# jianzongwu/betrayed-by-captions

Measured on NVIDIA B200. Metric: decoder_head_images_per_sec_1024, higher is better.
Workload: dtype bf16

## Files before the change

### betrayed-by-captions_b200/csrc/api.cu

```cuda
#include "../../include/cgg_b200.h"
#include "kernels.h"
#include "gemm_tc.h"
#include "gemm_tf32.h"
#include "tc_state.h"

#include <math.h>
#include <stdio.h>
#include <string.h>
#include <stdlib.h>
#include <string>
#include <vector>

using namespace cgg;

struct cgg_handle {
  cgg_config cfg;
  std::string err;
  bool prepared = false;
  int H4 = 0, W4 = 0, lh[CGG_NUM_LEVELS] = {0, 0, 0}, lw[CGG_NUM_LEVELS] = {0, 0, 0};
  int nl[CGG_NUM_LEVELS] = {0, 0, 0};
  float* pos_level[CGG_NUM_LEVELS] = {nullptr, nullptr, nullptr};
  float* wkv[CGG_NUM_LEVELS] = {nullptr, nullptr, nullptr};
  float* rk[CGG_NUM_LEVELS] = {nullptr, nullptr, nullptr};
  float* bkv[CGG_NUM_LEVELS] = {nullptr, nullptr, nullptr};
  TcState* tc = nullptr;
  cudaStream_t side[2] = {nullptr, nullptr};
  cudaEvent_t ev_fork = nullptr, ev_join[2] = {nullptr, nullptr}, ev_kv[CGG_NUM_LEVELS] = {nullptr, nullptr, nullptr};
  cudaEvent_t ev_me[CGG_MAX_LAYERS + 1] = {};
  bool overlap_kv = false;
  bool final_mask_only = false;
  TcState* tc_aux = nullptr;
  Tf32Ctx* tf32 = nullptr;
  struct K7Buf {
    __nv_bfloat16 *pred_hl = nullptr, *cap_hl = nullptr, *dst_hl = nullptr, *capT_hl = nullptr;
    float* S = nullptr;
    size_t n_pred = 0, n_cap = 0, n_dst = 0, n_capT = 0, n_S = 0;
    void release() {
      cudaFree(pred_hl); cudaFree(cap_hl); cudaFree(dst_hl); cudaFree(capT_hl); cudaFree(S);
      pred_hl = cap_hl = dst_hl = capT_hl = nullptr; S = nullptr; n_pred = n_cap = n_dst = n_capT = n_S = 0;
    }
  } k7;
  void free_tables() {
    for (int l = 0; l < CGG_NUM_LEVELS; ++l) {
      cudaFree(pos_level[l]); cudaFree(wkv[l]); cudaFree(rk[l]); cudaFree(bkv[l]);
      pos_level[l] = wkv[l] = rk[l] = bkv[l] = nullptr;
    }
  }
};

namespace {

int fail(cgg_handle* h, int code, const std::string& msg) {
  if (h) h->err = msg;
  return code;
}
#define CU(call)                                                                              \
  do {                                                                                        \
    cudaError_t e__ = (call);                                                                 \
    if (e__ != cudaSuccess)                                                                   \
      return fail(h, CGG_ERR_CUDA, std::string(#call) + ": " + cudaGetErrorString(e__));      \
  } while (0)
#define ST(call)                       \
  do {                                 \
    int s__ = (call);                  \
    if (s__ != CGG_OK) return s__;     \
  } while (0)

inline size_t align_up(size_t x) { return (x + 255) & ~(size_t)255; }

struct Workspace {
  size_t total = 0;
  size_t kv[CGG_NUM_LEVELS];
  size_t z, h1, h2, me, qb, kb, vb, o, t, x1, x2, f, xs, bitmap, allm, tcws;
  void carve(const cgg_handle* h, int B) {
    const cgg_config& c = h->cfg;
    size_t off = 0;
    auto take = [&](size_t bytes) { size_t o = off; off += align_up(bytes); return o; };
    const size_t kv_elt = (c.precision == CGG_BF16) ? 2 : 4;
    for (int l = 0; l < CGG_NUM_LEVELS; ++l)
      kv[l] = take((size_t)B * h->lh[l] * h->lw[l] * h->nl[l] * 2 * c.embed_dim * kv_elt);
    const size_t bqc = (size_t)B * c.num_queries * c.embed_dim * sizeof(float);
    z = take(bqc); h1 = take(bqc); h2 = take(bqc); me = take(bqc); qb = take(bqc); kb = take(bqc);
    vb = take(bqc); o = take(bqc); t = take(bqc); x1 = take(bqc); x2 = take(bqc);
    f = take((size_t)B * c.num_queries * c.ffn_dim * sizeof(float));
    xs = take(bqc * (c.num_layers + 1));
    int maxk = 0;
    for (int l = 0; l < CGG_NUM_LEVELS; ++l) maxk = max(maxk, h->lh[l] * h->lw[l]);
    bitmap = take((size_t)B * c.num_queries * ((maxk + 31) / 32) * sizeof(uint32_t));
    allm = take((size_t)B * c.num_queries);
    tcws = take(tc_workspace_bytes(h->tc, B));
    total = off;
  }
};

template <typename T>
T* at(void* ws, size_t off) { return reinterpret_cast<T*>(static_cast<char*>(ws) + off); }

int check_ws(cgg_handle* h, int B, void* ws, size_t bytes, Workspace& w) {
  if (!h->prepared) return fail(h, CGG_ERR_NOT_PREPARED, "cgg_prepare() has not been called");
  if (B <= 0) return fail(h, CGG_ERR_BAD_SHAPE, "batch must be positive");
  w.carve(h, B);
  if (!ws || bytes < w.total) return fail(h, CGG_ERR_WORKSPACE, "workspace too small");
  return CGG_OK;
}

int linear_rows(cgg_handle* h, cudaStream_t s, const float* x, const float* a2, int a2_mod, const float* W,
                const float* bias, float* y, int rows, int N, int K, float alpha = 1.f,
                const float* R = nullptr, bool relu = false) {
  GemmF32 p;
  p.A = x; p.sAm = K; p.sAk = 1;
  if (a2) { p.A2 = a2; p.sA2m = K; p.sA2k = 1; p.a2_mod = a2_mod; }
  p.W = W; p.sWn = K; p.sWk = 1;
  p.bias = bias; p.alpha = alpha;
  if (R) { p.R = R; p.sRm = N; p.sRn = 1; p.r_mod = rows; }
  p.C = y; p.sCm = N; p.sCn = 1;
  p.M = rows; p.N = N; p.K = K; p.batch = 1;
  if (relu) p.relu_from = 0;
  CU(launch_gemm_f32(p, s));
  return CGG_OK;
}

}

extern "C" const char* cgg_version(void) { return "1.0 sm_100a"; }

extern "C" uint64_t cgg_launch_count(void) { return (uint64_t)cgg::launch_count(); }

extern "C" const char* cgg_last_error(const cgg_handle* h) { return h ? h->err.c_str() : "null handle"; }

extern "C" int cgg_create(cgg_handle** out, const cgg_config* cfg) {
  if (!out || !cfg) return CGG_ERR_NULL;
  *out = nullptr;
  if (cfg->embed_dim != 256 || cfg->num_heads != 8) return CGG_ERR_UNSUPPORTED;
  if (cfg->num_layers < 1 || cfg->num_layers > CGG_MAX_LAYERS) return CGG_ERR_BAD_SHAPE;
  if (cfg->num_queries < 1 || cfg->num_queries > 1024 || cfg->ffn_dim < 1 || cfg->num_classes_p1 < 1 ||
      cfg->d_lang < 0 || (cfg->d_lang == 0 && cfg->pred_emb_norm))
    return CGG_ERR_BAD_SHAPE;
  if (cfg->precision != CGG_FP32 && cfg->precision != CGG_BF16) return CGG_ERR_UNSUPPORTED;
  int ndev = 0;
  if (cudaGetDeviceCount(&ndev) != cudaSuccess || ndev == 0) return CGG_ERR_CUDA;
  cgg_handle* h = new (std::nothrow) cgg_handle();
  if (!h) return CGG_ERR_CUDA;
  h->cfg = *cfg;
  if (cfg->precision == CGG_BF16) {
    h->tc = tc_create(*cfg);
    if (!h->tc) { delete h; return CGG_ERR_CUDA; }
    {
      int lo = 0, hi = 0;
      cudaDeviceGetStreamPriorityRange(&lo, &hi);
      bool ok = true;
      for (int i = 0; i < 2; ++i) ok = ok && cudaStreamCreateWithPriority(&h->side[i], cudaStreamNonBlocking, lo) == cudaSuccess;
      ok = ok && cudaEventCreateWithFlags(&h->ev_fork, cudaEventDisableTiming) == cudaSuccess;
      for (int i = 0; i < 2; ++i) ok = ok && cudaEventCreateWithFlags(&h->ev_join[i], cudaEventDisableTiming) == cudaSuccess;
      for (int i = 0; i < CGG_NUM_LEVELS; ++i) ok = ok && cudaEventCreateWithFlags(&h->ev_kv[i], cudaEventDisableTiming) == cudaSuccess;
      for (int i = 0; i <= CGG_MAX_LAYERS; ++i) ok = ok && cudaEventCreateWithFlags(&h->ev_me[i], cudaEventDisableTiming) == cudaSuccess;
      h->overlap_kv = ok;
// ... 89 lines not shown
  Workspace w;
  w.carve(h, batch);
  return w.total;
}

extern "C" size_t cgg_workspace_offset(const cgg_handle* h, int batch, const char* what) {
  if (!h || !h->prepared || batch <= 0 || !what) return (size_t)-1;
  Workspace w;
  w.carve(h, batch);
  const std::string n(what);
  if (n == "kv0") return w.kv[0];
  if (n == "kv1") return w.kv[1];
  if (n == "kv2") return w.kv[2];
  const size_t o = tc_workspace_offset(h->tc, batch, what);
  return o == (size_t)-1 ? o : w.tcws + o;
}

static int kv_project_levels(cgg_handle* h, const cgg_weights* w, int batch, const void* const memories[CGG_NUM_LEVELS],
                             void* workspace, size_t workspace_bytes, cudaStream_t s, int l_begin, int l_end,
                             int cta_cap = 0) {
  if (!h || !w || !memories) return CGG_ERR_NULL;
  Workspace ws;
  ST(check_ws(h, batch, workspace, workspace_bytes, ws));
  const int C = h->cfg.embed_dim;
  for (int l = l_begin; l < l_end; ++l) {
    if (h->nl[l] == 0) continue;
    if (!memories[l]) return fail(h, CGG_ERR_NULL, "null memory level");
    const int K = h->lh[l] * h->lw[l], N = h->nl[l] * 2 * C;
    if (h->cfg.precision == CGG_BF16) {
      int st = tc_kv_project(h->tc, l, batch, memories[l], at<void>(workspace, ws.kv[l]), at<void>(workspace, ws.tcws), s, cta_cap);
      if (st != CGG_OK) return fail(h, st, std::string("tc_kv_project: ") + tc_last_error(h->tc));
      continue;
    }
    GemmF32 p;
    p.A = static_cast<const float*>(memories[l]); p.sAb = (long)C * K; p.sAm = 1; p.sAk = K; p.a_mmajor = true;
    p.W = h->wkv[l]; p.sWn = C; p.sWk = 1;
    p.bias = h->bkv[l];
    p.R = h->rk[l]; p.sRm = (long)h->nl[l] * C; p.sRn = 1; p.r_mod = K; p.r_ncols = h->nl[l] * C;
    p.C = at<float>(workspace, ws.kv[l]); p.sCb = (long)K * N; p.sCm = N; p.sCn = 1;
    p.M = K; p.N = N; p.K = C; p.batch = batch;
    CU(launch_gemm_f32(p, s));
  }
  return CGG_OK;
}

extern "C" int cgg_kv_project(cgg_handle* h, const cgg_weights* w, int batch, const void* const memories[CGG_NUM_LEVELS],
                              void* workspace, size_t workspace_bytes, void* stream) {
  return kv_project_levels(h, w, batch, memories, workspace, workspace_bytes, (cudaStream_t)stream, 0, CGG_NUM_LEVELS);
}

extern "C" int cgg_attn_mask_from_logits(cgg_handle* h, int batch, const float* mask_pred, int H4, int W4, int th,
                                         int tw, uint32_t* bitmap, uint8_t* all_masked, void* stream) {
  if (!h || !mask_pred || !bitmap || !all_masked) return CGG_ERR_NULL;
  if (batch <= 0 || H4 <= 0 || W4 <= 0 || th <= 0 || tw <= 0) return fail(h, CGG_ERR_BAD_SHAPE, "bad shape");
  CU(launch_mask_bits(mask_pred, batch * h->cfg.num_queries, H4, W4, th, tw, bitmap, all_masked, (cudaStream_t)stream));
  return CGG_OK;
}

static int head_call_impl(cgg_handle* h, const cgg_weights* w, int batch, const float* x, const void* mask_features,
                          int target_level, float* cls, float* emb, void* mask, float* mask_embed_out,
                          uint32_t* bitmap, uint8_t* all_masked, void* workspace, size_t workspace_bytes,
                          cudaStream_t s, int call_slot, bool defer_einsum, bool fds_ready, bool z_ready = false) {
  if (!h || !w || !x || !mask_features || !cls || (!emb && h->cfg.d_lang > 0)) return CGG_ERR_NULL;
  if (!mask && !defer_einsum) return CGG_ERR_NULL;
  Workspace ws;
  ST(check_ws(h, batch, workspace, workspace_bytes, ws));
  if (bitmap && (target_level < 0 || target_level >= CGG_NUM_LEVELS)) return fail(h, CGG_ERR_BAD_SHAPE, "bad level");
  if (bitmap && !all_masked) return CGG_ERR_NULL;
  const cgg_config& c = h->cfg;
  const int C = c.embed_dim, Q = c.num_queries, rows = batch * Q, HW = h->H4 * h->W4;
  float* z = at<float>(workspace, ws.z);
  float* h1 = at<float>(workspace, ws.h1);
  float* h2 = at<float>(workspace, ws.h2);
  float* me = mask_embed_out ? mask_embed_out : at<float>(workspace, ws.me);
  if (c.precision == CGG_BF16) {
    int st = tc_query_heads(h->tc, w, batch, x, cls, emb, me, at<void>(workspace, ws.tcws), s, call_slot, z_ready);
    if (st != CGG_OK) return fail(h, st, std::string("tc_query_heads: ") + tc_last_error(h->tc));
  } else {
  CU(launch_layernorm(x, nullptr, w->post_norm_w, w->post_norm_b, z, rows, C, 1e-5f, true, s));
  ST(linear_rows(h, s, z, nullptr, 1, w->cls_w, w->cls_b, cls, rows, c.num_classes_p1, C));
  if (c.d_lang > 0) ST(linear_rows(h, s, z, nullptr, 1, w->v2l_w, w->v2l_b, emb, rows, c.d_lang, C));
  ST(linear_rows(h, s, z, nullptr, 1, w->me_w[0], w->me_b[0], h1, rows, C, C, 1.f, nullptr, true));
  ST(linear_rows(h, s, h1, nullptr, 1, w->me_w[1], w->me_b[1], h2, rows, C, C, 1.f, nullptr, true));
  ST(linear_rows(h, s, h2, nullptr, 1, w->me_w[2], w->me_b[2], me, rows, C, C));
  }
  if (c.pred_emb_norm && c.d_lang > 0) CU(launch_l2norm_rows(emb, rows, c.d_lang, s));
  if (c.precision == CGG_BF16) {
    void* tws = at<void>(workspace, ws.tcws);
#define TC(call)                                                                                \
  do {                                                                                          \
    int st__ = (call);                                                                          \
    if (st__ != CGG_OK) return fail(h, st__, std::string(#call) + ": " + tc_last_error(h->tc)); \
  } while (0)
    TC(tc_store_mask_embed(h->tc, batch, call_slot, me, tws, s));
    if (bitmap) {
      if (!fds_ready) TC(tc_downsample(h->tc, batch, mask_features, tws, s));
      TC(tc_mask_bits(h->tc, batch, call_slot, target_level, bitmap, all_masked, tws, s));
    }
    if (!defer_einsum) TC(tc_mask_einsum(h->tc, batch, call_slot, 1, mask_features, mask, 0, tws, s));
    return CGG_OK;
  }
  GemmF32 p;
  p.A = static_cast<const float*>(mask_features); p.sAb = (long)C * HW; p.sAm = 1; p.sAk = HW; p.a_mmajor = true;
  p.W = me; p.sWb = (long)Q * C; p.sWn = C; p.sWk = 1;
  p.C = static_cast<float*>(mask); p.sCb = (long)Q * HW; p.sCm = 1; p.sCn = HW; p.c_mmajor = true;
  p.M = HW; p.N = Q; p.K = C; p.batch = batch;
  CU(launch_gemm_f32(p, s));
  if (bitmap)
    CU(launch_mask_bits(static_cast<const float*>(mask), rows, h->H4, h->W4, h->lh[target_level], h->lw[target_level],
                        bitmap, all_masked, s));
  return CGG_OK;
}

extern "C" int cgg_head_call(cgg_handle* h, const cgg_weights* w, int batch, const float* x, const void* mask_features,
                             int target_level, float* cls, float* emb, void* mask, float* mask_embed_out,
                             uint32_t* bitmap, uint8_t* all_masked, void* workspace, size_t workspace_bytes,
                             void* stream) {
  if (!mask) return CGG_ERR_NULL;
  return head_call_impl(h, w, batch, x, mask_features, target_level, cls, emb, mask, mask_embed_out, bitmap, all_masked,
                        workspace, workspace_bytes, (cudaStream_t)stream, 0, false, false);
}

extern "C" int cgg_mask_einsum(cgg_handle* h, int batch, int first_call, int num_calls, const void* mask_features,
                               void* mask, void* workspace, size_t workspace_bytes, void* stream) {
  if (!h || !mask_features || !mask) return CGG_ERR_NULL;
  if (h->cfg.precision != CGG_BF16) return fail(h, CGG_ERR_UNSUPPORTED, "cgg_mask_einsum is a CGG_BF16 stage");
  Workspace ws;
  ST(check_ws(h, batch, workspace, workspace_bytes, ws));
  if (first_call < 0 || num_calls < 1 || first_call + num_calls > h->cfg.num_layers + 1)
    return fail(h, CGG_ERR_BAD_SHAPE, "bad head-call range");
  const long call_stride = (long)batch * h->cfg.num_queries * h->H4 * h->W4;
  int st = tc_mask_einsum(h->tc, batch, first_call, num_calls, mask_features, mask, call_stride,
                          at<void>(workspace, ws.tcws), (cudaStream_t)stream);
  if (st != CGG_OK) return fail(h, st, std::string("tc_mask_einsum: ") + tc_last_error(h->tc));
  return CGG_OK;
}

extern "C" int cgg_masked_attention(cgg_handle* h, int batch, int num_keys, const float* q, const void* k,
                                    const void* v, long kv_stride, long kv_batch_stride, const uint32_t* bitmap,
                                    const uint8_t* all_masked, float* out, void* stream) {
  if (!h || !q || !k || !v || !out) return CGG_ERR_NULL;
  if (batch <= 0 || num_keys <= 0) return fail(h, CGG_ERR_BAD_SHAPE, "bad shape");
  cudaStream_t s = (cudaStream_t)stream;
  if (h->cfg.precision == CGG_BF16) {
    int st = tc_attention(h->tc, batch, num_keys, q, k, v, kv_stride, kv_batch_stride, bitmap, all_masked, out, nullptr, s);
    if (st != CGG_OK) return fail(h, st, std::string("tc_attention: ") + tc_last_error(h->tc));
    return CGG_OK;
  }
  CU(launch_attention_f32(q, k, v, false, kv_stride, kv_batch_stride, bitmap, all_masked, out, nullptr, batch,
                          h->cfg.num_queries, num_keys, h->cfg.num_heads, s));
  return CGG_OK;
}

static int decoder_layer_impl(cgg_handle* h, const cgg_weights* w, int batch, int layer, const float* x_in,
                              const uint32_t* bitmap, const uint8_t* all_masked, float* x_out, void* workspace,
                              size_t workspace_bytes, void* stream, bool chained_in, bool chained_out,
                              bool q_ready = false);

extern "C" int cgg_decoder_layer(cgg_handle* h, const cgg_weights* w, int batch, int layer, const float* x_in,
                                 const uint32_t* bitmap, const uint8_t* all_masked, float* x_out, void* workspace,
                                 size_t workspace_bytes, void* stream) {
  return decoder_layer_impl(h, w, batch, layer, x_in, bitmap, all_masked, x_out, workspace, workspace_bytes, stream, false,
                            false);
}

static int decoder_layer_impl(cgg_handle* h, const cgg_weights* w, int batch, int layer, const float* x_in,
                              const uint32_t* bitmap, const uint8_t* all_masked, float* x_out, void* workspace,
                              size_t workspace_bytes, void* stream, bool chained_in, bool chained_out, bool q_ready) {
  if (!h || !w || !x_in || !x_out) return CGG_ERR_NULL;
  cudaStream_t s = (cudaStream_t)stream;
  Workspace ws;
  ST(check_ws(h, batch, workspace, workspace_bytes, ws));
  const cgg_config& c = h->cfg;
  if (layer < 0 || layer >= c.num_layers) return fail(h, CGG_ERR_BAD_SHAPE, "bad layer index");
  const int C = c.embed_dim, Q = c.num_queries, rows = batch * Q, F = c.ffn_dim;
  const int l = layer % CGG_NUM_LEVELS, sl = layer / CGG_NUM_LEVELS, n = h->nl[l];
  const int K = h->lh[l] * h->lw[l];
  if (c.precision == CGG_BF16) {
    const long kvs = (long)n * 2 * C, kvb = (long)K * kvs;
    const __nv_bfloat16* kv = at<__nv_bfloat16>(workspace, ws.kv[l]);
    int st = tc_decoder_layer(h->tc, w, batch, layer, x_in, kv + (size_t)sl * C, kv + (size_t)(n + sl) * C, kvs, kvb, K,
                              bitmap, all_masked, x_out, at<void>(workspace, ws.tcws), s, chained_in, chained_out, q_ready);
    if (st != CGG_OK) return fail(h, st, std::string("tc_decoder_layer: ") + tc_last_error(h->tc));
    return CGG_OK;
  }
  const cgg_layer_weights& lw = w->layers[layer];
  const float qscale = 1.0f / sqrtf((float)(C / c.num_heads));
  float* qb = at<float>(workspace, ws.qb);
  float* kb = at<float>(workspace, ws.kb);
  float* vb = at<float>(workspace, ws.vb);
  float* o = at<float>(workspace, ws.o);
  float* t = at<float>(workspace, ws.t);
  float* x1 = at<float>(workspace, ws.x1);
  float* x2 = at<float>(workspace, ws.x2);
  float* f = at<float>(workspace, ws.f);
  ST(linear_rows(h, s, x_in, w->query_embed, Q, lw.cross_in_w, lw.cross_in_b, qb, rows, C, C, qscale));
  const long kv_stride = (long)n * 2 * C, kv_bstride = (long)K * kv_stride;
  if (c.precision == CGG_BF16) {
    const __nv_bfloat16* kv = at<__nv_bfloat16>(workspace, ws.kv[l]);
    ST(cgg_masked_attention(h, batch, K, qb, kv + (size_t)sl * C, kv + (size_t)(n + sl) * C, kv_stride, kv_bstride,
                            bitmap, all_masked, o, stream));
  } else {
    const float* kv = at<float>(workspace, ws.kv[l]);
    ST(cgg_masked_attention(h, batch, K, qb, kv + (size_t)sl * C, kv + (size_t)(n + sl) * C, kv_stride, kv_bstride,
                            bitmap, all_masked, o, stream));
  }
  ST(linear_rows(h, s, o, nullptr, 1, lw.cross_out_w, lw.cross_out_b, t, rows, C, C, 1.f, x_in));
  CU(launch_layernorm(t, nullptr, lw.norm_w[0], lw.norm_b[0], x1, rows, C, 1e-5f, true, s));
  ST(linear_rows(h, s, x1, w->query_embed, Q, lw.self_in_w, lw.self_in_b, qb, rows, C, C, qscale));
  ST(linear_rows(h, s, x1, w->query_embed, Q, lw.self_in_w + (size_t)C * C, lw.self_in_b + C, kb, rows, C, C));
  ST(linear_rows(h, s, x1, nullptr, 1, lw.self_in_w + (size_t)2 * C * C, lw.self_in_b + 2 * C, vb, rows, C, C));
  CU(launch_attention_f32(qb, kb, vb, false, C, (long)Q * C, nullptr, nullptr, o, nullptr, batch, Q, Q, c.num_heads, s));
  ST(linear_rows(h, s, o, nullptr, 1, lw.self_out_w, lw.self_out_b, t, rows, C, C, 1.f, x1));
  CU(launch_layernorm(t, nullptr, lw.norm_w[1], lw.norm_b[1], x2, rows, C, 1e-5f, true, s));
  ST(linear_rows(h, s, x2, nullptr, 1, lw.ffn_w1, lw.ffn_b1, f, rows, F, C, 1.f, nullptr, true));
  ST(linear_rows(h, s, f, nullptr, 1, lw.ffn_w2, lw.ffn_b2, t, rows, C, F, 1.f, x2));
  CU(launch_layernorm(t, nullptr, lw.norm_w[2], lw.norm_b[2], x_out, rows, C, 1e-5f, true, s));
  return CGG_OK;
}

extern "C" int cgg_set_final_mask_only(cgg_handle* h, int on) {
  if (!h) return CGG_ERR_NULL;
  if (on && h->cfg.precision != CGG_BF16) return fail(h, CGG_ERR_UNSUPPORTED, "final-mask-only is a CGG_BF16 option");
  h->final_mask_only = on != 0;
  return CGG_OK;
}

extern "C" int cgg_decoder_forward(cgg_handle* h, const cgg_weights* w, int batch, const void* mask_features,
                                   const void* const memories[CGG_NUM_LEVELS], float* cls, float* emb, void* mask,
                                   float* x_states, uint32_t* const* bitmaps, uint8_t* all_masked, void* workspace,
                                   size_t workspace_bytes, void* stream) {
  if (!h || !w || !mask_features || !memories || !cls || (!emb && h->cfg.d_lang > 0) || !mask) return CGG_ERR_NULL;
  cudaStream_t s = (cudaStream_t)stream;
  Workspace ws;
  ST(check_ws(h, batch, workspace, workspace_bytes, ws));
  const cgg_config& c = h->cfg;
  const int C = c.embed_dim, Q = c.num_queries, L = c.num_layers;
  const size_t bqc = (size_t)batch * Q * C;
  const size_t HW = (size_t)h->H4 * h->W4;
  const size_t mask_elt = (c.precision == CGG_BF16) ? 2 : 4;
  float* xs = x_states ? x_states : at<float>(workspace, ws.xs);
  const bool tcm = c.precision == CGG_BF16;
  const bool ovl_kv = tcm && h->overlap_kv && L >= CGG_NUM_LEVELS;
  void* tws = at<void>(workspace, ws.tcws);
  if (ovl_kv) {
    CU(cudaEventRecord(h->ev_fork, s));
    CU(cudaStreamWaitEvent(h->side[0], h->ev_fork, 0));
    ST(kv_project_levels(h, w, batch, memories, workspace, workspace_bytes, s, 0, 1));
    for (int l = 1; l < CGG_NUM_LEVELS; ++l) {
      ST(kv_project_levels(h, w, batch, memories, workspace, workspace_bytes, h->side[0], l, l + 1));
      CU(cudaEventRecord(h->ev_kv[l], h->side[0]));
    }
  } else {
    ST(cgg_kv_project(h, w, batch, memories, workspace, workspace_bytes, stream));
  }
  if (tcm) {
    int st = tc_downsample(h->tc, batch, mask_features, tws, s);
    if (st != CGG_OK) return fail(h, st, std::string("tc_downsample: ") + tc_last_error(h->tc));
  }
  CU(launch_broadcast_rows(w->query_feat, xs, batch, Q, C, s));
  for (int j = 0; j <= L; ++j) {
    const bool need_mask = j < L;
    const bool q_par = ovl_kv && j > 0 && j < L;
    if (q_par) {
      CU(cudaEventRecord(h->ev_me[j], s));
      CU(cudaStreamWaitEvent(h->side[1], h->ev_me[j], 0));
      int st = tc_layer_qproj(h->tc, w, batch, j, tws, h->side[1]);
      if (st != CGG_OK) return fail(h, st, std::string("tc_layer_qproj: ") + tc_last_error(h->tc));
      CU(cudaEventRecord(h->ev_join[1], h->side[1]));
    }
    uint32_t* bm = need_mask ? ((bitmaps && bitmaps[j]) ? bitmaps[j] : at<uint32_t>(workspace, ws.bitmap)) : nullptr;
    uint8_t* am = need_mask ? (all_masked ? all_masked + (size_t)j * batch * Q : at<uint8_t>(workspace, ws.allm))
                            : nullptr;
    ST(head_call_impl(h, w, batch, xs + j * bqc, mask_features, j % CGG_NUM_LEVELS,
                      cls + (size_t)j * batch * Q * c.num_classes_p1, emb ? emb + (size_t)j * batch * Q * c.d_lang : nullptr,
                      static_cast<char*>(mask) + (size_t)j * batch * Q * HW * mask_elt, nullptr, bm, am, workspace,
                      workspace_bytes, s, j, tcm, true, tcm && j > 0));
    if (j < L) {
      const int lvl = j % CGG_NUM_LEVELS;
      if (ovl_kv && j == lvl && lvl > 0) CU(cudaStreamWaitEvent(s, h->ev_kv[lvl], 0));
      if (q_par) CU(cudaStreamWaitEvent(s, h->ev_join[1], 0));
      ST(decoder_layer_impl(h, w, batch, j, xs + j * bqc, bm, am, xs + (j + 1) * bqc, workspace, workspace_bytes, stream,
                            tcm && j > 0, tcm, q_par));
    }
  }
  if (tcm && h->final_mask_only) {
    int st = tc_mask_einsum(h->tc, batch, L, 1, mask_features, mask, (long)batch * Q * HW, tws, s);
    if (st != CGG_OK) return fail(h, st, std::string("tc_mask_einsum: ") + tc_last_error(h->tc));
  } else if (tcm) {
    int st = tc_mask_einsum(h->tc, batch, 0, L + 1, mask_features, mask, (long)batch * Q * HW, tws, s);
    if (st != CGG_OK) return fail(h, st, std::string("tc_mask_einsum: ") + tc_last_error(h->tc));
  }
  return CGG_OK;
}

extern "C" int cgg_noun_embeddings(cgg_handle* h, const float* table, const float* ln_w, const float* ln_b,
                                   const int64_t* ids, int n_ids, int d_lang, float eps, int text_emb_norm, float* out,
                                   void* stream) {
  if (!h || !table || !ids || !out) return CGG_ERR_NULL;
  if (text_emb_norm && (!ln_w || !ln_b)) return CGG_ERR_NULL;
  if (n_ids < 0 || d_lang <= 0) return fail(h, CGG_ERR_BAD_SHAPE, "bad shape");
  CU(launch_layernorm(table, ids, ln_w, ln_b, out, n_ids, d_lang, eps, text_emb_norm != 0, (cudaStream_t)stream));
  return CGG_OK;
}

extern "C" int cgg_similarity(cgg_handle* h, const float* a, const float* b, int M, int N, int D, float scale,
// ... 491 lines not shown
```

### betrayed-by-captions_b200/csrc/gemm_tc.cu

```cuda
#include "gemm_tc.h"
#include "kernels.h"
#include <cuda_fp16.h>
#include "tc_ptx.cuh"
#include "tc_state.h"

#include <cuda.h>
#include <cuda_bf16.h>
#include <string>
#include <stdio.h>
#include <stdlib.h>

namespace cgg {

namespace {

constexpr int TC_THREADS = 64 + 16 * 32;
constexpr int TC_BM = 128;
constexpr int TC_BK = 64;
constexpr int A_CHUNK_BYTES = 2 * 64 * 64 * 2;

enum { EPI_MASK_T = 0, EPI_ROWMAJOR = 1, EPI_BITS = 2, EPI_LINEAR_T = 3 };

struct TcGemmP {
  int NT, N_TILE, KC, stages;
  int a_resident;
  int a_kmajor;
  int k_identity;
  int a_kcoord[12];
  int b_kcoord[12];
  int split_cpc, split_K;
  TcSeg seg[3]; int nseg; const float* lin_bias; int n_tokens;
  long kpart_stride;
  int b_row0;
  int b_rows_per_batch;
  int acc_stride;
  int tmem_cols;
  int epi;
  int dbg;
  int f16;
  int ein_split, q_rows;
  int M_valid;
  int m_tiles, n_batch, n_work;
  __nv_bfloat16* out_mask; long out_call_stride, out_batch_stride, HW; int Q, q_pad, n_calls;
  __nv_bfloat16* out_rows; long ld_out, out_rows_batch_stride; const float* bias; const __nv_bfloat16* R;
  long ldr; int r_ncols;
  uint32_t* bitmap; int W32;
};

__device__ __forceinline__ bool masked_from_logit(float d) {
  return (1.0f / (1.0f + expf(-d))) < 0.5f;
}

__device__ __forceinline__ uint32_t pack_bf16x2(float lo, float hi) {
  __nv_bfloat162 v = __floats2bfloat162_rn(lo, hi);
  return *reinterpret_cast<uint32_t*>(&v);
}

__device__ __forceinline__ void split_bf16(float x, __nv_bfloat16& hi, __nv_bfloat16& lo) {
  hi = __float2bfloat16_rn(x);
  lo = __float2bfloat16_rn(x - __bfloat162float(hi));
}
__device__ __forceinline__ uint32_t pack2(__nv_bfloat16 a, __nv_bfloat16 b) {
  return (uint32_t)__bfloat16_as_ushort(a) | ((uint32_t)__bfloat16_as_ushort(b) << 16);
}


__device__ long long g_tc_trace[64];
#define TC_TRACE(gi, slot)                                                                         \
  do {                                                                                             \
    if ((p.dbg & 1) && blockIdx.x == 0 && (gi) >= 16 && (gi) < 24) g_tc_trace[((gi) - 16) * 8 + (slot)] = clock64(); \
  } while (0)

constexpr int EPI_WARPS = 16;
constexpr int EPI_PARTS = EPI_WARPS / 4;

struct EpiCtx {
  int lane, m, batch, part, chunks, wi, col0, g = -1;
  bool m_ok;
  uint32_t taddr;
};

__device__ __forceinline__ void epi_mask_t(const TcGemmP& p, const EpiCtx& c, uint8_t* sStage, const CUtensorMap* tmC,
                                           bool leader_warp, bool last, int m_tile, uint64_t* acc_empty_bar,
                                           bool arrive_on_leader) {
  const bool leader = leader_warp && c.lane == 0;
  static_assert(EPI_PARTS == 4, "four chunk slots per warp below");
  uint32_t r0[16], r1[16], r2[16], r3[16];
  const int ch0 = c.part, ch1 = c.part + 4, ch2 = c.part + 8, ch3 = c.part + 12;
  const bool on0 = ch0 < c.chunks, on1 = ch1 < c.chunks, on2 = ch2 < c.chunks, on3 = ch3 < c.chunks;
  if (on0) ptx::tmem_ld16_issue(c.taddr + (uint32_t)(ch0 * 16), r0);
  if (on1) ptx::tmem_ld16_issue(c.taddr + (uint32_t)(ch1 * 16), r1);
  if (on2) ptx::tmem_ld16_issue(c.taddr + (uint32_t)(ch2 * 16), r2);
  if (on3) ptx::tmem_ld16_issue(c.taddr + (uint32_t)(ch3 * 16), r3);
  if (on0) ptx::tmem_ld_wait16(r0);
  if (on1) ptx::tmem_ld_wait16(r1);
  if (on2) ptx::tmem_ld_wait16(r2);
  if (on3) ptx::tmem_ld_wait16(r3);
  ptx::tc_fence_before();
  __syncwarp();
  if (c.lane == 0) {
    if (arrive_on_leader) ptx::mbar_arrive_leader(acc_empty_bar);
    else ptx::mbar_arrive(acc_empty_bar);
  }
  if (leader) ptx::tma_store_wait_read();
  asm volatile("bar.sync 1, %0;" ::"n"(EPI_WARPS * 32) : "memory");
  if (leader) TC_TRACE(c.g, 6);
  const int row = c.m & (TC_BM - 1);
  auto stage16 = [&](const uint32_t (&r)[16], int ch) {
    __nv_bfloat16* dst = reinterpret_cast<__nv_bfloat16*>(sStage) + (long)(ch * 16) * TC_BM + row;
#pragma unroll
    for (int i = 0; i < 16; ++i) dst[i * TC_BM] = __float2bfloat16_rn(__uint_as_float(r[i]));
  };
  if (on0) stage16(r0, ch0);
  if (on1) stage16(r1, ch1);
  if (on2) stage16(r2, ch2);
  if (on3) stage16(r3, ch3);
  if (leader) TC_TRACE(c.g, 7);
  ptx::fence_proxy_async_smem();
  asm volatile("bar.sync 1, %0;" ::"n"(EPI_WARPS * 32) : "memory");
  if (leader) {
    const int r0 = c.col0;
    const int N_TILE = c.chunks * 16, q_pad = p.q_pad;
    if (N_TILE >= q_pad) {
      for (int sidx = 0; sidx * q_pad + q_pad <= N_TILE || sidx == 0; ++sidx) {
        const int call = r0 / q_pad + sidx;
        if (call >= p.n_calls || sidx * q_pad >= N_TILE) break;
        ptx::tma_store_3d(tmC, sStage + (long)sidx * q_pad * TC_BM * 2, m_tile * TC_BM, 0, call * p.n_batch + c.batch);
      }
    } else {
      const int call = r0 / q_pad, q0 = r0 - call * q_pad;
      if (call < p.n_calls) ptx::tma_store_3d(tmC, sStage, m_tile * TC_BM, q0, call * p.n_batch + c.batch);
    }
    ptx::tma_store_commit();
    if (last) ptx::tma_store_wait_read();
  }
}

__device__ __forceinline__ void epi_rowmajor(const TcGemmP& p, const EpiCtx& c, uint8_t* sStage, const float* sBias,
                                             const CUtensorMap* tmC, bool leader_warp, bool last, int m_tile,
                                             uint64_t* acc_empty_bar, bool arrive_on_leader = false) {
  const bool leader = leader_warp && c.lane == 0;
  static_assert(EPI_PARTS == 4, "four chunk slots per warp below");
  uint32_t r0[16], r1[16], r2[16], r3[16];
  const int ch0 = c.part, ch1 = c.part + 4, ch2 = c.part + 8, ch3 = c.part + 12;
  const bool on0 = ch0 < c.chunks, on1 = ch1 < c.chunks, on2 = ch2 < c.chunks, on3 = ch3 < c.chunks;
  if (on0) ptx::tmem_ld16_issue(c.taddr + (uint32_t)(ch0 * 16), r0);
  if (on1) ptx::tmem_ld16_issue(c.taddr + (uint32_t)(ch1 * 16), r1);
  if (on2) ptx::tmem_ld16_issue(c.taddr + (uint32_t)(ch2 * 16), r2);
  if (on3) ptx::tmem_ld16_issue(c.taddr + (uint32_t)(ch3 * 16), r3);
  if (on0) ptx::tmem_ld_wait16(r0);
  if (on1) ptx::tmem_ld_wait16(r1);
  if (on2) ptx::tmem_ld_wait16(r2);
  if (on3) ptx::tmem_ld_wait16(r3);
  ptx::tc_fence_before();
  __syncwarp();
  if (c.lane == 0) {
    if (arrive_on_leader) ptx::mbar_arrive_leader(acc_empty_bar);
    else ptx::mbar_arrive(acc_empty_bar);
  }
  if (leader) ptx::tma_store_wait_read();
  asm volatile("bar.sync 1, %0;" ::"n"(EPI_WARPS * 32) : "memory");
  const int row = c.m & (TC_BM - 1);
  auto stage16 = [&](const uint32_t (&r)[16], int ch) {
    const float* bf = sBias + c.col0 + ch * 16;
    uint4 o[2];
    uint32_t* ow = reinterpret_cast<uint32_t*>(o);
#pragma unroll
    for (int i = 0; i < 8; ++i)
      ow[i] = pack_bf16x2(__uint_as_float(r[2 * i]) + bf[2 * i], __uint_as_float(r[2 * i + 1]) + bf[2 * i + 1]);
    const int sub = ch >> 2, j = (ch & 3) * 2;
    uint8_t* base = sStage + sub * (TC_BM * 128) + row * 128;
    *reinterpret_cast<uint4*>(base + ((j ^ (row & 7)) << 4)) = o[0];
    *reinterpret_cast<uint4*>(base + (((j + 1) ^ (row & 7)) << 4)) = o[1];
  };
  if (on0) stage16(r0, ch0);
  if (on1) stage16(r1, ch1);
  if (on2) stage16(r2, ch2);
  if (on3) stage16(r3, ch3);
  ptx::fence_proxy_async_smem();
  asm volatile("bar.sync 1, %0;" ::"n"(EPI_WARPS * 32) : "memory");
  if (leader) {
    const int subs = c.chunks >> 2;
    for (int sub = 0; sub < subs; ++sub)
      ptx::tma_store_3d(tmC, sStage + sub * (TC_BM * 128), c.col0 + sub * 64, m_tile * TC_BM, c.batch);
    ptx::tma_store_commit();
    if (last) ptx::tma_store_wait_read();
  }
}

__device__ __forceinline__ void epi_bits_impl(int Q, int W32, uint32_t* bitmap, const EpiCtx& c) {
  uint32_t* brow = bitmap + (long)c.batch * Q * W32 + c.wi;
  const bool w_ok = c.wi < W32;
  for (int ch = c.part; ch < c.chunks; ch += EPI_PARTS) {
    float v[16];
    ptx::tmem_ld16(c.taddr + (uint32_t)(ch * 16), v);
    const int q0 = c.col0 + ch * 16;
#pragma unroll
    for (int i = 0; i < 16; ++i) {
      const uint32_t word = __ballot_sync(0xffffffffu, c.m_ok && v[i] <= -1.7881392e-07f);
      if (c.lane == 0 && w_ok && q0 + i < Q) brow[(long)(q0 + i) * W32] = word;
    }
  }
}
__device__ __forceinline__ void epi_bits(const TcGemmP& p, const EpiCtx& c) { epi_bits_impl(p.Q, p.W32, p.bitmap, c); }

struct LinCtx {
  bool on = false;
  int f = 0, mode = 0, rb_mod = 1, split_off = 0;
  long ld = 0, rb_ld = 0, res_ld = 0;
  float bias = 0.f, alpha = 1.f, floor = -INFINITY;
  void* ptr = nullptr;
  const float* rowbias = nullptr;
  const float* res = nullptr;
  __device__ __forceinline__ void init(const TcGemmP& p, int m) {
#pragma unroll
    for (int sgi = 0; sgi < 3; ++sgi) {
      if (sgi < p.nseg && m >= p.seg[sgi].col0 && m < p.seg[sgi].col0 + p.seg[sgi].ncols) {
        on = true;
        f = m - p.seg[sgi].col0;
        mode = p.seg[sgi].is_bf16 == 3 ? 3 : (p.seg[sgi].is_bf16 ? (p.seg[sgi].split ? 2 : 1) : 0);
        floor = p.seg[sgi].relu ? 0.f : -INFINITY;
        ptr = p.seg[sgi].ptr; ld = p.seg[sgi].ld; alpha = p.seg[sgi].alpha;
        rowbias = p.seg[sgi].rowbias; rb_mod = p.seg[sgi].rb_mod; rb_ld = p.seg[sgi].rb_ld;
        res = p.seg[sgi].res; res_ld = p.seg[sgi].res_ld; split_off = p.seg[sgi].ncols;
      }
    }
    if (on && p.lin_bias) bias = __ldg(p.lin_bias + m);
    if (blockIdx.z > 0) {
      bias = 0.f; res = nullptr; rowbias = nullptr;
      ptr = static_cast<float*>(ptr) + (long)blockIdx.z * p.kpart_stride;
    }
  }
};

struct LinPre {
  float a[16], b[16];
};
__device__ __forceinline__ void lin_prefetch(const TcGemmP& p, const EpiCtx& c, const LinCtx& L, LinPre& pre) {
  const int tok_base = c.batch * p.NT * p.N_TILE;
#pragma unroll
  for (int i = 0; i < 16; ++i) pre.a[i] = pre.b[i] = 0.f;
  if (!L.on || (L.rowbias == nullptr && L.res == nullptr)) return;
#pragma unroll
  for (int j = 0; j < 2; ++j) {
    const int ch = c.part + j * EPI_PARTS;
    if (ch >= c.chunks) break;
    const int tok0 = tok_base + ch * 16;
    const int nvalid = min(16, p.n_tokens - tok0);
    float* dst = j ? pre.b : pre.a;
    if (L.rowbias) {
      int tq = tok0 % L.rb_mod;
#pragma unroll
      for (int i = 0; i < 16; ++i) {
        if (i < nvalid) dst[i] = __ldg(L.rowbias + (long)tq * L.rb_ld + L.f);
        if (++tq == L.rb_mod) tq = 0;
      }
    } else {
      const float* rp = L.res + (long)tok0 * L.res_ld + L.f;
#pragma unroll
      for (int i = 0; i < 16; ++i)
        if (i < nvalid) dst[i] = __ldg(rp + (long)i * L.res_ld);
    }
  }
}

template <int MODE, bool HAS_RB, bool HAS_RES>
__device__ __forceinline__ void epi_linear_t(const TcGemmP& p, const EpiCtx& c, const LinCtx& L, const LinPre* pre) {
  const int n_tokens = p.n_tokens;
  const int tok_base = c.batch * p.NT * p.N_TILE + c.col0;
  int j = 0;
  for (int ch = c.part; ch < c.chunks; ch += EPI_PARTS, ++j) {
    const int tok0 = tok_base + ch * 16;
    const int nvalid = L.on ? min(16, n_tokens - tok0) : 0;
    float rb[16], rs[16];
    if (HAS_RB) {
      if (pre && j < 2) {
#pragma unroll
        for (int i = 0; i < 16; ++i) rb[i] = j ? pre->b[i] : pre->a[i];
      } else {
        int tq = tok0 % L.rb_mod;
#pragma unroll
        for (int i = 0; i < 16; ++i) {
          rb[i] = (i < nvalid) ? __ldg(L.rowbias + (long)tq * L.rb_ld + L.f) : 0.f;
          if (++tq == L.rb_mod) tq = 0;
        }
      }
    }
    if (HAS_RES) {
      if (pre && j < 2) {
#pragma unroll
        for (int i = 0; i < 16; ++i) rs[i] = j ? pre->b[i] : pre->a[i];
      } else {
        const float* rp = L.res + (long)tok0 * L.res_ld + L.f;
#pragma unroll
        for (int i = 0; i < 16; ++i) rs[i] = (i < nvalid) ? __ldg(rp + (long)i * L.res_ld) : 0.f;
      }
    }
    float v[16];
    ptx::tmem_ld16(c.taddr + (uint32_t)(ch * 16), v);
#pragma unroll
    for (int i = 0; i < 16; ++i) {
      float x = v[i] + L.bias;
      if (HAS_RB) x += rb[i];
      x *= L.alpha;
      if (HAS_RES) x += rs[i];
      x = fmaxf(x, L.floor);
      if (i < nvalid) {
        const long off = (long)(tok0 + i) * L.ld + L.f;
        if (MODE == 0) {
          static_cast<float*>(L.ptr)[off] = x;
        } else if (MODE == 1) {
          static_cast<__nv_bfloat16*>(L.ptr)[off] = __float2bfloat16_rn(x);
        } else if (MODE == 3) {
          static_cast<__half*>(L.ptr)[off] = __float2half_rn(x);
        } else {
          __nv_bfloat16 hi, lo;
          split_bf16(x, hi, lo);
          static_cast<__nv_bfloat16*>(L.ptr)[off] = hi;
          static_cast<__nv_bfloat16*>(L.ptr)[off + L.split_off] = lo;
        }
      }
    }
  }
}

__device__ __forceinline__ void epi_linear_dispatch(const TcGemmP& p, const EpiCtx& c, const LinCtx& L, const LinPre* pre) {
  const bool rb = L.rowbias != nullptr, rs = L.res != nullptr;
  if (L.mode == 0) {
    if (rb) epi_linear_t<0, true, false>(p, c, L, pre);
    else if (rs) epi_linear_t<0, false, true>(p, c, L, pre);
    else epi_linear_t<0, false, false>(p, c, L, pre);
  } else if (L.mode == 1) {
    if (rb) epi_linear_t<1, true, false>(p, c, L, pre);
    else epi_linear_t<1, false, false>(p, c, L, pre);
  } else if (L.mode == 3) {
    epi_linear_t<3, false, false>(p, c, L, pre);
  } else {
    epi_linear_t<2, false, false>(p, c, L, pre);
  }
}

__device__ unsigned long long g_tc_stamps[16];
#define TC_STAMP(i)                                                            \
  do {                                                                         \
    if ((p.dbg & 1) && blockIdx.x == 0 && blockIdx.y == 0) g_tc_stamps[i] = ptx::global_timer_ns(); \
  } while (0)

template <int EPI>
__global__ void __launch_bounds__(TC_THREADS, 1)
tc_gemm_kernel(const __grid_constant__ CUtensorMap tmA, const __grid_constant__ CUtensorMap tmB,
               const __grid_constant__ CUtensorMap tmC, const __grid_constant__ TcGemmP p) {
  constexpr bool A_KMAJOR = (EPI == EPI_LINEAR_T);
  constexpr bool A_RESIDENT = (EPI == EPI_MASK_T || EPI == EPI_ROWMAJOR);
  extern __shared__ uint8_t smem_raw[];
  uint8_t* smem = reinterpret_cast<uint8_t*>((reinterpret_cast<uintptr_t>(smem_raw) + 1023) & ~(uintptr_t)1023);
  const int b_tile_bytes = p.N_TILE * 128;
  const int a_in_stage = A_RESIDENT ? 0 : A_CHUNK_BYTES;
  const int b_stage_bytes = a_in_stage + b_tile_bytes;
  uint8_t* sA = smem;
  uint8_t* sB = sA + (A_RESIDENT ? p.KC * A_CHUNK_BYTES : 0);
  uint64_t* bars = reinterpret_cast<uint64_t*>(sB + p.stages * b_stage_bytes);
  uint64_t* a_full = bars;
  uint64_t* a_empty = bars + 4;
  uint64_t* b_full = bars + 8;
  uint64_t* b_empty = b_full + p.stages;
  uint64_t* acc_full = b_empty + p.stages;
  uint64_t* acc_empty = acc_full + 2;
  uint32_t* tmem_slot = reinterpret_cast<uint32_t*>(acc_empty + 2);
  uint8_t* sStage = reinterpret_cast<uint8_t*>((reinterpret_cast<uintptr_t>(tmem_slot + 4) + 1023) & ~(uintptr_t)1023);
  float* sBias = reinterpret_cast<float*>(sStage + (size_t)p.N_TILE * TC_BM * 2);

  const int warp = threadIdx.x >> 5, lane = threadIdx.x & 31;
  const int n_work = A_RESIDENT ? p.n_work : 1;
  const int w_first = A_RESIDENT ? (int)blockIdx.x : 0;
  const int w_stride = A_RESIDENT ? (int)gridDim.x : 1;
  auto tile_of = [&](int w, int& m_tile, int& batch) {
    if (A_RESIDENT) { batch = w / p.m_tiles; m_tile = w - batch * p.m_tiles; }
    else { m_tile = blockIdx.x; batch = blockIdx.y; }
  };
  if (threadIdx.x == 0) TC_STAMP(0);
  auto kcoords = [&](int kc, int& ka, int& kb) {
    if (p.split_cpc > 0) {
      const int term = kc / p.split_cpc, j = kc - term * p.split_cpc;
      const int k0 = ((int)blockIdx.z * p.split_cpc + j) * TC_BK;
      ka = (term == 2 ? p.split_K : 0) + k0;
      kb = (term == 1 ? p.split_K : 0) + k0;
    } else if (p.k_identity) {
      ka = kb = ((int)blockIdx.z * p.KC + kc) * TC_BK;
    } else {
      ka = p.a_kcoord[kc]; kb = p.b_kcoord[kc];
    }
  };

  if (warp == 0 && lane == 0) {
    ptx::prefetch_tmap(&tmA);
    ptx::prefetch_tmap(&tmB);
    for (int i = 0; i < 4; ++i) { ptx::mbar_init(&a_full[i], 1); ptx::mbar_init(&a_empty[i], 1); }
    for (int i = 0; i < p.stages; ++i) { ptx::mbar_init(&b_full[i], 1); ptx::mbar_init(&b_empty[i], 1); }
    for (int i = 0; i < 2; ++i) { ptx::mbar_init(&acc_full[i], 1); ptx::mbar_init(&acc_empty[i], EPI_WARPS); }
    ptx::fence_mbar_init();
  }
  if (warp == 1) {
    ptx::tmem_alloc(tmem_slot, (uint32_t)p.tmem_cols);
    ptx::tmem_relinquish();
  }
  ptx::tc_fence_before();
  __syncthreads();
  ptx::tc_fence_after();
  const uint32_t tmem_base = *tmem_slot;
  if (threadIdx.x == 0) TC_STAMP(1);
  ptx::grid_dep_launch();
  int n_pre = 0;
  if (EPI == EPI_LINEAR_T && warp == 0 && lane == 0) {
    const int total = p.NT * p.KC;
    n_pre = total < p.stages ? total : p.stages;
    for (int i = 0; i < n_pre; ++i) {
      const int kc = i % p.KC;
      int kco, kcb;
      kcoords(kc, kco, kcb);
      ptx::mbar_expect_tx(&b_full[i], (uint32_t)b_stage_bytes);
      ptx::tma_load_2d(sB + i * b_stage_bytes, &tmA, &b_full[i], kco, (int)blockIdx.x * TC_BM);
    }
  }
  ptx::grid_dep_wait();

  if (warp == 0) {
    if (lane == 0) {
      int m_tile = 0, batch = 0;
      auto load_a = [&](uint8_t* dst, uint64_t* bar, int kc) {
        int kco, kcb;
        kcoords(kc, kco, kcb);
        if (A_KMAJOR) {
          ptx::tma_load_2d(dst, &tmA, bar, kco, m_tile * TC_BM);
        } else {
          for (int g = 0; g < 2; ++g)
            ptx::tma_load_3d(dst + g * (A_CHUNK_BYTES / 2), &tmA, bar, m_tile * TC_BM + g * 64, kco, batch);
        }
      };
      int it = 0, tl = 0;
      for (int w = w_first; w < n_work; w += w_stride, ++tl) {
       tile_of(w, m_tile, batch);
       if (A_RESIDENT && tl == 0)
         for (int kc = 0; kc < p.KC; ++kc) {
           ptx::mbar_expect_tx(&a_full[kc], (uint32_t)A_CHUNK_BYTES);
           load_a(sA + kc * A_CHUNK_BYTES, &a_full[kc], kc);
         }
       for (int t = 0; t < p.NT; ++t)
        for (int kc = 0; kc < p.KC; ++kc, ++it) {
          if (A_RESIDENT && t == 0 && tl > 0) {
            ptx::mbar_wait(&a_empty[kc], (uint32_t)(tl & 1) ^ 1u);
            ptx::mbar_expect_tx(&a_full[kc], (uint32_t)A_CHUNK_BYTES);
            load_a(sA + kc * A_CHUNK_BYTES, &a_full[kc], kc);
          }
          const int s = it % p.stages;
          const uint32_t ph = (uint32_t)(it / p.stages) & 1u;
          uint8_t* stage = sB + s * b_stage_bytes;
          if (it >= n_pre) {
            ptx::mbar_wait(&b_empty[s], ph ^ 1u);
            ptx::mbar_expect_tx(&b_full[s], (uint32_t)b_stage_bytes);
            if (!A_RESIDENT) load_a(stage, &b_full[s], kc);
          }
          int kca, kcb;
          kcoords(kc, kca, kcb);
          ptx::tma_load_2d(stage + a_in_stage, &tmB, &b_full[s], kcb, batch * p.b_rows_per_batch + p.b_row0 + t * p.N_TILE);
        }
      }
    }
  } else if (warp == 1) {
    const uint32_t idesc = ptx::umma_idesc_bf16(TC_BM, p.N_TILE,  !A_KMAJOR,  false, p.f16 != 0);
    const uint64_t ad0 = A_KMAJOR ? ptx::umma_desc_sw128(ptx::smem_u32(A_RESIDENT ? sA : sB), 16, 1024)
                                  : ptx::umma_desc_sw128(ptx::smem_u32(A_RESIDENT ? sA : sB), A_CHUNK_BYTES / 2, 1024);
    const uint64_t bd0 = ptx::umma_desc_sw128(ptx::smem_u32(sB + a_in_stage), 16, 1024);
    const uint32_t a_step = A_KMAJOR ? 2u : (2048u >> 4);
    const uint32_t stage16 = (uint32_t)b_stage_bytes >> 4;
    int it = 0, g = 0, tl = 0;
    for (int w = w_first; w < n_work; w += w_stride, ++tl)
      for (int t = 0; t < p.NT; ++t, ++g) {
        const int buf = g & 1;
        const uint32_t use = (uint32_t)(g >> 1);
        ptx::mbar_wait(&acc_empty[buf], (use & 1u) ^ 1u);
        ptx::tc_fence_after();
        const uint32_t d_tmem = tmem_base + (uint32_t)(buf * p.acc_stride);
        for (int kc = 0; kc < p.KC; ++kc, ++it) {
          const int s = it % p.stages;
          const uint32_t ph = (uint32_t)(it / p.stages) & 1u;
          if (A_RESIDENT && t == 0) ptx::mbar_wait(&a_full[kc], (uint32_t)(tl & 1));
          ptx::mbar_wait(&b_full[s], ph);
          ptx::tc_fence_after();
          if (it == 0 && lane == 0) TC_STAMP(2);
          if (ptx::elect_one()) {
            const uint64_t ad = ad0 + (uint64_t)(A_RESIDENT ? (uint32_t)kc * (A_CHUNK_BYTES >> 4) : (uint32_t)s * stage16);
            const uint64_t bd = bd0 + (uint64_t)((uint32_t)s * stage16);
#pragma unroll
            for (int k = 0; k < TC_BK / 16; ++k)
              ptx::mma_bf16_ss(d_tmem, ad + (uint64_t)(k * a_step), bd + (uint64_t)(k * 2), idesc, (kc | k) != 0 ? 1u : 0u);
            ptx::mma_commit(&b_empty[s]);
            if (A_RESIDENT && t == p.NT - 1) ptx::mma_commit(&a_empty[kc]);
            if (kc == p.KC - 1) ptx::mma_commit(&acc_full[buf]);
          }
          __syncwarp();
        }
        if (g == 0 && lane == 0) TC_STAMP(3);
      }
  } else {
    const int quarter = warp & 3;
    const int part = (warp - 2) >> 2;
    if (EPI == EPI_ROWMAJOR) {
      for (int i = threadIdx.x - 64; i < p.NT * p.N_TILE; i += EPI_WARPS * 32) sBias[i] = __ldg(p.bias + i);
      asm volatile("bar.sync 1, %0;" ::"n"(EPI_WARPS * 32) : "memory");
    }
    int g = 0;
    for (int w = w_first; w < n_work; w += w_stride) {
    int m_tile, batch;
    tile_of(w, m_tile, batch);
    const bool last_work = w + w_stride >= n_work;
    const int m = m_tile * TC_BM + quarter * 32 + lane;
    const bool m_ok = m < p.M_valid;
    EpiCtx ctx;
    ctx.lane = lane; ctx.m = m; ctx.m_ok = m_ok; ctx.batch = batch; ctx.part = part;
    ctx.chunks = p.N_TILE / 16; ctx.wi = (m_tile * TC_BM + quarter * 32) >> 5;
    LinCtx lin;
    LinPre pre;
    const bool use_pre = EPI == EPI_LINEAR_T && p.NT == 1;
    if (EPI == EPI_LINEAR_T) {
      lin.init(p, m);
      if (use_pre) lin_prefetch(p, ctx, lin, pre);
    }
    for (int t = 0; t < p.NT; ++t, ++g) {
      const int buf = g & 1;
      const uint32_t use = (uint32_t)(g >> 1);
      ptx::mbar_wait(&acc_full[buf], use & 1u);
      ptx::tc_fence_after();
      if (g == 0 && warp == 2 && lane == 0) TC_STAMP(4);
      ctx.taddr = tmem_base + (uint32_t)(buf * p.acc_stride) + ((uint32_t)(quarter * 32) << 16);
      ctx.col0 = t * p.N_TILE;
      const bool last = last_work && t == p.NT - 1;
      if (EPI == EPI_MASK_T) epi_mask_t(p, ctx, sStage, &tmC, warp == 2, last, m_tile, &acc_empty[buf], false);
      else if (EPI == EPI_ROWMAJOR) epi_rowmajor(p, ctx, sStage, sBias, &tmC, warp == 2, last, m_tile, &acc_empty[buf]);
      else if (EPI == EPI_BITS) epi_bits(p, ctx);
      else epi_linear_dispatch(p, ctx, lin, use_pre ? &pre : nullptr);
      if (EPI != EPI_MASK_T && EPI != EPI_ROWMAJOR) {
// ... 550 lines not shown
    const int quarter = warp & 3;
    EpiCtx ctx;
    ctx.lane = lane; ctx.batch = batch; ctx.part = (warp - 2) >> 2; ctx.chunks = p.N_TILE / 16; ctx.col0 = 0;
    int t = 0;
    for (int mt = blockIdx.x; mt < p.m_tiles; mt += gridDim.x, ++t) {
      const int buf = t & 1;
      ptx::mbar_wait(&acc_full[buf], ((uint32_t)(t >> 1)) & 1u);
      ptx::tc_fence_after();
      ctx.m = mt * TC_BM + quarter * 32 + lane;
      ctx.m_ok = ctx.m < p.K_valid;
      ctx.wi = (mt * TC_BM + quarter * 32) >> 5;
      ctx.taddr = tmem_base + (uint32_t)(buf * p.acc_stride) + ((uint32_t)(quarter * 32) << 16);
      epi_bits_impl(p.Q, p.W32, p.bitmap, ctx);
      ptx::tc_fence_before();
      __syncwarp();
      if (lane == 0) ptx::mbar_arrive(&acc_empty[buf]);
    }
  }
  ptx::tc_fence_before();
  __syncthreads();
  if (warp == 1) {
    __syncwarp();
    ptx::tmem_dealloc(tmem_base, (uint32_t)p.tmem_cols);
  }
}

__global__ void __launch_bounds__(256) downsample3_kernel(const __nv_bfloat16* __restrict__ F, int planes, int C, int H4,
                                                          int W4, __half* __restrict__ d8, __half* __restrict__ d4,
                                                          __half* __restrict__ d2, int p8, int p4, int p2) {
  ptx::grid_dep_launch();
  ptx::grid_dep_wait();
  const int bw = W4 >> 3, bh = H4 >> 3;
  const long idx = (long)blockIdx.x * blockDim.x + threadIdx.x;
  const long total = (long)planes * bh * bw;
  if (idx >= total) return;
  const int bx = (int)(idx % bw);
  const int by = (int)((idx / bw) % bh);
  const long plane = idx / ((long)bw * bh);
  const __nv_bfloat16* src = F + plane * (long)H4 * W4 + (long)by * 8 * W4 + bx * 8;
  float px[8][8];
#pragma unroll
  for (int r = 0; r < 8; ++r) {
    const uint4 x = *reinterpret_cast<const uint4*>(src + (long)r * W4);
    const __nv_bfloat162* h = reinterpret_cast<const __nv_bfloat162*>(&x);
#pragma unroll
    for (int j = 0; j < 4; ++j) {
      const float2 f = __bfloat1622float2(h[j]);
      px[r][2 * j] = f.x;
      px[r][2 * j + 1] = f.y;
    }
  }
  auto avg = [&](int r, int c) {
    return 0.5f * (0.5f * px[r][c] + 0.5f * px[r][c + 1]) + 0.5f * (0.5f * px[r + 1][c] + 0.5f * px[r + 1][c + 1]);
  };
  auto h2 = [](float a, float b) {
    const __half2 v = __floats2half2_rn(a, b);
    return *reinterpret_cast<const uint32_t*>(&v);
  };
  d8[plane * (long)p8 + (long)by * bw + bx] = __float2half_rn(avg(3, 3));
  {
    const int w = W4 >> 2;
    const long off = (long)(by * 2) * w + bx * 2;
#pragma unroll
    for (int r = 0; r < 2; ++r)
      *reinterpret_cast<uint32_t*>(d4 + plane * (long)p4 + off + (long)r * w) = h2(avg(4 * r + 1, 1), avg(4 * r + 1, 5));
  }
  {
    const int w = W4 >> 1;
    const long off = (long)(by * 4) * w + bx * 4;
#pragma unroll
    for (int r = 0; r < 4; ++r) {
      uint2 ph;
      ph.x = h2(avg(2 * r, 0), avg(2 * r, 2));
      ph.y = h2(avg(2 * r, 4), avg(2 * r, 6));
      *reinterpret_cast<uint2*>(d2 + plane * (long)p2 + off + (long)r * w) = ph;
    }
  }
}

__global__ void repitch_kernel(const __nv_bfloat16* __restrict__ src, __nv_bfloat16* __restrict__ dst, long rows, int K,
                               int pitch) {
  ptx::grid_dep_launch();
  ptx::grid_dep_wait();
  const long i = (long)blockIdx.x * blockDim.x + threadIdx.x;
  if (i >= rows * pitch) return;
  const int k = (int)(i % pitch);
  const long r = i / pitch;
  dst[i] = k < K ? src[r * K + k] : __float2bfloat16(0.f);
}

__global__ void store_me_kernel(const float* __restrict__ me, __nv_bfloat16* __restrict__ dst, int B, int Q, int C,
                                int rows_per_batch, int row0) {
  ptx::grid_dep_launch();
  ptx::grid_dep_wait();
  const long i = (long)blockIdx.x * blockDim.x + threadIdx.x;
  const long total = (long)B * Q * C;
  if (i >= total) return;
  const int c = (int)(i % C);
  const long bq = i / C;
  const int q = (int)(bq % Q);
  const int b = (int)(bq / Q);
  __nv_bfloat16* row = dst + ((long)b * rows_per_batch + row0 + q) * 2 * C;
  row[c] = __float2bfloat16_rn(me[i]);
  reinterpret_cast<__half*>(row)[C + c] = __float2half_rn(me[i]);
}

__global__ void __launch_bounds__(256) all_masked_kernel(const uint32_t* __restrict__ bitmap, int rows, int W32, int K,
                                                         uint8_t* __restrict__ all_masked) {
  ptx::grid_dep_launch();
  ptx::grid_dep_wait();
  const int row = blockIdx.x * 8 + (threadIdx.x >> 5), lane = threadIdx.x & 31;
  if (row >= rows) return;
  int cnt = 0;
  for (int i = lane; i < W32; i += 32) cnt += __popc(bitmap[(long)row * W32 + i]);
#pragma unroll
  for (int o = 16; o > 0; o >>= 1) cnt += __shfl_xor_sync(0xffffffffu, cnt, o);
  if (lane == 0) all_masked[row] = (cnt == K) ? 1 : 0;
}

inline int round_up(int x, int m) { return (x + m - 1) / m * m; }
inline size_t align256(size_t x) { return (x + 255) & ~(size_t)255; }

}

namespace {

int make_map_A(TcState* t, CUtensorMap* m, const void* base, int pixels, int C, int B, int pitch = -1) {
  if (pitch < 0) pitch = pixels;
  if ((pitch * 2) % 16 != 0 || (reinterpret_cast<uintptr_t>(base) & 15))
    return tc_fail(t, CGG_ERR_UNSUPPORTED, "TMA needs 16-byte aligned channel planes (pixel pitch multiple of 8)");
  cuuint64_t dims[3] = {(cuuint64_t)pixels, (cuuint64_t)C, (cuuint64_t)B};
  cuuint64_t strides[2] = {(cuuint64_t)pitch * 2, (cuuint64_t)pitch * C * 2};
  cuuint32_t box[3] = {64, 64, 1};
  cuuint32_t es[3] = {1, 1, 1};
  CUresult r = t->encode(m, CU_TENSOR_MAP_DATA_TYPE_BFLOAT16, 3, const_cast<void*>(base), dims, strides, box, es,
                         CU_TENSOR_MAP_INTERLEAVE_NONE, CU_TENSOR_MAP_SWIZZLE_128B, CU_TENSOR_MAP_L2_PROMOTION_L2_128B,
                         CU_TENSOR_MAP_FLOAT_OOB_FILL_NONE);
  if (r != CUDA_SUCCESS) return tc_fail(t, CGG_ERR_CUDA, "cuTensorMapEncodeTiled(A) failed: " + std::to_string((int)r));
  return CGG_OK;
}
int make_map_B(TcState* t, CUtensorMap* m, const void* base, long rows, int C, int n_tile) {
  cuuint64_t dims[2] = {(cuuint64_t)C, (cuuint64_t)rows};
  cuuint64_t strides[1] = {(cuuint64_t)C * 2};
  cuuint32_t box[2] = {64, (cuuint32_t)n_tile};
  cuuint32_t es[2] = {1, 1};
  CUresult r = t->encode(m, CU_TENSOR_MAP_DATA_TYPE_BFLOAT16, 2, const_cast<void*>(base), dims, strides, box, es,
                         CU_TENSOR_MAP_INTERLEAVE_NONE, CU_TENSOR_MAP_SWIZZLE_128B, CU_TENSOR_MAP_L2_PROMOTION_L2_256B,
                         CU_TENSOR_MAP_FLOAT_OOB_FILL_NONE);
  if (r != CUDA_SUCCESS) return tc_fail(t, CGG_ERR_CUDA, "cuTensorMapEncodeTiled(B) failed: " + std::to_string((int)r));
  return CGG_OK;
}

int launch_tc_gemm(TcState* t, const CUtensorMap& mA, const CUtensorMap& mB, TcGemmP p, int m_tiles, int batch,
                   cudaStream_t s, const CUtensorMap* mC = nullptr, int kparts = 1) {
  if (p.N_TILE % 16 != 0 || p.N_TILE < 16 || p.N_TILE > 256) return tc_fail(t, CGG_ERR_BAD_SHAPE, "bad N tile");
  p.acc_stride = p.N_TILE <= 128 ? 128 : 256;
  if (p.N_TILE <= 32) p.acc_stride = 32; else if (p.N_TILE <= 64) p.acc_stride = 64;
  p.tmem_cols = 2 * p.acc_stride;
  const size_t a_bytes = p.a_resident ? (size_t)p.KC * A_CHUNK_BYTES : 0;
  const size_t b_stage = (size_t)p.N_TILE * 128 + (p.a_resident ? 0 : A_CHUNK_BYTES);
  if (p.KC > 12 && !p.k_identity && p.split_cpc == 0) return tc_fail(t, CGG_ERR_BAD_SHAPE, "too many K chunks");
  const size_t stage_bytes = (p.epi == EPI_MASK_T || p.epi == EPI_ROWMAJOR)
                                 ? (size_t)p.N_TILE * TC_BM * 2 + 1024 + (p.epi == EPI_ROWMAJOR ? (size_t)p.NT * p.N_TILE * 4 : 0) : 0;
  const size_t budget = (size_t)204 * 1024 - stage_bytes;
  int stages = (int)((budget - a_bytes) / b_stage);
  if (stages > 8) stages = 8;
  if (stages > p.NT * p.KC) stages = p.NT * p.KC;
  if (stages < 2) return tc_fail(t, CGG_ERR_BAD_SHAPE, "tile does not fit shared memory");
  p.stages = stages;
  const size_t smem = 1024 + a_bytes + stages * b_stage + (8 + 2 * stages + 4) * 8 + 64 + stage_bytes;
  if (!t->smem_attr_set) {
    TCU(cudaFuncSetAttribute(tc_gemm_kernel<EPI_MASK_T>, cudaFuncAttributeMaxDynamicSharedMemorySize, 227 * 1024));
    TCU(cudaFuncSetAttribute(tc_gemm_kernel<EPI_ROWMAJOR>, cudaFuncAttributeMaxDynamicSharedMemorySize, 227 * 1024));
    TCU(cudaFuncSetAttribute(tc_gemm_kernel<EPI_BITS>, cudaFuncAttributeMaxDynamicSharedMemorySize, 227 * 1024));
    TCU(cudaFuncSetAttribute(tc_gemm_kernel<EPI_LINEAR_T>, cudaFuncAttributeMaxDynamicSharedMemorySize, 227 * 1024));
    t->smem_attr_set = true;
  }
  const bool want_res = (p.epi == EPI_MASK_T || p.epi == EPI_ROWMAJOR), want_km = (p.epi == EPI_LINEAR_T);
  if (want_res && p.KC > 4) return tc_fail(t, CGG_ERR_BAD_SHAPE, "resident A tile limited to 4 K chunks");
  if ((p.a_resident != 0) != want_res || (p.a_kmajor != 0) != want_km)
    return tc_fail(t, CGG_ERR_BAD_SHAPE, "operand layout does not match the kernel specialisation");
  static const bool timing = getenv("CGG_TC_TIMING") != nullptr;
  p.dbg = timing ? 1 : 0;
  cudaEvent_t e0 = nullptr, e1 = nullptr;
  if (timing) { cudaEventCreate(&e0); cudaEventCreate(&e1); cudaStreamSynchronize(s); cudaEventRecord(e0, s); }
  dim3 grid(m_tiles, batch, kparts);
  const dim3 block(TC_THREADS);
  p.m_tiles = m_tiles; p.n_batch = batch; p.n_work = m_tiles * batch;
  if (want_res) {
    const int persist = 1;
    if (t->num_sms == 0) {
      int dev = 0;
      cudaGetDevice(&dev);
      cudaDeviceGetAttribute(&t->num_sms, cudaDevAttrMultiProcessorCount, dev);
    }
    int ctas = persist ? (p.n_work < t->num_sms ? p.n_work : t->num_sms) : p.n_work;
    if (persist && t->cta_cap > 0 && ctas > t->cta_cap) ctas = t->cta_cap;
    grid = dim3(ctas, 1, 1);
  }
  const CUtensorMap& mCC = mC ? *mC : mB;
  switch (p.epi) {
    case EPI_MASK_T: TCU(launch_pdl(tc_gemm_kernel<EPI_MASK_T>, grid, block, smem, s, mA, mB, mCC, p)); break;
    case EPI_ROWMAJOR: TCU(launch_pdl(tc_gemm_kernel<EPI_ROWMAJOR>, grid, block, smem, s, mA, mB, mCC, p)); break;
    case EPI_BITS: TCU(launch_pdl(tc_gemm_kernel<EPI_BITS>, grid, block, smem, s, mA, mB, mCC, p)); break;
    default: TCU(launch_pdl(tc_gemm_kernel<EPI_LINEAR_T>, grid, block, smem, s, mA, mB, mCC, p)); break;
  }
  count_launch();
  TCU(cudaGetLastError());
  if (timing) {
    cudaEventRecord(e1, s);
    cudaStreamSynchronize(s);
    float ms = 0.f;
    cudaEventElapsedTime(&ms, e0, e1);
    unsigned long long st[16];
    cudaMemcpyFromSymbol(st, g_tc_stamps, sizeof(st));
    fprintf(stderr, "[tc_gemm] grid %dx%d epi %d NT %d KC %d N_TILE %d stages %d smem %zu: event %.1f us | setup %.1f first-data %.1f mma-issued %.1f "
            "acc-ready %.1f epi-done %.1f teardown %.1f (us since entry)\n", m_tiles, batch, p.epi, p.NT, p.KC, p.N_TILE, p.stages, smem,
            ms * 1e3, (st[1] - st[0]) * 1e-3, (st[2] - st[0]) * 1e-3, (st[3] - st[0]) * 1e-3, (st[4] - st[0]) * 1e-3,
            (st[5] - st[0]) * 1e-3, (st[6] - st[0]) * 1e-3);
    cudaEventDestroy(e0); cudaEventDestroy(e1);
  }
  return CGG_OK;
}

}

TcState* tc_create(const cgg_config& cfg) {
  TcState* t = new (std::nothrow) TcState();
  if (!t) return nullptr;
  t->cfg = cfg;
  void* fn = nullptr;
  cudaDriverEntryPointQueryResult qres;
  if (cudaGetDriverEntryPoint("cuTensorMapEncodeTiled", &fn, cudaEnableDefault, &qres) != cudaSuccess || !fn) {
    delete t;
    return nullptr;
  }
  t->encode = reinterpret_cast<EncodeTiledFn>(fn);
  const int Q = cfg.num_queries, calls = cfg.num_layers + 1;
  if (2 * round_up(Q, 8) <= 256 && calls % 2 == 0) {
    t->q_pad = round_up(Q, 8) < 16 ? 16 : round_up(Q, 8); t->ein_ntile = 2 * t->q_pad; t->ein_calls_per_tile = 2;
  } else if (round_up(Q, 16) <= 256) {
    t->q_pad = round_up(Q, 16); t->ein_ntile = t->q_pad; t->ein_calls_per_tile = 1;
  } else {
    t->q_pad = round_up(Q, 32); t->ein_ntile = t->q_pad / 2; t->ein_calls_per_tile = 0;
    if (t->ein_ntile > 256) { delete t; return nullptr; }
  }
  if (round_up(Q, 16) <= 256) { t->bits_ntile = round_up(Q, 16); t->bits_nt = 1; }
  else { t->bits_ntile = round_up(Q, 32) / 2; t->bits_nt = 2; }
  t->rows_per_batch = calls * t->q_pad;
  t->live_bytes = 1 << 20;
  if (cudaMalloc(&t->live_buf, t->live_bytes) != cudaSuccess) { delete t; return nullptr; }
  return t;
}

void tc_destroy(TcState* t) {
  if (!t) return;
  t->free_all();
  t->free_packed();
  cudaFree(t->live_buf);
  delete t;
}

const char* tc_last_error(const TcState* t) { return t ? t->err.c_str() : ""; }

size_t tc_workspace_bytes(const TcState* t, int batch) {
  if (!t) return 0;
  TcWs w;
  w.carve(t, batch);
  return w.total;
}

size_t tc_workspace_offset(const TcState* t, int batch, const char* what) {
  if (!t || !what) return (size_t)-1;
  TcWs w;
  w.carve(t, batch);
  const std::string n(what);
  if (n == "me_all") return w.me_all;
  if (n == "fds0") return w.fds[0];
  if (n == "fds1") return w.fds[1];
  if (n == "fds2") return w.fds[2];
  return (size_t)-1;
}
const void* tc_key_bias_table(const TcState* t, int level, long* cols) {
  if (cols) *cols = 2L * t->nl[level] * t->cfg.embed_dim;
  return t->rk[level];
}
int tc_rows_per_batch(const TcState* t) { return t ? t->rows_per_batch : 0; }
int tc_q_pad(const TcState* t) { return t ? t->q_pad : 0; }

int tc_prepare(TcState* t, const cgg_weights* w, int H4, int W4, const int* lh, const int* lw, const int* nl,
               float* const* wkv_f32, float* const* rk_f32, float* const* bkv_f32, cudaStream_t s) {
  const int C = t->cfg.embed_dim;
  const int ratio[3] = {8, 4, 2};
  for (int l = 0; l < 3; ++l)
    if (lh[l] * ratio[l] != H4 || lw[l] * ratio[l] != W4)
      return tc_fail(t, CGG_ERR_UNSUPPORTED,
                     "bf16 mode needs level sizes at exactly 1/8, 1/4, 1/2 of the mask-feature size (inputs padded to /32)");
  bool same = t->H4 == H4 && t->W4 == W4;
  for (int l = 0; l < 3; ++l) same = same && t->lh[l] == lh[l] && t->lw[l] == lw[l] && t->nl[l] == nl[l] && t->wkv[l];
  if (!same) {
    t->free_all();
    t->H4 = H4; t->W4 = W4;
    for (int l = 0; l < 3; ++l) {
      t->lh[l] = lh[l]; t->lw[l] = lw[l]; t->nl[l] = nl[l];
      const int n = nl[l] > 0 ? nl[l] : 1;
      TCU(cudaMalloc(&t->wkv[l], (size_t)n * 2 * C * C * 2));
      TCU(cudaMalloc(&t->rk[l], (size_t)lh[l] * lw[l] * n * C * 2 * 2));
    }
  }
  for (int l = 0; l < 3; ++l) {
    if (nl[l] == 0) continue;
    TCU(launch_cast_bf16(wkv_f32[l], t->wkv[l], (size_t)nl[l] * 2 * C * C, s));
    TCU(launch_cast_bf16_split(rk_f32[l], t->rk[l], lh[l] * lw[l], nl[l] * C, s));
    t->bkv[l] = bkv_f32[l];
  }
  return tc_pack_weights(t, w, s);
}

int tc_kv_project(TcState* t, int level, int batch, const void* mem_bf16, void* kv_bf16, void* ws, cudaStream_t s,
                  int cta_cap) {
  const int C = t->cfg.embed_dim, K = t->lh[level] * t->lw[level], N = t->nl[level] * 2 * C;
  CUtensorMap mA, mB;
  int pitch = K;
  if (K % 8) {
    TcWs w;
    w.carve(t, batch);
    pitch = pitch8(K);
    __nv_bfloat16* dst = reinterpret_cast<__nv_bfloat16*>(static_cast<char*>(ws) + w.memp[level]);
    const long total = (long)batch * C * pitch;
    TCU(launch_pdl(repitch_kernel, dim3((unsigned)((total + 255) / 256)), dim3(256), 0, s,
                   static_cast<const __nv_bfloat16*>(mem_bf16), dst, (long)batch * C, K, pitch));
    count_launch();
    mem_bf16 = dst;
  }
  int st = make_map_A(t, &mA, mem_bf16, K, C, batch, pitch);
  if (st != CGG_OK) return st;
  TcGemmP p = {};
  p.N_TILE = 256;
  if (N % p.N_TILE != 0) return tc_fail(t, CGG_ERR_BAD_SHAPE, "K/V width not a multiple of 256");
// ... 158 lines not shown
  TCU(launch_pdl(all_masked_kernel, dim3((rows + 7) / 8), dim3(256), 0, s, (const uint32_t*)bitmap, rows, p.W32, K, all_masked));
  count_launch();
  TCU(cudaGetLastError());
  return CGG_OK;
}

int tc_mask_einsum(TcState* t, int batch, int first_call, int num_calls, const void* mask_features_bf16,
                   void* mask_bf16, long call_stride, void* ws, cudaStream_t s) {
  TcWs w;
  w.carve(t, batch);
  const int C = t->cfg.embed_dim, Q = t->cfg.num_queries;
  const long HW = (long)t->H4 * t->W4;
  char* base = static_cast<char*>(ws);
  CUtensorMap mA, mB;
  int st = make_map_A(t, &mA, mask_features_bf16, (int)HW, C, batch);
  if (st != CGG_OK) return st;
  TcGemmP p = {};
  p.KC = C / TC_BK;
  p.a_resident = 1;
  for (int kc = 0; kc < p.KC; ++kc) p.a_kcoord[kc] = p.b_kcoord[kc] = kc * TC_BK;
  p.b_row0 = first_call * t->q_pad; p.b_rows_per_batch = t->rows_per_batch;
  p.epi = EPI_MASK_T; p.M_valid = (int)HW; p.Q = Q; p.q_pad = t->q_pad; p.n_calls = num_calls;
  p.out_mask = static_cast<__nv_bfloat16*>(mask_bf16);
  p.out_call_stride = call_stride; p.out_batch_stride = (long)Q * HW; p.HW = HW;
  if (t->ein_calls_per_tile == 2 && num_calls % 2 == 0) {
    p.N_TILE = t->ein_ntile; p.NT = num_calls / 2;
  } else if (t->ein_calls_per_tile == 0) {
    p.N_TILE = t->ein_ntile; p.NT = 2 * num_calls;
  } else {
    p.N_TILE = round_up(t->q_pad, 16); p.NT = num_calls;
    if (p.N_TILE != t->q_pad && num_calls > 1) {
      for (int c = 0; c < num_calls; ++c) {
        st = tc_mask_einsum(t, batch, first_call + c, 1, mask_features_bf16,
                            static_cast<__nv_bfloat16*>(mask_bf16) + (long)c * call_stride, call_stride, ws, s);
        if (st != CGG_OK) return st;
      }
      return CGG_OK;
    }
  }
  st = make_map_B(t, &mB, base + w.me_all, (long)batch * t->rows_per_batch + 128, 2 * C, p.N_TILE);
  if (st != CGG_OK) return st;
  if (num_calls > 1 && call_stride != (long)batch * Q * HW)
    return tc_fail(t, CGG_ERR_BAD_SHAPE, "mask outputs of consecutive head calls must be contiguous");
  CUtensorMap mC;
  {
    cuuint64_t dims[3] = {(cuuint64_t)HW, (cuuint64_t)Q, (cuuint64_t)num_calls * batch};
    cuuint64_t strides[2] = {(cuuint64_t)HW * 2, (cuuint64_t)Q * HW * 2};
    cuuint32_t box[3] = {(cuuint32_t)TC_BM, (cuuint32_t)(t->q_pad < p.N_TILE ? t->q_pad : p.N_TILE), 1};
    cuuint32_t es[3] = {1, 1, 1};
    CUresult r = t->encode(&mC, CU_TENSOR_MAP_DATA_TYPE_BFLOAT16, 3, mask_bf16, dims, strides, box, es,
                           CU_TENSOR_MAP_INTERLEAVE_NONE, CU_TENSOR_MAP_SWIZZLE_NONE, CU_TENSOR_MAP_L2_PROMOTION_NONE,
                           CU_TENSOR_MAP_FLOAT_OOB_FILL_NONE);
    if (r != CUDA_SUCCESS) return tc_fail(t, CGG_ERR_CUDA, "cuTensorMapEncodeTiled(mask out) failed: " + std::to_string((int)r));
  }
  const int m_tiles = (int)((HW + TC_BM - 1) / TC_BM);
  const bool t_split = t->q_pad > 128;
  const int t_rows = t_split ? t->q_pad / 2 : t->q_pad;
  if (m_tiles % 2 == 0 && HW % (2 * TC_BM) == 0 && t->q_pad <= 256 && t_rows % 8 == 0 && t_rows <= 128 && p.KC == 4 && C == 256) {
    const size_t e_chunk = (size_t)t_rows * 128;
    const size_t smem = 1024 + 4 * A_CHUNK_BYTES + 8 * e_chunk + 4 * e_chunk + 24 * 8 + 64;
    if (smem <= 227 * 1024) {
      CUtensorMap mE, mCt;
      st = make_map_B(t, &mE, base + w.me_all, (long)batch * t->rows_per_batch + 128, 2 * C, t_rows);
      if (st != CGG_OK) return st;
      {
        cuuint64_t dims[3] = {(cuuint64_t)HW, (cuuint64_t)Q, (cuuint64_t)num_calls * batch};
        cuuint64_t strides[2] = {(cuuint64_t)HW * 2, (cuuint64_t)Q * HW * 2};
        cuuint32_t box[3] = {64, (cuuint32_t)t_rows, 1};
        cuuint32_t es[3] = {1, 1, 1};
        CUresult r = t->encode(&mCt, CU_TENSOR_MAP_DATA_TYPE_BFLOAT16, 3, mask_bf16, dims, strides, box, es,
                               CU_TENSOR_MAP_INTERLEAVE_NONE, CU_TENSOR_MAP_SWIZZLE_128B, CU_TENSOR_MAP_L2_PROMOTION_NONE,
                               CU_TENSOR_MAP_FLOAT_OOB_FILL_NONE);
        if (r != CUDA_SUCCESS) return tc_fail(t, CGG_ERR_CUDA, "cuTensorMapEncodeTiled(mask out, swizzled) failed: " + std::to_string((int)r));
      }
      p.m_tiles = m_tiles; p.n_batch = batch; p.n_work = m_tiles * batch;
      p.dbg = 0; p.ein_split = t_split ? 1 : 0; p.q_rows = t_rows;
      if (!t->attr_ein_t) {
        TCU(cudaFuncSetAttribute(tc_einsum_t_kernel, cudaFuncAttributeMaxDynamicSharedMemorySize, 227 * 1024));
        t->attr_ein_t = true;
      }
      if (t->num_sms == 0) {
        int dev = 0;
        cudaGetDevice(&dev);
        cudaDeviceGetAttribute(&t->num_sms, cudaDevAttrMultiProcessorCount, dev);
      }
      int pairs = t->num_sms / 2;
      if (pairs > p.n_work / 2) pairs = p.n_work / 2;
      TCU(launch_pdl_cluster(2, tc_einsum_t_kernel, dim3(2 * pairs), dim3(TC_THREADS), smem, s, mA, mE, mCt, p));
      count_launch();
      TCU(cudaGetLastError());
      return CGG_OK;
    }
  }
  if (m_tiles % 2 == 0 && HW % TC_BM == 0 && p.N_TILE % 16 == 0 && p.KC == 4) {
    st = make_map_B(t, &mB, base + w.me_all, (long)batch * t->rows_per_batch + 128, 2 * C, p.N_TILE / 2);
    if (st != CGG_OK) return st;
    p.acc_stride = p.N_TILE <= 128 ? 128 : 256;
    p.tmem_cols = 2 * p.acc_stride;
    p.m_tiles = m_tiles; p.n_batch = batch; p.n_work = m_tiles * batch;
    p.dbg = 0;
    const size_t stage_bytes = (size_t)p.N_TILE * TC_BM * 2 + 1024;
    const size_t b_chunk = (size_t)(p.N_TILE / 2) * 128;
    const size_t smem = 1024 + 4 * A_CHUNK_BYTES + 8 * b_chunk + 24 * 8 + 64 + stage_bytes;
    if (smem <= 227 * 1024) {
      p.stages = 8;
      if (!t->attr_ein_pair) {
        TCU(cudaFuncSetAttribute(tc_einsum_pair_kernel, cudaFuncAttributeMaxDynamicSharedMemorySize, 227 * 1024));
        t->attr_ein_pair = true;
      }
      if (t->num_sms == 0) {
        int dev = 0;
        cudaGetDevice(&dev);
        cudaDeviceGetAttribute(&t->num_sms, cudaDevAttrMultiProcessorCount, dev);
      }
      int pairs = t->num_sms / 2;
      if (pairs > p.n_work / 2) pairs = p.n_work / 2;
      if (getenv("CGG_TC_TIMING")) p.dbg |= 1;
      TCU(launch_pdl_cluster(2, tc_einsum_pair_kernel, dim3(2 * pairs), dim3(TC_THREADS), smem, s, mA, mB, mC, p));
      count_launch();
      TCU(cudaGetLastError());
      if (p.dbg & 1) {
        cudaStreamSynchronize(s);
        long long tr[64];
        cudaMemcpyFromSymbol(tr, g_tc_trace, sizeof(tr));
        fprintf(stderr, "[pair einsum trace] cycles rel. to N-tile 16: mma(acc_empty ok, first B ok, committed) epi(acc_full ok, epi done, arrived) epi-inner(after bar1, after chunk loop)\n");
        for (int i = 0; i < 8; ++i) {
          fprintf(stderr, "  g=%d:", 16 + i);
          for (int j = 0; j < 8; ++j) fprintf(stderr, " %7lld", tr[i * 8 + j] - tr[0]);
          fprintf(stderr, "\n");
        }
      }
      return CGG_OK;
    }
  }
  return launch_tc_gemm(t, mA, mB, p, m_tiles, batch, s, &mC);
}

namespace {
int make_map_act(TcState* t, CUtensorMap* m, const void* base, long rows, int K) {
  cuuint64_t dims[2] = {(cuuint64_t)K, (cuuint64_t)rows};
  cuuint64_t strides[1] = {(cuuint64_t)K * 2};
  cuuint32_t box[2] = {64, 128};
  cuuint32_t es[2] = {1, 1};
  CUresult r = t->encode(m, CU_TENSOR_MAP_DATA_TYPE_BFLOAT16, 2, const_cast<void*>(base), dims, strides, box, es,
                         CU_TENSOR_MAP_INTERLEAVE_NONE, CU_TENSOR_MAP_SWIZZLE_128B, CU_TENSOR_MAP_L2_PROMOTION_L2_128B,
                         CU_TENSOR_MAP_FLOAT_OOB_FILL_NONE);
  if (r != CUDA_SUCCESS) return tc_fail(t, CGG_ERR_CUDA, "cuTensorMapEncodeTiled(act) failed: " + std::to_string((int)r));
  return CGG_OK;
}

}

int tc_linear(TcState* t, const __nv_bfloat16* A, int M, int K, const __nv_bfloat16* W, int n_padded, const float* bias,
              const TcSeg* segs, int nsegs, cudaStream_t s, bool split_k, int kparts, long kpart_stride, bool f16) {
  if (kparts < 1) kparts = 1;
  if (kparts > 1 && (nsegs != 1 || segs[0].is_bf16 || segs[0].relu || (K / TC_BK) % kparts != 0))
    return tc_fail(t, CGG_ERR_BAD_SHAPE, "K-parts need one plain fp32 output segment");
  if (K % TC_BK != 0 || n_padded % TC_BM != 0 || nsegs < 1 || nsegs > 3)
    return tc_fail(t, CGG_ERR_BAD_SHAPE, "tc_linear shape (features must be padded to 128)");
  for (int i = 0; i < nsegs; ++i)
    if (segs[i].col0 % 32 != 0) return tc_fail(t, CGG_ERR_BAD_SHAPE, "segment start must be a multiple of 32");
  const int row_len = split_k ? 2 * K : K;
  TcGemmP p = {};
  const int tok_cap = 128;
  const int n_tok_tiles = (M + tok_cap - 1) / tok_cap;
  p.N_TILE = ((M + n_tok_tiles - 1) / n_tok_tiles + 15) / 16 * 16;
  CUtensorMap mW, mX;
  int st = make_map_act(t, &mW, W, n_padded, row_len);
  if (st != CGG_OK) return st;
  st = make_map_B(t, &mX, A, M, row_len, p.N_TILE);
  if (st != CGG_OK) return st;
  p.NT = 1; p.KC = K / TC_BK / kparts; p.kpart_stride = kpart_stride;
  p.a_kmajor = 1; p.k_identity = 1; p.a_resident = 0;
  if (split_k) {
    p.k_identity = 0; p.split_cpc = K / TC_BK / kparts; p.split_K = K; p.KC = 3 * p.split_cpc;
  }
  p.b_row0 = 0; p.b_rows_per_batch = p.N_TILE;
  p.epi = EPI_LINEAR_T; p.M_valid = n_padded; p.n_tokens = M;
  p.f16 = f16 ? 1 : 0;
  p.nseg = nsegs; p.lin_bias = bias;
  for (int i = 0; i < nsegs; ++i) p.seg[i] = segs[i];
  return launch_tc_gemm(t, mW, mX, p, n_padded / TC_BM, n_tok_tiles, s, nullptr, kparts);
}

}
```

### betrayed-by-captions_b200/csrc/gemm_tc.h

```cpp
#pragma once
#include "../../include/cgg_b200.h"
#include <cuda_runtime.h>
#include <cuda_bf16.h>

namespace cgg {

struct TcState;

struct TcSeg {
  int col0, ncols;
  void* ptr; long ld;
  int is_bf16, relu;
  int split;
  float alpha;
  const float* rowbias; int rb_mod; long rb_ld;
  const float* res; long res_ld;
  int remap_q, remap_rows, remap_row0;
};

TcState* tc_create(const cgg_config& cfg);
void tc_destroy(TcState* t);
const char* tc_last_error(const TcState* t);
size_t tc_workspace_bytes(const TcState* t, int batch);
size_t tc_workspace_offset(const TcState* t, int batch, const char* what);
int tc_rows_per_batch(const TcState* t);
int tc_q_pad(const TcState* t);

int tc_prepare(TcState* t, const cgg_weights* w, int H4, int W4, const int* lh, const int* lw, const int* nl,
               float* const* wkv_f32, float* const* rk_f32, float* const* bkv_f32, cudaStream_t s);

int tc_kv_project(TcState* t, int level, int batch, const void* mem_bf16, void* kv_bf16, void* ws, cudaStream_t s,
                  int cta_cap = 0);

int tc_downsample(TcState* t, int batch, const void* mask_features_bf16, void* ws, cudaStream_t s);

int tc_store_mask_embed(TcState* t, int batch, int call_idx, const float* me_f32, void* ws, cudaStream_t s);

int tc_mask_bits(TcState* t, int batch, int call_idx, int level, uint32_t* bitmap, uint8_t* all_masked, void* ws,
                 cudaStream_t s);

int tc_mask_einsum(TcState* t, int batch, int first_call, int num_calls, const void* mask_features_bf16,
                   void* mask_bf16, long call_stride, void* ws, cudaStream_t s);

int tc_linear(TcState* t, const __nv_bfloat16* A, int M, int K, const __nv_bfloat16* W, int n_padded, const float* bias,
              const TcSeg* segs, int nsegs, cudaStream_t s, bool split_k = false, int kparts = 1, long kpart_stride = 0,
              bool f16 = false);
int tc_decoder_layer(TcState* t, const cgg_weights* w, int batch, int layer, const float* x_in, const void* k,
                     const void* v, long kv_stride, long kv_bstride, int num_keys, const uint32_t* bitmap,
                     const uint8_t* all_masked, float* x_out, void* ws, cudaStream_t s, bool chained_in = false,
                     bool chained_out = false, bool q_ready = false);
int tc_layer_qproj(TcState* t, const cgg_weights* w, int batch, int layer, void* ws, cudaStream_t s);
int tc_query_heads(TcState* t, const cgg_weights* w, int batch, const float* x, float* cls, float* emb, float* me_f32,
                   void* ws, cudaStream_t s, int call_slot = 0, bool z_ready = false);

int tc_attention(TcState* t, int batch, int num_keys, const float* q, const void* k, const void* v, long kv_stride,
                 long kv_bstride, const uint32_t* bitmap, const uint8_t* all_masked, float* out,
                 __nv_bfloat16* out_bf16, cudaStream_t s, const void* r_table = nullptr, long r_cols = 0, int r_col0 = 0,
                 int out_mode = 0);
const void* tc_key_bias_table(const TcState* t, int level, long* cols);

}
```

### betrayed-by-captions_b200/csrc/path_bf16.cu

```cuda
#include "gemm_tc.h"
#include "kernels.h"
#include "tc_ptx.cuh"
#include "tc_state.h"
#include <cuda_fp16.h>

#include <math.h>
#include <stdlib.h>

namespace cgg {

namespace {

inline int round_up(int x, int m) { return (x + m - 1) / m * m; }

__device__ __forceinline__ void split_pack(float a, float b, uint32_t& hi, uint32_t& lo) {
  const __nv_bfloat162 h = __floats2bfloat162_rn(a, b);
  const float2 back = __bfloat1622float2(h);
  const __nv_bfloat162 l = __floats2bfloat162_rn(a - back.x, b - back.y);
  hi = *reinterpret_cast<const uint32_t*>(&h);
  lo = *reinterpret_cast<const uint32_t*>(&l);
}

__global__ void add_qe_cast_kernel(const float* __restrict__ x, const float* __restrict__ qe,
                                   __nv_bfloat16* __restrict__ dst, long total, int per ) {
  ptx::grid_dep_launch();
  ptx::grid_dep_wait();
  const long i = ((long)blockIdx.x * blockDim.x + threadIdx.x) * 4;
  if (i >= total) return;
  const float4 a = *reinterpret_cast<const float4*>(x + i);
  const float4 b = *reinterpret_cast<const float4*>(qe + (i % per));
  const __half2 lo = __floats2half2_rn(a.x + b.x, a.y + b.y), hi = __floats2half2_rn(a.z + b.z, a.w + b.w);
  uint2 pk;
  pk.x = *reinterpret_cast<const uint32_t*>(&lo);
  pk.y = *reinterpret_cast<const uint32_t*>(&hi);
  *reinterpret_cast<uint2*>(dst + i) = pk;
}

__global__ void __launch_bounds__(256) ln_rows_kernel(const float* __restrict__ x, int nparts, long part_stride,
                                                      const float* __restrict__ w,
                                                      const float* __restrict__ b, int rows, float* __restrict__ out_f32,
                                                      __nv_bfloat16* __restrict__ out_bf16,
                                                      __nv_bfloat16* __restrict__ out_bf16_q,
                                                      const float* __restrict__ qe, int Q,
                                                      __nv_bfloat16* __restrict__ out_hl,
                                                      const float* __restrict__ w2, const float* __restrict__ b2) {
  ptx::grid_dep_launch();
  ptx::grid_dep_wait();
  const int row = blockIdx.x * 8 + (threadIdx.x >> 5), lane = threadIdx.x & 31;
  if (row >= rows) return;
  const int n0 = lane * 8;
  const float4* xr = reinterpret_cast<const float4*>(x + (long)row * 256 + n0);
  const float4 a = xr[0], c = xr[1];
  float v[8] = {a.x, a.y, a.z, a.w, c.x, c.y, c.z, c.w};
  for (int pt = 1; pt < nparts; ++pt) {
    const float4* xp = reinterpret_cast<const float4*>(x + pt * part_stride + (long)row * 256 + n0);
    const float4 e = xp[0], f = xp[1];
    v[0] += e.x; v[1] += e.y; v[2] += e.z; v[3] += e.w; v[4] += f.x; v[5] += f.y; v[6] += f.z; v[7] += f.w;
  }
  float s = 0.f;
#pragma unroll
  for (int i = 0; i < 8; ++i) s += v[i];
#pragma unroll
  for (int o = 16; o > 0; o >>= 1) s += __shfl_xor_sync(0xffffffffu, s, o);
  const float mu = s * (1.0f / 256.0f);
  float q = 0.f;
#pragma unroll
  for (int i = 0; i < 8; ++i) { const float d = v[i] - mu; q = fmaf(d, d, q); }
#pragma unroll
  for (int o = 16; o > 0; o >>= 1) q += __shfl_xor_sync(0xffffffffu, q, o);
  const float rstd = 1.0f / sqrtf(q * (1.0f / 256.0f) + 1e-5f);
  float y[8];
#pragma unroll
  for (int i = 0; i < 8; ++i) y[i] = (v[i] - mu) * rstd * __ldg(w + n0 + i) + __ldg(b + n0 + i);
  if (out_f32) {
    float4* d = reinterpret_cast<float4*>(out_f32 + (long)row * 256 + n0);
    d[0] = make_float4(y[0], y[1], y[2], y[3]);
    d[1] = make_float4(y[4], y[5], y[6], y[7]);
  }
  auto store_hl = [&](__nv_bfloat16* dst, const float* v8) {
    uint4 ph, pl;
    split_pack(v8[0], v8[1], ph.x, pl.x);
    split_pack(v8[2], v8[3], ph.y, pl.y);
    split_pack(v8[4], v8[5], ph.z, pl.z);
    split_pack(v8[6], v8[7], ph.w, pl.w);
    *reinterpret_cast<uint4*>(dst + (long)row * 512 + n0) = ph;
    *reinterpret_cast<uint4*>(dst + (long)row * 512 + 256 + n0) = pl;
  };
  auto store_h = [&](__nv_bfloat16* dst, const float* v8) {
    uint4 pk;
    uint32_t* w = reinterpret_cast<uint32_t*>(&pk);
#pragma unroll
    for (int i = 0; i < 4; ++i) {
      const __half2 h2 = __floats2half2_rn(v8[2 * i], v8[2 * i + 1]);
      w[i] = *reinterpret_cast<const uint32_t*>(&h2);
    }
    *reinterpret_cast<uint4*>(dst + (long)row * 256 + n0) = pk;
  };
  if (out_bf16) store_h(out_bf16, y);
  if (out_bf16_q) {
    const float* e = qe + (long)(row % Q) * 256 + n0;
    float yq[8];
#pragma unroll
    for (int i = 0; i < 8; ++i) yq[i] = y[i] + e[i];
    store_h(out_bf16_q, yq);
  }
  if (out_hl && w2) {
    float s2 = 0.f;
#pragma unroll
    for (int i = 0; i < 8; ++i) s2 += y[i];
#pragma unroll
    for (int o = 16; o > 0; o >>= 1) s2 += __shfl_xor_sync(0xffffffffu, s2, o);
    const float mu2 = s2 * (1.0f / 256.0f);
    float q2 = 0.f;
#pragma unroll
    for (int i = 0; i < 8; ++i) { const float d = y[i] - mu2; q2 = fmaf(d, d, q2); }
#pragma unroll
    for (int o = 16; o > 0; o >>= 1) q2 += __shfl_xor_sync(0xffffffffu, q2, o);
    const float rstd2 = 1.0f / sqrtf(q2 * (1.0f / 256.0f) + 1e-5f);
#pragma unroll
    for (int i = 0; i < 8; ++i) y[i] = (y[i] - mu2) * rstd2 * __ldg(w2 + n0 + i) + __ldg(b2 + n0 + i);
  }
  if (out_hl) store_hl(out_hl, y);
}

cudaError_t launch_ln_rows(const float* x, const float* w, const float* b, int rows, float* out_f32,
                           __nv_bfloat16* out_bf16, __nv_bfloat16* out_bf16_q, const float* qe, int Q,
                           __nv_bfloat16* out_hl, cudaStream_t s, const float* w2 = nullptr, const float* b2 = nullptr,
                           int nparts = 1, long part_stride = 0) {
  cudaError_t e = launch_pdl(ln_rows_kernel, dim3((rows + 7) / 8), dim3(256), 0, s, x, nparts, part_stride, w, b, rows, out_f32, out_bf16, out_bf16_q,
                             qe, Q > 0 ? Q : 1, out_hl, w2, b2);
  count_launch();
  return e != cudaSuccess ? e : cudaGetLastError();
}

template <typename T>
T* at(void* ws, size_t off) { return reinterpret_cast<T*>(static_cast<char*>(ws) + off); }

TcSeg seg(int col0, int ncols, void* ptr, long ld, bool bf16, bool relu, float alpha = 1.f, const float* rowbias = nullptr,
          int rb_mod = 1, long rb_ld = 0, bool split = false, const float* res = nullptr, long res_ld = 0) {
  TcSeg s;
  s.res = res; s.res_ld = res_ld; s.remap_q = 0; s.remap_rows = 0; s.remap_row0 = 0;
  s.col0 = col0; s.ncols = ncols; s.ptr = ptr; s.ld = ld; s.is_bf16 = bf16 ? 1 : 0; s.relu = relu ? 1 : 0;
  s.split = split ? 1 : 0;
  s.alpha = alpha; s.rowbias = rowbias; s.rb_mod = rb_mod; s.rb_ld = rb_ld;
  return s;
}

inline bool debug_sync_on() {
  static const bool on = getenv("CGG_DEBUG_SYNC") != nullptr;
  return on;
}
#define TST(call)                                                                                      \
  do {                                                                                                 \
    int st__ = (call);                                                                                 \
    if (st__ != CGG_OK) return st__;                                                                   \
    if (debug_sync_on()) {                                                                             \
      cudaError_t e2__ = cudaStreamSynchronize(s);                                                     \
      if (e2__ != cudaSuccess)                                                                         \
        return tc_fail(t, CGG_ERR_CUDA, std::string("after ") + #call + ": " + cudaGetErrorString(e2__)); \
    }                                                                                                  \
  } while (0)

}

int tc_pack_weights(TcState* t, const cgg_weights* w, cudaStream_t s) {
  const cgg_config& c = t->cfg;
  const int C = c.embed_dim, F = c.ffn_dim, Q = c.num_queries, L = c.num_layers;
  const int nh = round_up(c.d_lang + C + c.num_classes_p1, 256);
  if (c.d_lang % 16 != 0) return tc_fail(t, CGG_ERR_UNSUPPORTED, "d_lang must be a multiple of 16");
  if (!t->packed_alloc || t->nh_padded != nh) {
    t->free_packed();
    for (int i = 0; i < L; ++i) {
      TcState::LayerW& l = t->pl[i];
      TCU(cudaMalloc(&l.wq_c, (size_t)C * C * 2));
      TCU(cudaMalloc(&l.wo_c, (size_t)C * C * 2));
      TCU(cudaMalloc(&l.wqkv_s, (size_t)3 * C * C * 2));
      TCU(cudaMalloc(&l.wo_s, (size_t)C * C * 2));
      TCU(cudaMalloc(&l.w1, (size_t)F * C * 2));
      TCU(cudaMalloc(&l.w2, (size_t)C * F * 2));
      TCU(cudaMalloc(&l.rowbias_v, (size_t)Q * C * 4));
    }
    TCU(cudaMalloc(&t->wh, (size_t)nh * 2 * C * 2));
    TCU(cudaMalloc(&t->wme1, (size_t)C * 2 * C * 2));
    TCU(cudaMalloc(&t->wme2, (size_t)C * 2 * C * 2));
    TCU(cudaMalloc(&t->bias_h, (size_t)nh * 4));
    t->nh_padded = nh;
    t->packed_alloc = true;
  }
  for (int i = 0; i < L; ++i) {
    const cgg_layer_weights& lw = w->layers[i];
    TcState::LayerW& l = t->pl[i];
    TCU(launch_cast_f16(lw.cross_in_w, l.wq_c, (size_t)C * C, s));
    TCU(launch_cast_f16(lw.cross_out_w, l.wo_c, (size_t)C * C, s));
    TCU(launch_cast_f16(lw.self_in_w, l.wqkv_s, (size_t)3 * C * C, s));
    TCU(launch_cast_f16(lw.self_out_w, l.wo_s, (size_t)C * C, s));
    TCU(launch_cast_f16(lw.ffn_w1, l.w1, (size_t)F * C, s));
    TCU(launch_cast_f16(lw.ffn_w2, l.w2, (size_t)C * F, s));
    GemmF32 g;
    g.A = w->query_embed; g.sAm = C; g.sAk = 1;
    g.W = lw.self_in_w + (size_t)2 * C * C; g.sWn = C; g.sWk = 1;
    g.C = l.rowbias_v; g.sCm = C; g.sCn = 1;
    g.M = Q; g.N = C; g.K = C; g.alpha = -1.f;
    TCU(launch_gemm_f32(g, s));
  }
  TCU(cudaMemsetAsync(t->wh, 0, (size_t)nh * 2 * C * 2, s));
  TCU(cudaMemsetAsync(t->bias_h, 0, (size_t)nh * 4, s));
  if (c.d_lang > 0) TCU(launch_cast_bf16_split(w->v2l_w, t->wh, c.d_lang, C, s));
  TCU(launch_cast_bf16_split(w->me_w[0], t->wh + (size_t)c.d_lang * 2 * C, C, C, s));
  TCU(launch_cast_bf16_split(w->cls_w, t->wh + (size_t)(c.d_lang + C) * 2 * C, c.num_classes_p1, C, s));
  if (c.d_lang > 0) TCU(cudaMemcpyAsync(t->bias_h, w->v2l_b, (size_t)c.d_lang * 4, cudaMemcpyDeviceToDevice, s));
  TCU(cudaMemcpyAsync(t->bias_h + c.d_lang, w->me_b[0], (size_t)C * 4, cudaMemcpyDeviceToDevice, s));
  TCU(cudaMemcpyAsync(t->bias_h + c.d_lang + C, w->cls_b, (size_t)c.num_classes_p1 * 4, cudaMemcpyDeviceToDevice, s));
  TCU(launch_cast_bf16_split(w->me_w[1], t->wme1, C, C, s));
  TCU(launch_cast_bf16_split(w->me_w[2], t->wme2, C, C, s));
  return CGG_OK;
}

int tc_query_heads(TcState* t, const cgg_weights* w, int batch, const float* x, float* cls, float* emb, float* me,
                   void* ws, cudaStream_t s, int call_slot, bool z_ready) {
  const cgg_config& c = t->cfg;
  const int C = c.embed_dim, M = batch * c.num_queries;
  TcWs o;
  o.carve(t, batch);
  __nv_bfloat16* zb = at<__nv_bfloat16>(ws, o.zb);
  __nv_bfloat16* h1b = at<__nv_bfloat16>(ws, o.h1b);
  __nv_bfloat16* h2b = at<__nv_bfloat16>(ws, o.h2b);
  if (!z_ready) TCU(launch_ln_rows(x, w->post_norm_w, w->post_norm_b, M, nullptr, nullptr, nullptr, nullptr, 0, zb, s));
  TcSeg sh[3] = {seg(0, c.d_lang, emb, c.d_lang, false, false),
                 seg(c.d_lang, C, h1b, 2 * C, true, true, 1.f, nullptr, 1, 0, true),
                 seg(c.d_lang + C, c.num_classes_p1, cls, c.num_classes_p1, false, false)};
  TST(tc_linear(t, zb, M, C, t->wh, t->nh_padded, t->bias_h, sh, 3, s, true));
  TcSeg s2[1] = {seg(0, C, h2b, 2 * C, true, true, 1.f, nullptr, 1, 0, true)};
  TST(tc_linear(t, h1b, M, C, t->wme1, C, w->me_b[1], s2, 1, s, true));
  TcSeg s3[1] = {seg(0, C, me, C, false, false)};
  if (!me) {
    s3[0] = seg(0, C, at<__nv_bfloat16>(ws, o.me_all), 2 * C, true, false, 1.f, nullptr, 1, 0, true);
    s3[0].remap_q = c.num_queries; s3[0].remap_rows = t->rows_per_batch; s3[0].remap_row0 = call_slot * t->q_pad;
  }
  TST(tc_linear(t, h2b, M, C, t->wme2, C, w->me_b[2], s3, 1, s, true));
  return CGG_OK;
}

int tc_decoder_layer(TcState* t, const cgg_weights* w, int batch, int layer, const float* x_in, const void* k,
                     const void* v, long kv_stride, long kv_bstride, int num_keys, const uint32_t* bitmap,
                     const uint8_t* all_masked, float* x_out, void* ws, cudaStream_t s, bool chained_in, bool chained_out,
                     bool q_ready) {
  const cgg_config& c = t->cfg;
  const int C = c.embed_dim, Q = c.num_queries, M = batch * Q, F = c.ffn_dim;
  const cgg_layer_weights& lw = w->layers[layer];
  const TcState::LayerW& pw = t->pl[layer];
  const float qscale = 1.0f / sqrtf((float)(C / c.num_heads));
  TcWs o;
  o.carve(t, batch);
  __nv_bfloat16* xqb = at<__nv_bfloat16>(ws, o.xqb);
  __nv_bfloat16* xb = at<__nv_bfloat16>(ws, o.xb);
  __nv_bfloat16* ob = at<__nv_bfloat16>(ws, o.ob);
  __nv_bfloat16* fb = at<__nv_bfloat16>(ws, o.fb);
  float* qf = at<float>(ws, o.qf);
  float* qs = at<float>(ws, o.qs);
  float* kvs = at<float>(ws, o.kvs);
  float* x1 = at<float>(ws, o.x1);
  float* x2 = at<float>(ws, o.x2);
  float* t1 = at<float>(ws, o.t1);
  const long total = (long)M * C;
  if (!chained_in) {
    TCU(launch_pdl(add_qe_cast_kernel, dim3((unsigned)((total / 4 + 255) / 256)), dim3(256), 0, s, x_in, w->query_embed, xqb,
                   total, Q * C));
    count_launch();
    TCU(cudaGetLastError());
  }
  if (!q_ready) {
    TcSeg sq[1] = {seg(0, C, qf, C, false, false, qscale)};
    TST(tc_linear(t, xqb, M, C, pw.wq_c, C, lw.cross_in_b, sq, 1, s, false, 1, 0, true));
  }
  {
    const int level = layer % CGG_NUM_LEVELS, slot = layer / CGG_NUM_LEVELS;
    long rcols = 0;
    const void* rtab = tc_key_bias_table(t, level, &rcols);
    TST(tc_attention(t, batch, num_keys, qf, k, v, kv_stride, kv_bstride, bitmap, all_masked, nullptr, ob, s, rtab, rcols,
                     slot * C,  2));
  }
  TcSeg so[1] = {seg(0, C, t1, C, false, false, 1.f, nullptr, 1, 0, false, x_in, C)};
  TST(tc_linear(t, ob, M, C, pw.wo_c, C, lw.cross_out_b, so, 1, s, false, 1, 0, true));
  TCU(launch_ln_rows(t1, lw.norm_w[0], lw.norm_b[0], M, x1, nullptr, xqb, w->query_embed, Q, nullptr, s));
  __nv_bfloat16* kvb = reinterpret_cast<__nv_bfloat16*>(kvs);
  TcSeg sk[3] = {seg(0, C, qs, C, false, false, qscale), seg(C, C, kvb, 2 * C, true, false),
                 seg(2 * C, C, kvb + C, 2 * C, true, false, 1.f, pw.rowbias_v, Q, C)};
  TST(tc_linear(t, xqb, M, C, pw.wqkv_s, 3 * C, lw.self_in_b, sk, 3, s, false, 1, 0, true));
  TST(tc_attention(t, batch, Q, qs, kvb, kvb + C, 2 * C, (long)Q * 2 * C, nullptr, nullptr, nullptr, ob, s, nullptr, 0, 0,
                    2));
  TcSeg so2[1] = {seg(0, C, t1, C, false, false, 1.f, nullptr, 1, 0, false, x1, C)};
  TST(tc_linear(t, ob, M, C, pw.wo_s, C, lw.self_out_b, so2, 1, s, false, 1, 0, true));
  TCU(launch_ln_rows(t1, lw.norm_w[1], lw.norm_b[1], M, x2, xb, nullptr, nullptr, 0, nullptr, s));
  TcSeg sf[1] = {seg(0, F, fb, F, true, true)};
  sf[0].is_bf16 = 3;
  TST(tc_linear(t, xb, M, C, pw.w1, F, lw.ffn_b1, sf, 1, s, false, 1, 0, true));
  TcSeg sf2[1] = {seg(0, C, t1, C, false, false, 1.f, nullptr, 1, 0, false, x2, C)};
  const int kparts = (F / 64) % 4 == 0 ? 4 : 1;
  const long pstride = (long)M * C;
  TST(tc_linear(t, fb, M, F, pw.w2, C, lw.ffn_b2, sf2, 1, s, false, kparts, pstride, true));
  if (chained_out)
    TCU(launch_ln_rows(t1, lw.norm_w[2], lw.norm_b[2], M, x_out, nullptr, xqb, w->query_embed, Q, at<__nv_bfloat16>(ws, o.zb), s,
                       w->post_norm_w, w->post_norm_b, kparts, pstride));
  else
    TCU(launch_ln_rows(t1, lw.norm_w[2], lw.norm_b[2], M, x_out, nullptr, nullptr, nullptr, 0, nullptr, s, nullptr, nullptr,
                       kparts, pstride));
  return CGG_OK;
}

int tc_layer_qproj(TcState* t, const cgg_weights* w, int batch, int layer, void* ws, cudaStream_t s) {
  const cgg_config& c = t->cfg;
  const int C = c.embed_dim, M = batch * c.num_queries;
  const float qscale = 1.0f / sqrtf((float)(C / c.num_heads));
  TcWs o;
  o.carve(t, batch);
  TcSeg sq[1] = {seg(0, C, at<float>(ws, o.qf), C, false, false, qscale)};
  TST(tc_linear(t, at<__nv_bfloat16>(ws, o.xqb), M, C, t->pl[layer].wq_c, C, w->layers[layer].cross_in_b, sq, 1, s, false, 1, 0,
                true));
  return CGG_OK;
}

}
```

### betrayed-by-captions_b200/csrc/tc_ptx.cuh

```cuda
#pragma once
#include <cuda.h>
#include <cuda_runtime.h>
#include <stdint.h>
#include <stdlib.h>
#include <utility>

namespace cgg {

template <typename... KArgs, typename... Args>
inline cudaError_t launch_pdl_cluster(int cluster_x, void (*kernel)(KArgs...), dim3 grid, dim3 block, size_t smem,
                                      cudaStream_t s, Args&&... args) {
  static const bool off = getenv("CGG_NO_PDL") != nullptr;
  cudaLaunchConfig_t cfg = {};
  cfg.gridDim = grid; cfg.blockDim = block; cfg.dynamicSmemBytes = smem; cfg.stream = s;
  cudaLaunchAttribute attr[2];
  int n = 0;
  if (!off) {
    attr[n].id = cudaLaunchAttributeProgrammaticStreamSerialization;
    attr[n].val.programmaticStreamSerializationAllowed = 1;
    ++n;
  }
  if (cluster_x > 1) {
    attr[n].id = cudaLaunchAttributeClusterDimension;
    attr[n].val.clusterDim.x = (unsigned)cluster_x; attr[n].val.clusterDim.y = 1; attr[n].val.clusterDim.z = 1;
    ++n;
  }
  cfg.attrs = attr; cfg.numAttrs = n;
  return cudaLaunchKernelEx(&cfg, kernel, std::forward<Args>(args)...);
}
template <typename... KArgs, typename... Args>
inline cudaError_t launch_pdl(void (*kernel)(KArgs...), dim3 grid, dim3 block, size_t smem, cudaStream_t s, Args&&... args) {
  return launch_pdl_cluster(1, kernel, grid, block, smem, s, std::forward<Args>(args)...);
}

namespace ptx {

__device__ __forceinline__ void grid_dep_wait() { asm volatile("griddepcontrol.wait;" ::: "memory"); }
__device__ __forceinline__ void grid_dep_launch() { asm volatile("griddepcontrol.launch_dependents;" ::: "memory"); }

__device__ __forceinline__ uint32_t smem_u32(const void* p) {
  return static_cast<uint32_t>(__cvta_generic_to_shared(p));
}
__device__ __forceinline__ bool elect_one() {
  uint32_t pred;
  asm volatile(
      "{\n\t.reg .pred p;\n\telect.sync _|p, 0xffffffff;\n\tselp.u32 %0, 1, 0, p;\n\t}\n"
      : "=r"(pred));
  return pred != 0;
}

__device__ __forceinline__ void mbar_init(uint64_t* bar, uint32_t count) {
  asm volatile("mbarrier.init.shared::cta.b64 [%0], %1;" ::"r"(smem_u32(bar)), "r"(count));
}
__device__ __forceinline__ void fence_mbar_init() {
  asm volatile("fence.mbarrier_init.release.cluster;" ::: "memory");
}
__device__ __forceinline__ void mbar_expect_tx(uint64_t* bar, uint32_t bytes) {
  asm volatile("mbarrier.arrive.expect_tx.shared::cta.b64 _, [%0], %1;" ::"r"(smem_u32(bar)), "r"(bytes)
               : "memory");
}
__device__ __forceinline__ void mbar_arrive(uint64_t* bar) {
  asm volatile("mbarrier.arrive.shared::cta.b64 _, [%0];" ::"r"(smem_u32(bar)) : "memory");
}
__device__ __forceinline__ uint64_t global_timer_ns() {
  uint64_t t;
  asm volatile("mov.u64 %0, %globaltimer;" : "=l"(t));
  return t;
}
__device__ __forceinline__ void mbar_wait(uint64_t* bar, uint32_t parity) {
  const uint32_t addr = smem_u32(bar);
  uint32_t done = 0;
  uint64_t t0 = 0;
  for (uint32_t it = 0;; ++it) {
    asm volatile(
        "{\n\t.reg .pred p;\n\t"
        "mbarrier.try_wait.parity.shared::cta.b64 p, [%1], %2;\n\t"
        "selp.u32 %0, 1, 0, p;\n\t}\n"
        : "=r"(done)
        : "r"(addr), "r"(parity)
        : "memory");
    if (done) return;
    if ((it & 255u) == 255u) {
      const uint64_t now = global_timer_ns();
      if (t0 == 0) t0 = now;
      else if (now - t0 > 2000000000ull) __trap();
    }
  }
}

__device__ __forceinline__ void prefetch_tmap(const CUtensorMap* m) {
  asm volatile("prefetch.tensormap [%0];" ::"l"(reinterpret_cast<uint64_t>(m)) : "memory");
}
__device__ __forceinline__ void tma_load_2d(void* smem_dst, const CUtensorMap* m, uint64_t* bar, int c0, int c1) {
  asm volatile(
      "cp.async.bulk.tensor.2d.shared::cluster.global.mbarrier::complete_tx::bytes [%0], [%1, {%3, %4}], [%2];"
      ::"r"(smem_u32(smem_dst)), "l"(reinterpret_cast<uint64_t>(m)), "r"(smem_u32(bar)), "r"(c0), "r"(c1)
      : "memory");
}
__device__ __forceinline__ void tma_load_3d(void* smem_dst, const CUtensorMap* m, uint64_t* bar, int c0, int c1,
                                            int c2) {
  asm volatile(
      "cp.async.bulk.tensor.3d.shared::cluster.global.mbarrier::complete_tx::bytes [%0], [%1, {%3, %4, %5}], [%2];"
      ::"r"(smem_u32(smem_dst)), "l"(reinterpret_cast<uint64_t>(m)), "r"(smem_u32(bar)), "r"(c0), "r"(c1), "r"(c2)
      : "memory");
}

__device__ __forceinline__ void tma_load_4d(void* smem_dst, const CUtensorMap* m, uint64_t* bar, int c0, int c1,
                                            int c2, int c3) {
  asm volatile(
      "cp.async.bulk.tensor.4d.shared::cluster.global.mbarrier::complete_tx::bytes [%0], [%1, {%3, %4, %5, %6}], [%2];"
      ::"r"(smem_u32(smem_dst)), "l"(reinterpret_cast<uint64_t>(m)), "r"(smem_u32(bar)), "r"(c0), "r"(c1), "r"(c2), "r"(c3)
      : "memory");
}

__device__ __forceinline__ uint32_t cluster_ctarank() {
  uint32_t r;
  asm volatile("mov.u32 %0, %%cluster_ctarank;" : "=r"(r));
  return r;
}
__device__ __forceinline__ void cluster_sync_all() {
  asm volatile("barrier.cluster.arrive.release.aligned;\n\tbarrier.cluster.wait.acquire.aligned;" ::: "memory");
}

__device__ __forceinline__ void tma_store_3d(const CUtensorMap* m, const void* smem_src, int c0, int c1, int c2) {
  asm volatile("cp.async.bulk.tensor.3d.global.shared::cta.bulk_group [%0, {%2, %3, %4}], [%1];"
               ::"l"(reinterpret_cast<uint64_t>(m)), "r"(smem_u32(smem_src)), "r"(c0), "r"(c1), "r"(c2)
               : "memory");
}
__device__ __forceinline__ void tma_store_commit() { asm volatile("cp.async.bulk.commit_group;" ::: "memory"); }
__device__ __forceinline__ void tma_store_wait_read() { asm volatile("cp.async.bulk.wait_group.read 0;" ::: "memory"); }
__device__ __forceinline__ void fence_proxy_async_smem() { asm volatile("fence.proxy.async.shared::cta;" ::: "memory"); }

__device__ __forceinline__ void tmem_alloc(uint32_t* smem_result, uint32_t ncols) {
  asm volatile("tcgen05.alloc.cta_group::1.sync.aligned.shared::cta.b32 [%0], %1;" ::"r"(smem_u32(smem_result)),
               "r"(ncols)
               : "memory");
}
__device__ __forceinline__ void tmem_relinquish() {
  asm volatile("tcgen05.relinquish_alloc_permit.cta_group::1.sync.aligned;" ::: "memory");
}
__device__ __forceinline__ void tmem_dealloc(uint32_t taddr, uint32_t ncols) {
  asm volatile("tcgen05.dealloc.cta_group::1.sync.aligned.b32 %0, %1;" ::"r"(taddr), "r"(ncols) : "memory");
}
__device__ __forceinline__ void tc_fence_before() { asm volatile("tcgen05.fence::before_thread_sync;" ::: "memory"); }
__device__ __forceinline__ void tc_fence_after() { asm volatile("tcgen05.fence::after_thread_sync;" ::: "memory"); }

__device__ __forceinline__ void mma_bf16_ss(uint32_t d_tmem, uint64_t adesc, uint64_t bdesc, uint32_t idesc,
                                            uint32_t accumulate) {
  asm volatile(
      "{\n\t.reg .pred p;\n\tsetp.ne.b32 p, %4, 0;\n\t"
      "tcgen05.mma.cta_group::1.kind::f16 [%0], %1, %2, %3, p;\n\t}\n"
      ::"r"(d_tmem), "l"(adesc), "l"(bdesc), "r"(idesc), "r"(accumulate)
      : "memory");
}
__device__ __forceinline__ void mma_commit(uint64_t* bar) {
  asm volatile("tcgen05.commit.cta_group::1.mbarrier::arrive::one.shared::cluster.b64 [%0];" ::"r"(smem_u32(bar))
               : "memory");
}
__device__ __forceinline__ void tmem_ld16(uint32_t taddr, float* v) {
  uint32_t r[16];
  asm volatile(
      "tcgen05.ld.sync.aligned.32x32b.x16.b32 {%0, %1, %2, %3, %4, %5, %6, %7, %8, %9, %10, %11, %12, %13, %14, %15}, [%16];"
      : "=r"(r[0]), "=r"(r[1]), "=r"(r[2]), "=r"(r[3]), "=r"(r[4]), "=r"(r[5]), "=r"(r[6]), "=r"(r[7]), "=r"(r[8]),
        "=r"(r[9]), "=r"(r[10]), "=r"(r[11]), "=r"(r[12]), "=r"(r[13]), "=r"(r[14]), "=r"(r[15])
      : "r"(taddr));
  asm volatile("tcgen05.wait::ld.sync.aligned;" ::: "memory");
#pragma unroll
  for (int i = 0; i < 16; ++i) v[i] = __uint_as_float(r[i]);
}

__device__ __forceinline__ void tmem_ld16_issue(uint32_t taddr, uint32_t* r) {
  asm volatile(
      "tcgen05.ld.sync.aligned.32x32b.x16.b32 {%0, %1, %2, %3, %4, %5, %6, %7, %8, %9, %10, %11, %12, %13, %14, %15}, [%16];"
      : "=r"(r[0]), "=r"(r[1]), "=r"(r[2]), "=r"(r[3]), "=r"(r[4]), "=r"(r[5]), "=r"(r[6]), "=r"(r[7]), "=r"(r[8]),
        "=r"(r[9]), "=r"(r[10]), "=r"(r[11]), "=r"(r[12]), "=r"(r[13]), "=r"(r[14]), "=r"(r[15])
      : "r"(taddr));
}
__device__ __forceinline__ void tmem_ld_wait16(uint32_t* r) {
  asm volatile("tcgen05.wait::ld.sync.aligned;"
               : "+r"(r[0]), "+r"(r[1]), "+r"(r[2]), "+r"(r[3]), "+r"(r[4]), "+r"(r[5]), "+r"(r[6]), "+r"(r[7]), "+r"(r[8]),
                 "+r"(r[9]), "+r"(r[10]), "+r"(r[11]), "+r"(r[12]), "+r"(r[13]), "+r"(r[14]), "+r"(r[15])
               :: "memory");
}

constexpr uint32_t kPeerBitMask = 0xFEFFFFFFu;
__device__ __forceinline__ void tma_load_2d_2sm(void* smem_dst, const CUtensorMap* m, uint64_t* leader_bar, int c0, int c1) {
  asm volatile(
      "cp.async.bulk.tensor.2d.cta_group::2.shared::cluster.global.mbarrier::complete_tx::bytes [%0], [%1, {%3, %4}], [%2];"
      ::"r"(smem_u32(smem_dst)), "l"(reinterpret_cast<uint64_t>(m)), "r"(smem_u32(leader_bar) & kPeerBitMask), "r"(c0), "r"(c1)
      : "memory");
}
__device__ __forceinline__ void tma_load_3d_2sm(void* smem_dst, const CUtensorMap* m, uint64_t* leader_bar, int c0, int c1,
                                                int c2) {
  asm volatile(
      "cp.async.bulk.tensor.3d.cta_group::2.shared::cluster.global.mbarrier::complete_tx::bytes [%0], [%1, {%3, %4, %5}], [%2];"
      ::"r"(smem_u32(smem_dst)), "l"(reinterpret_cast<uint64_t>(m)), "r"(smem_u32(leader_bar) & kPeerBitMask), "r"(c0), "r"(c1),
        "r"(c2)
      : "memory");
}
__device__ __forceinline__ void mbar_arrive_leader(uint64_t* bar) {
  asm volatile("mbarrier.arrive.shared::cluster.b64 _, [%0];" ::"r"(smem_u32(bar) & kPeerBitMask) : "memory");
}
__device__ __forceinline__ void tmem_alloc_2sm(uint32_t* smem_result, uint32_t ncols) {
  asm volatile("tcgen05.alloc.cta_group::2.sync.aligned.shared::cta.b32 [%0], %1;" ::"r"(smem_u32(smem_result)),
               "r"(ncols)
               : "memory");
}
__device__ __forceinline__ void tmem_relinquish_2sm() {
  asm volatile("tcgen05.relinquish_alloc_permit.cta_group::2.sync.aligned;" ::: "memory");
}
__device__ __forceinline__ void tmem_dealloc_2sm(uint32_t taddr, uint32_t ncols) {
  asm volatile("tcgen05.dealloc.cta_group::2.sync.aligned.b32 %0, %1;" ::"r"(taddr), "r"(ncols) : "memory");
}
__device__ __forceinline__ void mma_bf16_ss_2sm(uint32_t d_tmem, uint64_t adesc, uint64_t bdesc, uint32_t idesc,
                                                uint32_t accumulate) {
  asm volatile(
      "{\n\t.reg .pred p;\n\tsetp.ne.b32 p, %4, 0;\n\t"
      "tcgen05.mma.cta_group::2.kind::f16 [%0], %1, %2, %3, p;\n\t}\n"
      ::"r"(d_tmem), "l"(adesc), "l"(bdesc), "r"(idesc), "r"(accumulate)
      : "memory");
}
__device__ __forceinline__ void mma_commit_2sm(uint64_t* bar) {
  asm volatile("tcgen05.commit.cta_group::2.mbarrier::arrive::one.shared::cluster.multicast::cluster.b64 [%0], %1;"
               ::"r"(smem_u32(bar)), "h"((uint16_t)3)
               : "memory");
}

__device__ __forceinline__ uint64_t umma_desc_sw128(uint32_t smem_addr, uint32_t lbo_bytes, uint32_t sbo_bytes) {
  return (uint64_t)((smem_addr >> 4) & 0x3FFFu) | ((uint64_t)((lbo_bytes >> 4) & 0x3FFFu) << 16) |
         ((uint64_t)((sbo_bytes >> 4) & 0x3FFFu) << 32) | (1ull << 46) | (2ull << 61);
}
__host__ __device__ constexpr uint32_t umma_idesc_bf16(int M, int N, bool a_mn_major, bool b_mn_major, bool f16 = false) {
  return (1u << 4) | (f16 ? 0u : ((1u << 7) | (1u << 10))) | ((a_mn_major ? 1u : 0u) << 15) |
         ((b_mn_major ? 1u : 0u) << 16) | ((uint32_t)(N >> 3) << 17) | ((uint32_t)(M >> 4) << 24);
}

}
}
```

### betrayed-by-captions_b200/csrc/tc_state.h

```cpp
#pragma once
#include "gemm_tc.h"
#include <cuda.h>
#include <cuda_bf16.h>
#include <string>

namespace cgg {

typedef CUresult (*EncodeTiledFn)(CUtensorMap*, CUtensorMapDataType, cuuint32_t, void*, const cuuint64_t*,
                                  const cuuint64_t*, const cuuint32_t*, const cuuint32_t*, CUtensorMapInterleave,
                                  CUtensorMapSwizzle, CUtensorMapL2promotion, CUtensorMapFloatOOBfill);


struct TcState {
  cgg_config cfg;
  std::string err;
  EncodeTiledFn encode = nullptr;
  int num_sms = 0, cta_cap = 0;
  int H4 = 0, W4 = 0, lh[3] = {0, 0, 0}, lw[3] = {0, 0, 0}, nl[3] = {0, 0, 0};
  __nv_bfloat16* wkv[3] = {nullptr, nullptr, nullptr};
  __nv_bfloat16* rk[3] = {nullptr, nullptr, nullptr};
  const float* bkv[3] = {nullptr, nullptr, nullptr};
  int q_pad = 0, ein_ntile = 0, ein_calls_per_tile = 0, bits_ntile = 0, bits_nt = 0;
  int rows_per_batch = 0;
  struct LayerW {
    __nv_bfloat16 *wq_c = nullptr, *wo_c = nullptr, *wqkv_s = nullptr, *wo_s = nullptr, *w1 = nullptr, *w2 = nullptr;
    float* rowbias_v = nullptr;
  } pl[CGG_MAX_LAYERS];
  __nv_bfloat16 *wh = nullptr, *wme1 = nullptr, *wme2 = nullptr;
  float* bias_h = nullptr;
  int nh_padded = 0;
  bool packed_alloc = false;
  bool smem_attr_set = false, attn_attr_set = false;
  bool attr_kv_pair = false, attr_bits = false, attr_ein_t = false, attr_ein_pair = false;
  uint8_t* live_buf = nullptr;
  size_t live_bytes = 0;
  void free_all() {
    for (int l = 0; l < 3; ++l) { cudaFree(wkv[l]); cudaFree(rk[l]); wkv[l] = rk[l] = nullptr; }
  }
  void free_packed() {
    for (int i = 0; i < CGG_MAX_LAYERS; ++i) {
      cudaFree(pl[i].wq_c); cudaFree(pl[i].wo_c); cudaFree(pl[i].wqkv_s); cudaFree(pl[i].wo_s); cudaFree(pl[i].w1);
      cudaFree(pl[i].w2); cudaFree(pl[i].rowbias_v);
      pl[i] = LayerW();
    }
    cudaFree(wh); cudaFree(wme1); cudaFree(wme2); cudaFree(bias_h);
    wh = wme1 = wme2 = nullptr; bias_h = nullptr; packed_alloc = false;
  }
};


inline int pitch8(int k) { return (k + 7) & ~7; }

struct TcWs {
  size_t me_all, fds[3], memp[3], xqb, xb, ob, fb, zb, h1b, h2b, qf, qs, kvs, x1, x2, t1, total;
  void carve(const TcState* t, int B) {
    size_t off = 0;
    auto take = [&](size_t b) { size_t o = off; off += (b + 255) & ~(size_t)255; return o; };
    const int C = t->cfg.embed_dim;
    const size_t M = (size_t)B * t->cfg.num_queries;
    me_all = take((size_t)B * t->rows_per_batch * 2 * C * 2 + 128 * 1024);
    for (int l = 0; l < 3; ++l) fds[l] = take((size_t)B * C * pitch8(t->lh[l] * t->lw[l]) * 2);
    for (int l = 0; l < 3; ++l) {
      const int K = t->lh[l] * t->lw[l];
      memp[l] = take((K % 8) ? (size_t)B * C * pitch8(K) * 2 : 0);
    }
    xqb = take(M * C * 2); xb = take(M * C * 2); ob = take(M * C * 2);
    fb = take(M * t->cfg.ffn_dim * 2);
    zb = take(M * 2 * C * 2); h1b = take(M * 2 * C * 2); h2b = take(M * 2 * C * 2);
    qf = take(M * C * 4); qs = take(M * C * 4); kvs = take(M * 2 * C * 4);
    x1 = take(M * C * 4); x2 = take(M * C * 4); t1 = take(4 * M * C * 4);
    total = off;
  }
};

int tc_pack_weights(TcState* t, const cgg_weights* w, cudaStream_t s);

inline int tc_fail(TcState* t, int code, const std::string& m) { t->err = m; return code; }

#define TCU(call)                                                                                  \
  do {                                                                                             \
    cudaError_t e__ = (call);                                                                      \
    if (e__ != cudaSuccess) return tc_fail(t, CGG_ERR_CUDA, std::string(#call) + ": " + cudaGetErrorString(e__)); \
  } while (0)

}
```

### betrayed-by-captions_b200/lib.py

```python
import ctypes as C
import os

HERE = os.path.dirname(os.path.abspath(__file__))
LIB_PATH = os.environ.get('CGG_LIB', os.path.join(HERE, 'libcgg_b200.so'))

MAX_LAYERS = 16
NUM_LEVELS = 3
FP32, BF16 = 0, 1
c_float_p = C.POINTER(C.c_float)

EXPORTS = ['cgg_create', 'cgg_destroy', 'cgg_last_error', 'cgg_version', 'cgg_launch_count', 'cgg_prepare', 'cgg_workspace_bytes', 'cgg_workspace_offset',
           'cgg_decoder_forward', 'cgg_kv_project', 'cgg_head_call', 'cgg_attn_mask_from_logits',
           'cgg_decoder_layer', 'cgg_mask_einsum', 'cgg_masked_attention', 'cgg_noun_embeddings', 'cgg_similarity',
           'cgg_grounding_scratch_bytes', 'cgg_grounding_loss', 'cgg_grounding_bwd_scratch_bytes',
           'cgg_grounding_loss_backward', 'cgg_set_final_mask_only',
           'cgg_gemm_f32', 'cgg_layernorm', 'cgg_layernorm_bwd_scratch_bytes', 'cgg_layernorm_backward', 'cgg_relu_backward',
           'cgg_axpy', 'cgg_add_rows', 'cgg_sum_batch', 'cgg_colsum', 'cgg_mem_prep', 'cgg_mem_prep_backward', 'cgg_sine_pos',
           'cgg_attention_f32', 'cgg_attention_backward', 'cgg_attn_softmax_rows', 'cgg_attn_dscore', 'cgg_point_sample', 'cgg_point_sample_backward',
           'cgg_matching_cost', 'cgg_point_losses', 'cgg_point_losses_backward', 'cgg_weighted_ce', 'cgg_weighted_ce_backward',
           'cgg_upsample_masks', 'cgg_instance_mask_stats', 'cgg_softmax_rows', 'cgg_panoptic_scratch_bytes',
           'cgg_panoptic_fuse',
           'cgg_ms_deform_attn', 'cgg_ms_deform_attn_backward', 'cgg_group_norm_scratch_bytes', 'cgg_group_norm_tokens',
           'cgg_group_norm_tokens_backward', 'cgg_upsample_add_tokens', 'cgg_upsample_add_tokens_backward',
           'cgg_tokens_to_nchw', 'cgg_nchw_to_tokens']


class Config(C.Structure):
    _fields_ = [(n, C.c_int) for n in ('num_queries', 'embed_dim', 'num_heads', 'ffn_dim', 'num_layers',
                                       'num_classes_p1', 'd_lang', 'precision', 'pred_emb_norm')]


class LayerWeights(C.Structure):
    _fields_ = [(n, C.c_void_p) for n in ('cross_in_w', 'cross_in_b', 'cross_out_w', 'cross_out_b', 'self_in_w',
                                          'self_in_b', 'self_out_w', 'self_out_b', 'ffn_w1', 'ffn_b1', 'ffn_w2',
                                          'ffn_b2')] + [('norm_w', C.c_void_p * 3), ('norm_b', C.c_void_p * 3)]


class Weights(C.Structure):
    _fields_ = [(n, C.c_void_p) for n in ('query_embed', 'query_feat', 'level_embed', 'cls_w', 'cls_b')] + \
               [('me_w', C.c_void_p * 3), ('me_b', C.c_void_p * 3)] + \
               [(n, C.c_void_p) for n in ('v2l_w', 'v2l_b', 'post_norm_w', 'post_norm_b')] + \
               [('layers', LayerWeights * MAX_LAYERS)]


class GemmDesc(C.Structure):
    _fields_ = [('A', C.c_void_p), ('sAb', C.c_long), ('sAm', C.c_long), ('sAk', C.c_long),
                ('A2', C.c_void_p), ('sA2m', C.c_long), ('sA2k', C.c_long), ('a2_mod', C.c_int),
                ('W', C.c_void_p), ('sWb', C.c_long), ('sWn', C.c_long), ('sWk', C.c_long),
                ('bias', C.c_void_p),
                ('R', C.c_void_p), ('sRb', C.c_long), ('sRm', C.c_long), ('sRn', C.c_long), ('r_mod', C.c_int),
                ('r_ncols', C.c_int),
                ('C', C.c_void_p), ('sCb', C.c_long), ('sCm', C.c_long), ('sCn', C.c_long),
                ('M', C.c_int), ('N', C.c_int), ('K', C.c_int), ('batch', C.c_int),
                ('relu', C.c_int), ('alpha', C.c_float), ('a_mmajor', C.c_int), ('c_mmajor', C.c_int), ('tf32', C.c_int),
                ('batch_inner', C.c_int), ('sAb2', C.c_long), ('sWb2', C.c_long), ('sCb2', C.c_long), ('accumulate', C.c_int), ('slot', C.c_int), ('conv_cin', C.c_int)]


class CggError(RuntimeError):
    pass


_lib = None


def load():
    global _lib
    if _lib is not None:
        return _lib
    if not os.path.exists(LIB_PATH):
        raise CggError('%s not found: build it with `python -m cgg_b200.build` '
                       '(there is no fallback path)' % LIB_PATH)
    lib = C.CDLL(LIB_PATH)
    vp, i, sz = C.c_void_p, C.c_int, C.c_size_t
    lib.cgg_create.argtypes = [C.POINTER(vp), C.POINTER(Config)]
    lib.cgg_destroy.argtypes = [vp]
    lib.cgg_destroy.restype = None
    lib.cgg_last_error.argtypes = [vp]
    lib.cgg_last_error.restype = C.c_char_p
    lib.cgg_version.restype = C.c_char_p
    lib.cgg_launch_count.restype = C.c_uint64
    lib.cgg_prepare.argtypes = [vp, C.POINTER(Weights), i, i, C.POINTER(i), C.POINTER(i), vp]
    lib.cgg_workspace_bytes.argtypes = [vp, i]
    lib.cgg_workspace_bytes.restype = sz
    lib.cgg_workspace_offset.argtypes = [vp, i, C.c_char_p]
    lib.cgg_workspace_offset.restype = sz
    lib.cgg_decoder_forward.argtypes = [vp, C.POINTER(Weights), i, vp, C.POINTER(vp), vp, vp, vp, vp,
                                        C.POINTER(vp), vp, vp, sz, vp]
    lib.cgg_kv_project.argtypes = [vp, C.POINTER(Weights), i, C.POINTER(vp), vp, sz, vp]
    lib.cgg_head_call.argtypes = [vp, C.POINTER(Weights), i, vp, vp, i, vp, vp, vp, vp, vp, vp, vp, sz, vp]
    lib.cgg_mask_einsum.argtypes = [vp, i, i, i, vp, vp, vp, sz, vp]
    lib.cgg_attn_mask_from_logits.argtypes = [vp, i, vp, i, i, i, i, vp, vp, vp]
    lib.cgg_decoder_layer.argtypes = [vp, C.POINTER(Weights), i, i, vp, vp, vp, vp, vp, sz, vp]
    lib.cgg_masked_attention.argtypes = [vp, i, i, vp, vp, vp, C.c_long, C.c_long, vp, vp, vp, vp]
    lib.cgg_noun_embeddings.argtypes = [vp, vp, vp, vp, vp, i, i, C.c_float, i, vp, vp]
    lib.cgg_similarity.argtypes = [vp, vp, vp, i, i, i, C.c_float, vp, vp]
    lib.cgg_grounding_scratch_bytes.argtypes = [i, i, i]
    lib.cgg_grounding_scratch_bytes.restype = sz
    lib.cgg_grounding_loss.argtypes = [vp, vp, vp, vp, i, i, i, i, C.c_float, C.c_float, vp, vp, sz, vp]
    lib.cgg_set_final_mask_only.argtypes = [vp, i]
    lib.cgg_grounding_bwd_scratch_bytes.argtypes = [i, i, i]
    lib.cgg_grounding_bwd_scratch_bytes.restype = sz
    lib.cgg_grounding_loss_backward.argtypes = [vp, vp, vp, vp, i, i, i, i, C.c_float, C.c_float, C.c_float, vp, vp, sz, vp]
    f32, lg = C.c_float, C.c_long
    lib.cgg_gemm_f32.argtypes = [vp, C.POINTER(GemmDesc), vp]
    lib.cgg_layernorm.argtypes = [vp, vp, vp, vp, vp, i, i, f32, vp]
    lib.cgg_layernorm_bwd_scratch_bytes.argtypes = [i, i]
    lib.cgg_layernorm_bwd_scratch_bytes.restype = sz
    lib.cgg_layernorm_backward.argtypes = [vp, vp, vp, vp, vp, vp, vp, vp, sz, i, i, f32, vp]
    lib.cgg_relu_backward.argtypes = [vp, vp, vp, vp, lg, f32, vp]
    lib.cgg_axpy.argtypes = [vp, vp, vp, lg, f32, vp]
    lib.cgg_add_rows.argtypes = [vp, vp, vp, vp, i, lg, vp]
    lib.cgg_sum_batch.argtypes = [vp, vp, vp, i, lg, vp]
    lib.cgg_colsum.argtypes = [vp, vp, vp, lg, i, f32, i, vp]
    lib.cgg_mem_prep.argtypes = [vp, vp, vp, vp, vp, vp, i, i, i, vp]
    lib.cgg_mem_prep_backward.argtypes = [vp, vp, vp, vp, i, i, i, vp]
    lib.cgg_sine_pos.argtypes = [vp, vp, i, i, i, vp]
    lib.cgg_attention_f32.argtypes = [vp, i, i, i, vp, vp, vp, lg, lg, vp, vp, vp, vp]
    lib.cgg_attention_backward.argtypes = [vp, i, i, i, vp, vp, vp, lg, lg, vp, vp, vp, vp, vp, vp, vp, lg, lg, vp, vp]
    lib.cgg_attn_softmax_rows.argtypes = [vp, vp, vp, vp, i, i, i, i, vp]
    lib.cgg_attn_dscore.argtypes = [vp, vp, vp, vp, vp, i, i, i, i, i, vp]
    f = C.c_float
    lib.cgg_point_sample.argtypes = [vp, vp, vp, vp, i, i, i, i, i, vp]
    lib.cgg_point_sample_backward.argtypes = [vp, vp, vp, vp, i, i, i, i, i, vp]
    lib.cgg_matching_cost.argtypes = [vp, vp, vp, vp, vp, vp, i, i, i, i, f, f, f, f, f, vp, vp, vp]
    lib.cgg_point_losses.argtypes = [vp, vp, vp, i, i, f, vp, vp, vp, vp]
    lib.cgg_point_losses_backward.argtypes = [vp, vp, vp, vp, i, i, f, vp, vp, vp, vp]
    lib.cgg_weighted_ce.argtypes = [vp, vp, vp, vp, i, i, vp, vp, vp, vp]
    lib.cgg_weighted_ce_backward.argtypes = [vp, vp, vp, vp, vp, i, i, vp, vp, vp]
    lib.cgg_upsample_masks.argtypes = [vp, vp, i, vp, i, i, i, i, i, vp]
    lib.cgg_instance_mask_stats.argtypes = [vp, vp, i, vp, i, i, i, i, i, i, i, i, vp, vp, vp, vp, vp]
    lib.cgg_softmax_rows.argtypes = [vp, vp, i, i, vp]
    lib.cgg_panoptic_scratch_bytes.argtypes = [i, i]
    lib.cgg_panoptic_scratch_bytes.restype = sz
    dbl = C.c_double
    lib.cgg_panoptic_fuse.argtypes = [vp, vp, i, vp, vp, i, i, i, i, i, i, i, i, i, i, dbl, dbl, i, vp, vp, vp, vp, vp, sz, vp]
    ip = C.POINTER(C.c_int)
    lib.cgg_ms_deform_attn.argtypes = [vp, vp, lg, vp, lg, vp, lg, vp, i, i, i, i, i, ip, ip, vp]
    lib.cgg_ms_deform_attn_backward.argtypes = [vp, vp, vp, vp, vp, vp, vp, vp, i, i, i, i, i, ip, ip, vp]
    lib.cgg_group_norm_scratch_bytes.argtypes = [i, i, i, i]
    lib.cgg_group_norm_scratch_bytes.restype = sz
    lib.cgg_group_norm_tokens.argtypes = [vp, vp, vp, vp, vp, vp, vp, sz, i, i, i, i, f32, i, vp]
    lib.cgg_group_norm_tokens_backward.argtypes = [vp, vp, vp, vp, vp, vp, vp, vp, vp, sz, i, i, i, i, vp]
    lib.cgg_upsample_add_tokens.argtypes = [vp, vp, vp, lg, vp, i, i, i, i, i, i, vp]
    lib.cgg_upsample_add_tokens_backward.argtypes = [vp, vp, vp, i, i, i, i, i, i, vp]
    lib.cgg_tokens_to_nchw.argtypes = [vp, vp, lg, vp, i, i, i, i, vp]
    lib.cgg_nchw_to_tokens.argtypes = [vp, vp, vp, lg, i, i, i, i, vp]
    for name in EXPORTS:
        fn = getattr(lib, name)
        if fn.restype is C.c_int and name not in ('cgg_destroy',):
            fn.restype = C.c_int
    _lib = lib
    return lib


STATUS = {0: 'CGG_OK', -1: 'CGG_ERR_BAD_SHAPE', -2: 'CGG_ERR_UNSUPPORTED', -3: 'CGG_ERR_CUDA',
          -4: 'CGG_ERR_NOT_PREPARED', -5: 'CGG_ERR_WORKSPACE', -6: 'CGG_ERR_NULL'}


def check(status, handle=None, what=''):
    if status != 0:
        msg = ''
        if handle:
            msg = load().cgg_last_error(handle).decode()
        raise CggError('%s failed: %s %s' % (what, STATUS.get(status, status), msg))


class no_gc_during_capture:

    def __enter__(self):
        import gc
        self._was = gc.isenabled()
        gc.collect()
        gc.disable()
        return self

    def __exit__(self, *exc):
        import gc
        if self._was:
            gc.enable()
        return False
```

### include/cgg_b200.h

```cpp
#ifndef CGG_B200_H
#define CGG_B200_H

#include <stddef.h>
#include <stdint.h>

#ifdef __cplusplus
extern "C" {
#endif

#define CGG_MAX_LAYERS 16
#define CGG_NUM_LEVELS 3

typedef enum {
  CGG_OK = 0,
  CGG_ERR_BAD_SHAPE = -1,
  CGG_ERR_UNSUPPORTED = -2,
  CGG_ERR_CUDA = -3,
  CGG_ERR_NOT_PREPARED = -4,
  CGG_ERR_WORKSPACE = -5,
  CGG_ERR_NULL = -6
} cgg_status;

typedef enum {
  CGG_FP32 = 0,
  CGG_BF16 = 1
} cgg_precision;

typedef struct {
  int num_queries;
  int embed_dim;
  int num_heads;
  int ffn_dim;
  int num_layers;
  int num_classes_p1;
  int d_lang;
  int precision;
  int pred_emb_norm;
} cgg_config;

typedef struct {
  const float *cross_in_w, *cross_in_b;
  const float *cross_out_w, *cross_out_b;
  const float *self_in_w, *self_in_b;
  const float *self_out_w, *self_out_b;
  const float *ffn_w1, *ffn_b1;
  const float *ffn_w2, *ffn_b2;
  const float *norm_w[3], *norm_b[3];
} cgg_layer_weights;

typedef struct {
  const float *query_embed;
  const float *query_feat;
  const float *level_embed;
  const float *cls_w, *cls_b;
  const float *me_w[3], *me_b[3];
  const float *v2l_w, *v2l_b;
  const float *post_norm_w, *post_norm_b;
  cgg_layer_weights layers[CGG_MAX_LAYERS];
} cgg_weights;

typedef struct cgg_handle cgg_handle;

int cgg_create(cgg_handle **out, const cgg_config *cfg);
void cgg_destroy(cgg_handle *h);
const char *cgg_last_error(const cgg_handle *h);
const char *cgg_version(void);
uint64_t cgg_launch_count(void);

int cgg_prepare(cgg_handle *h, const cgg_weights *w, int H4, int W4,
                const int level_h[CGG_NUM_LEVELS], const int level_w[CGG_NUM_LEVELS],
                void *stream);

size_t cgg_workspace_bytes(const cgg_handle *h, int batch);
size_t cgg_workspace_offset(const cgg_handle *h, int batch, const char *what);

int cgg_decoder_forward(cgg_handle *h, const cgg_weights *w, int batch,
                        const void *mask_features, const void *const memories[CGG_NUM_LEVELS],
                        float *cls, float *emb, void *mask,
                        float *x_states, uint32_t *const *bitmaps, uint8_t *all_masked,
                        void *workspace, size_t workspace_bytes, void *stream);


int cgg_kv_project(cgg_handle *h, const cgg_weights *w, int batch,
                   const void *const memories[CGG_NUM_LEVELS], void *workspace,
                   size_t workspace_bytes, void *stream);

int cgg_head_call(cgg_handle *h, const cgg_weights *w, int batch, const float *x,
                  const void *mask_features, int target_level, float *cls, float *emb,
                  void *mask, float *mask_embed_out, uint32_t *bitmap, uint8_t *all_masked,
                  void *workspace, size_t workspace_bytes, void *stream);

int cgg_mask_einsum(cgg_handle *h, int batch, int first_call, int num_calls, const void *mask_features,
                    void *mask, void *workspace, size_t workspace_bytes, void *stream);

int cgg_attn_mask_from_logits(cgg_handle *h, int batch, const float *mask_pred, int H4, int W4,
                              int th, int tw, uint32_t *bitmap, uint8_t *all_masked, void *stream);

int cgg_decoder_layer(cgg_handle *h, const cgg_weights *w, int batch, int layer,
                      const float *x_in, const uint32_t *bitmap, const uint8_t *all_masked,
                      float *x_out, void *workspace, size_t workspace_bytes, void *stream);

int cgg_masked_attention(cgg_handle *h, int batch, int num_keys, const float *q, const void *k,
                         const void *v, long kv_stride, long kv_batch_stride,
                         const uint32_t *bitmap, const uint8_t *all_masked,
                         float *out, void *stream);


int cgg_noun_embeddings(cgg_handle *h, const float *table, const float *ln_w, const float *ln_b,
                        const int64_t *ids, int n_ids, int d_lang, float eps, int text_emb_norm,
                        float *out, void *stream);

int cgg_similarity(cgg_handle *h, const float *a, const float *b, int M, int N, int D,
                   float scale, float *out, void *stream);

size_t cgg_grounding_scratch_bytes(int Bg, int Q, int T);
int cgg_grounding_loss(cgg_handle *h, const float *pred, const float *cap, const int64_t *cap_mask,
                       int Bg, int Q, int T, int D, float temperature, float loss_weight,
                       float *loss, void *scratch, size_t scratch_bytes, void *stream);

int cgg_set_final_mask_only(cgg_handle *h, int on);

size_t cgg_grounding_bwd_scratch_bytes(int Bg, int Q, int T);
int cgg_grounding_loss_backward(cgg_handle *h, const float *pred, const float *cap, const int64_t *cap_mask,
                                int Bg, int Q, int T, int D, float temperature, float loss_weight, float grad_out,
                                float *dpred, void *scratch, size_t scratch_bytes, void *stream);


typedef struct {
  const float *A; long sAb, sAm, sAk;
  const float *A2; long sA2m, sA2k; int a2_mod;
  const float *W; long sWb, sWn, sWk;
  const float *bias;
  const float *R; long sRb, sRm, sRn; int r_mod; int r_ncols;
  float *C; long sCb, sCm, sCn;
  int M, N, K, batch;
  int relu;
  float alpha;
  int a_mmajor, c_mmajor;
  int tf32;
  int batch_inner;
  long sAb2, sWb2, sCb2;
  int accumulate;
  int slot;
  int conv_cin;
} cgg_gemm_desc;
int cgg_gemm_f32(cgg_handle *h, const cgg_gemm_desc *d, void *stream);

int cgg_layernorm(cgg_handle *h, const float *x, const float *w, const float *b, float *y, int rows, int n, float eps,
                  void *stream);
size_t cgg_layernorm_bwd_scratch_bytes(int rows, int n);
int cgg_layernorm_backward(cgg_handle *h, const float *x, const float *w, const float *dy, float *dx, float *dw,
                           float *db, void *scratch, size_t scratch_bytes, int rows, int n, float eps, void *stream);
int cgg_relu_backward(cgg_handle *h, const float *y, const float *dy, float *dx, long n, float alpha, void *stream);
int cgg_axpy(cgg_handle *h, const float *in, float *out, long n, float alpha, void *stream);
int cgg_add_rows(cgg_handle *h, const float *x, const float *add, float *out, int batch, long per, void *stream);
int cgg_sum_batch(cgg_handle *h, const float *g, float *out, int batch, long per, void *stream);
int cgg_colsum(cgg_handle *h, const float *g, float *out, long rows, int n, float alpha, int accumulate, void *stream);
int cgg_mem_prep(cgg_handle *h, const float *mem, const float *level, const float *pos_level, float *key_in,
                 float *val_in, int batch, int C, int K, void *stream);
int cgg_mem_prep_backward(cgg_handle *h, const float *dkey_in, const float *dval_in, float *dmem, int batch, int C,
                          int K, void *stream);
int cgg_sine_pos(cgg_handle *h, float *out, int hh, int ww, int C, void *stream);
int cgg_attention_f32(cgg_handle *h, int batch, int num_q, int num_keys, const float *q, const float *k, const float *v,
                      long kv_stride, long kv_batch_stride, const uint32_t *bitmap, const uint8_t *all_masked,
                      float *out, void *stream);
int cgg_attention_backward(cgg_handle *h, int batch, int num_q, int num_keys, const float *q, const float *k,
                           const float *v, long kv_stride, long kv_batch_stride, const uint32_t *bitmap,
                           const uint8_t *all_masked, const float *out, const float *dout, float *dq, float *dk,
                           float *dv, long dkv_stride, long dkv_batch_stride, float *scratch, void *stream);
int cgg_attn_softmax_rows(cgg_handle *h, float *scores, const uint32_t *bitmap, const uint8_t *all_masked, int batch,
                          int heads, int num_q, int num_keys, void *stream);
int cgg_attn_dscore(cgg_handle *h, const float *probs, float *dprobs, const float *out, const float *dout, int batch,
                    int heads, int head_dim, int num_q, int num_keys, void *stream);


int cgg_point_sample(cgg_handle *h, const float *in, const float *coords, float *out, int planes, int hh, int ww,
                     int num_points, int coords_shared, void *stream);
int cgg_point_sample_backward(cgg_handle *h, const float *dout, const float *coords, float *din, int planes, int hh, int ww,
                              int num_points, int coords_shared, void *stream);
int cgg_matching_cost(cgg_handle *h, const float *mask_points, const float *gt_points, const float *cls_scores,
                      const float *cls_emb_logits, const int64_t *gt_labels, int num_q, int num_gt, int classes_p1,
                      int num_points, float w_cls, float w_cls_emb, float w_mask, float w_dice, float dice_eps,
                      float *scratch, float *cost, void *stream);
int cgg_point_losses(cgg_handle *h, const float *pred_points, const float *target_points, int rows, int num_points,
                     float dice_eps, float *abc, float *dice_rows, float *bce_rows, void *stream);
int cgg_point_losses_backward(cgg_handle *h, const float *pred_points, const float *target_points, const float *abc,
                              int rows, int num_points, float dice_eps, const float *g_dice_rows, const float *g_bce_rows,
                              float *dpred, void *stream);
int cgg_weighted_ce(cgg_handle *h, const float *logits, const int64_t *labels, const float *class_weight, int rows,
                    int classes_p1, float *row_loss, float *row_weight, float *lse, void *stream);
int cgg_weighted_ce_backward(cgg_handle *h, const float *logits, const int64_t *labels, const float *class_weight,
                             const float *lse, int rows, int classes_p1, const float *g_rows, float *dlogits, void *stream);

int cgg_upsample_masks(cgg_handle *h, const void *logits, int is_bf16, float *out, int planes, int h4, int w4, int up_h,
                       int up_w, void *stream);
int cgg_instance_mask_stats(cgg_handle *h, const void *logits, int is_bf16, const int *geom, int batch, int num_q, int h4,
                            int w4, int up_h, int up_w, int max_out_h, int max_out_w, uint32_t *bits, int *count,
                            float *sig_sum, int *bbox, void *stream);
int cgg_softmax_rows(cgg_handle *h, float *x, int rows, int n, void *stream);
size_t cgg_panoptic_scratch_bytes(int batch, int num_q);
int cgg_panoptic_fuse(cgg_handle *h, const void *logits, int is_bf16, const float *probs, const int *geom, int batch,
                      int num_q, int classes_p1, int num_things, int h4, int w4, int up_h, int up_w, int max_out_h,
                      int max_out_w, double object_mask_thr, double iou_thr, int filter_low_score, int *pan,
                      int *mask_area, int *original_area, int *seg_value, void *scratch, size_t scratch_bytes,
                      void *stream);

int cgg_ms_deform_attn(cgg_handle *h, const float *value, long value_stride, const float *offsets, long offset_stride,
                       const float *weight_logits, long logit_stride, float *out, int batch, int tokens, int heads,
                       int levels, int points, const int *level_h, const int *level_w, void *stream);
int cgg_ms_deform_attn_backward(cgg_handle *h, const float *value, const float *offsets, const float *weight_logits,
                                const float *dout, float *dvalue, float *doffsets, float *dweight_logits, int batch,
                                int tokens, int heads, int levels, int points, const int *level_h, const int *level_w,
                                void *stream);
size_t cgg_group_norm_scratch_bytes(int batch, int pixels, int channels, int groups);
int cgg_group_norm_tokens(cgg_handle *h, const float *x, const float *gamma, const float *beta, float *y, float *mean_rstd,
                          void *scratch, size_t scratch_bytes, int batch, int pixels, int channels, int groups, float eps,
                          int relu, void *stream);
int cgg_group_norm_tokens_backward(cgg_handle *h, const float *x, const float *dy, const float *mean_rstd,
                                   const float *gamma, float *dx, float *dgamma, float *dbeta, void *scratch,
                                   size_t scratch_bytes, int batch, int pixels, int channels, int groups, void *stream);
int cgg_upsample_add_tokens(cgg_handle *h, const float *lateral, const float *coarse, long coarse_batch_stride, float *out,
                            int batch, int H, int W, int ch, int cw, int channels, void *stream);
int cgg_upsample_add_tokens_backward(cgg_handle *h, const float *dout, float *dcoarse, int batch, int H, int W, int ch,
                                     int cw, int channels, void *stream);
int cgg_tokens_to_nchw(cgg_handle *h, const float *tokens, long token_batch_stride, void *out, int out_bf16, int batch,
                       int pixels, int channels, void *stream);
int cgg_nchw_to_tokens(cgg_handle *h, const float *in, float *tokens, long token_batch_stride, int batch, int pixels,
                       int channels, int accumulate, void *stream);

#ifdef __cplusplus
}
#endif
#endif
```

Measured before the change: 6725.

## Fuse output projections and FFN with residual LayerNorm via cluster DSMEM reduction

Adds a layer_ln_kernel that runs the attention out-projection (or the full FFN: W1+ReLU kept in shared memory, then W2) on tensor cores and performs bias, residual add and LayerNorm in the same kernel. Thread-block clusters exchange partial accumulators through distributed shared memory instead of writing fp32 partials to global memory. This replaces separate linear launches, the split-K fp32 partial buffer and the LN kernels in the decoder layer, cutting launches and global round trips. It risks low occupancy (one CTA per SM, small grids at modest M) and adds cluster synchronisation overhead; the FFN hidden is stored as fp16.

Result: no change. 6768, median of 6 (+0.6%).

```diff
diff --git a/betrayed-by-captions_b200/csrc/api.cu b/betrayed-by-captions_b200/csrc/api.cu
--- a/betrayed-by-captions_b200/csrc/api.cu
+++ b/betrayed-by-captions_b200/csrc/api.cu
@@ -2,6 +2,7 @@
 #include "kernels.h"
 #include "gemm_tc.h"
 #include "gemm_tf32.h"
+#include "ln_row.cuh"
 #include "tc_state.h"
 
 #include <math.h>
@@ -397,6 +398,22 @@
   return CGG_OK;
 }
 
+extern "C" int cgg_linear_ln(cgg_handle* h, int rows, const void* X, const void* W, const float* bias, const void* W1,
+                             const float* b1, const float* res, const float* ln_w, const float* ln_b, float* out_f32,
+                             void* out_h, void* out_hq, const float* qe, void* out_hl, const float* w2, const float* b2,
+                             void* stream) {
+  if (!h || !X || !W || !bias || !res || !ln_w || !ln_b || (W1 && !b1) || (out_hq && !qe)) return CGG_ERR_NULL;
+  if (h->cfg.precision != CGG_BF16) return fail(h, CGG_ERR_UNSUPPORTED, "cgg_linear_ln is a CGG_BF16 stage");
+  if (rows < 0) return fail(h, CGG_ERR_BAD_SHAPE, "bad row count");
+  typedef __nv_bfloat16 hb;
+  const LnRowOut o = {ln_w, ln_b, out_f32, static_cast<hb*>(out_h), static_cast<hb*>(out_hq), qe, h->cfg.num_queries,
+                      static_cast<hb*>(out_hl), w2, b2};
+  int st = tc_linear_ln(h->tc, static_cast<const hb*>(X), rows, static_cast<const hb*>(W), bias, static_cast<const hb*>(W1), b1,
+                        h->cfg.ffn_dim, res, o, (cudaStream_t)stream);
+  if (st != CGG_OK) return fail(h, st, std::string("tc_linear_ln: ") + tc_last_error(h->tc));
+  return CGG_OK;
+}
+
 static int decoder_layer_impl(cgg_handle* h, const cgg_weights* w, int batch, int layer, const float* x_in,
                               const uint32_t* bitmap, const uint8_t* all_masked, float* x_out, void* workspace,
                               size_t workspace_bytes, void* stream, bool chained_in, bool chained_out,
diff --git a/betrayed-by-captions_b200/csrc/gemm_tc.cu b/betrayed-by-captions_b200/csrc/gemm_tc.cu
--- a/betrayed-by-captions_b200/csrc/gemm_tc.cu
+++ b/betrayed-by-captions_b200/csrc/gemm_tc.cu
@@ -1,5 +1,6 @@
 #include "gemm_tc.h"
 #include "kernels.h"
+#include "ln_row.cuh"
 #include <cuda_fp16.h>
 #include "tc_ptx.cuh"
 #include "tc_state.h"
@@ -30,7 +31,6 @@
   int b_kcoord[12];
   int split_cpc, split_K;
   TcSeg seg[3]; int nseg; const float* lin_bias; int n_tokens;
-  long kpart_stride;
   int b_row0;
   int b_rows_per_batch;
   int acc_stride;
@@ -226,10 +226,6 @@
       }
     }
     if (on && p.lin_bias) bias = __ldg(p.lin_bias + m);
-    if (blockIdx.z > 0) {
-      bias = 0.f; res = nullptr; rowbias = nullptr;
-      ptr = static_cast<float*>(ptr) + (long)blockIdx.z * p.kpart_stride;
-    }
   }
 };
 
@@ -382,11 +378,11 @@
   auto kcoords = [&](int kc, int& ka, int& kb) {
     if (p.split_cpc > 0) {
       const int term = kc / p.split_cpc, j = kc - term * p.split_cpc;
-      const int k0 = ((int)blockIdx.z * p.split_cpc + j) * TC_BK;
+      const int k0 = j * TC_BK;
       ka = (term == 2 ? p.split_K : 0) + k0;
       kb = (term == 1 ? p.split_K : 0) + k0;
     } else if (p.k_identity) {
-      ka = kb = ((int)blockIdx.z * p.KC + kc) * TC_BK;
+      ka = kb = kc * TC_BK;
     } else {
       ka = p.a_kcoord[kc]; kb = p.b_kcoord[kc];
     }
@@ -1243,7 +1239,7 @@
 }
 
 int launch_tc_gemm(TcState* t, const CUtensorMap& mA, const CUtensorMap& mB, TcGemmP p, int m_tiles, int batch,
-                   cudaStream_t s, const CUtensorMap* mC = nullptr, int kparts = 1) {
+                   cudaStream_t s, const CUtensorMap* mC = nullptr) {
   if (p.N_TILE % 16 != 0 || p.N_TILE < 16 || p.N_TILE > 256) return tc_fail(t, CGG_ERR_BAD_SHAPE, "bad N tile");
   p.acc_stride = p.N_TILE <= 128 ? 128 : 256;
   if (p.N_TILE <= 32) p.acc_stride = 32; else if (p.N_TILE <= 64) p.acc_stride = 64;
@@ -1275,7 +1271,7 @@
   p.dbg = timing ? 1 : 0;
   cudaEvent_t e0 = nullptr, e1 = nullptr;
   if (timing) { cudaEventCreate(&e0); cudaEventCreate(&e1); cudaStreamSynchronize(s); cudaEventRecord(e0, s); }
-  dim3 grid(m_tiles, batch, kparts);
+  dim3 grid(m_tiles, batch);
   const dim3 block(TC_THREADS);
   p.m_tiles = m_tiles; p.n_batch = batch; p.n_work = m_tiles * batch;
   if (want_res) {
@@ -1740,10 +1736,7 @@
 }
 
 int tc_linear(TcState* t, const __nv_bfloat16* A, int M, int K, const __nv_bfloat16* W, int n_padded, const float* bias,
-              const TcSeg* segs, int nsegs, cudaStream_t s, bool split_k, int kparts, long kpart_stride, bool f16) {
-  if (kparts < 1) kparts = 1;
-  if (kparts > 1 && (nsegs != 1 || segs[0].is_bf16 || segs[0].relu || (K / TC_BK) % kparts != 0))
-    return tc_fail(t, CGG_ERR_BAD_SHAPE, "K-parts need one plain fp32 output segment");
+              const TcSeg* segs, int nsegs, cudaStream_t s, bool split_k, bool f16) {
   if (K % TC_BK != 0 || n_padded % TC_BM != 0 || nsegs < 1 || nsegs > 3)
     return tc_fail(t, CGG_ERR_BAD_SHAPE, "tc_linear shape (features must be padded to 128)");
   for (int i = 0; i < nsegs; ++i)
@@ -1758,17 +1751,243 @@
   if (st != CGG_OK) return st;
   st = make_map_B(t, &mX, A, M, row_len, p.N_TILE);
   if (st != CGG_OK) return st;
-  p.NT = 1; p.KC = K / TC_BK / kparts; p.kpart_stride = kpart_stride;
+  p.NT = 1; p.KC = K / TC_BK;
   p.a_kmajor = 1; p.k_identity = 1; p.a_resident = 0;
   if (split_k) {
-    p.k_identity = 0; p.split_cpc = K / TC_BK / kparts; p.split_K = K; p.KC = 3 * p.split_cpc;
+    p.k_identity = 0; p.split_cpc = K / TC_BK; p.split_K = K; p.KC = 3 * p.split_cpc;
   }
   p.b_row0 = 0; p.b_rows_per_batch = p.N_TILE;
   p.epi = EPI_LINEAR_T; p.M_valid = n_padded; p.n_tokens = M;
   p.f16 = f16 ? 1 : 0;
   p.nseg = nsegs; p.lin_bias = bias;
   for (int i = 0; i < nsegs; ++i) p.seg[i] = segs[i];
-  return launch_tc_gemm(t, mW, mX, p, n_padded / TC_BM, n_tok_tiles, s, nullptr, kparts);
-}
-
-}
+  return launch_tc_gemm(t, mW, mX, p, n_padded / TC_BM, n_tok_tiles, s);
+}
+
+namespace {
+constexpr int LN_X_CHUNK = 128 * 128;
+constexpr int LN_W_CHUNK = 256 * 128;
+constexpr int LN_RECV_LD = 260;
+constexpr int LN_RING = 4 * LN_W_CHUNK;
+constexpr int LN_RECV = 128 * LN_RECV_LD * 4;
+constexpr int LN_OUT_G = 4;
+constexpr size_t LN_SMEM = 1024 + 4 * LN_X_CHUNK + (LN_RECV > LN_RING ? LN_RECV : LN_RING) + 256;
+
+struct LayerLnP {
+  int M;
+  const float* bias;
+  const float* b1;
+  const float* res;
+  LnRowOut o;
+};
+
+template <bool FFN>
+__global__ void __launch_bounds__(TC_THREADS, 1)
+layer_ln_kernel(const __grid_constant__ CUtensorMap tmX, const __grid_constant__ CUtensorMap tmW1,
+                const __grid_constant__ CUtensorMap tmW, const __grid_constant__ LayerLnP p) {
+  extern __shared__ uint8_t smem_raw[];
+  uint8_t* smem = reinterpret_cast<uint8_t*>((reinterpret_cast<uintptr_t>(smem_raw) + 1023) & ~(uintptr_t)1023);
+  uint8_t* sX = smem;
+  uint8_t* sW = sX + 4 * LN_X_CHUNK;
+  float* recv = reinterpret_cast<float*>(sW);
+  uint64_t* bars = reinterpret_cast<uint64_t*>(sW + (LN_RECV > LN_RING ? LN_RECV : LN_RING));
+  uint64_t* x_full = bars;
+  uint64_t* w_full = bars + 4;
+  uint64_t* w_empty = bars + 8;
+  uint64_t* d_full = bars + 12;
+  uint64_t* h_full = bars + 13;
+  uint32_t* tmem_slot = reinterpret_cast<uint32_t*>(bars + 14);
+
+  const int warp = threadIdx.x >> 5, lane = threadIdx.x & 31;
+  const int G = gridDim.x, rank = (int)ptx::cluster_ctarank(), tile = blockIdx.y;
+  const int rows_per = TC_BM / G;
+  const int ncols = FFN ? 256 : 256 / G;
+  if (warp == 0 && lane == 0) {
+    ptx::prefetch_tmap(&tmX);
+    ptx::prefetch_tmap(&tmW);
+    if (FFN) ptx::prefetch_tmap(&tmW1);
+    for (int i = 0; i < 4; ++i) { ptx::mbar_init(&x_full[i], 1); ptx::mbar_init(&w_full[i], 1); ptx::mbar_init(&w_empty[i], 1); }
+    ptx::mbar_init(d_full, 1);
+    ptx::mbar_init(h_full, EPI_WARPS);
+    ptx::fence_mbar_init();
+  }
+  if (warp == 1) {
+    ptx::tmem_alloc(tmem_slot, 256);
+    ptx::tmem_relinquish();
+  }
+  ptx::tc_fence_before();
+  __syncthreads();
+  ptx::tc_fence_after();
+  const uint32_t tmem_base = *tmem_slot;
+  ptx::grid_dep_launch();
+  if (warp == 0 && lane == 0)
+    for (int kc = 0; kc < 4; ++kc) {
+      ptx::mbar_expect_tx(&w_full[kc], (uint32_t)(ncols * 128));
+      ptx::tma_load_2d(sW + kc * LN_W_CHUNK, FFN ? &tmW1 : &tmW, &w_full[kc], kc * TC_BK, rank * ncols);
+    }
+  ptx::grid_dep_wait();
+
+  if (warp == 0) {
+    if (lane == 0) {
+      for (int kc = 0; kc < 4; ++kc) {
+        ptx::mbar_expect_tx(&x_full[kc], (uint32_t)LN_X_CHUNK);
+        ptx::tma_load_2d(sX + kc * LN_X_CHUNK, &tmX, &x_full[kc], kc * TC_BK, tile * TC_BM);
+      }
+      if (FFN)
+        for (int kc = 0; kc < 4; ++kc) {
+          ptx::mbar_wait(&w_empty[kc], 0);
+          ptx::mbar_expect_tx(&w_full[kc], (uint32_t)LN_W_CHUNK);
+          ptx::tma_load_2d(sW + kc * LN_W_CHUNK, &tmW, &w_full[kc], rank * 256 + kc * TC_BK, 0);
+        }
+    }
+    __syncwarp();
+  } else if (warp == 1) {
+    const uint32_t idesc = ptx::umma_idesc_bf16(TC_BM, ncols, false, false, true);
+    const uint64_t xd0 = ptx::umma_desc_sw128(ptx::smem_u32(sX), 16, 1024);
+    const uint64_t wd0 = ptx::umma_desc_sw128(ptx::smem_u32(sW), 16, 1024);
+    auto gemm = [&](uint32_t w_phase, bool wait_x) {
+      for (int kc = 0; kc < 4; ++kc) {
+        if (wait_x) ptx::mbar_wait(&x_full[kc], 0);
+        ptx::mbar_wait(&w_full[kc], w_phase);
+        ptx::tc_fence_after();
+        if (ptx::elect_one()) {
+          const uint64_t xd = xd0 + (uint64_t)(kc * (LN_X_CHUNK >> 4)), wd = wd0 + (uint64_t)(kc * (LN_W_CHUNK >> 4));
+#pragma unroll
+          for (int k = 0; k < TC_BK / 16; ++k)
+            ptx::mma_bf16_ss(tmem_base, xd + (uint64_t)(k * 2), wd + (uint64_t)(k * 2), idesc, (kc | k) != 0 ? 1u : 0u);
+          if (FFN && w_phase == 0) ptx::mma_commit(&w_empty[kc]);
+          if (kc == 3) ptx::mma_commit(d_full);
+        }
+        __syncwarp();
+      }
+    };
+    gemm(0, true);
+    if (FFN) {
+      ptx::mbar_wait(h_full, 0);
+      ptx::tc_fence_after();
+      gemm(1, false);
+    }
+  } else {
+    const int quarter = warp & 3, part = (warp - 2) >> 2;
+    const int m = quarter * 32 + lane;
+    const uint32_t taddr = tmem_base + ((uint32_t)(quarter * 32) << 16) + (uint32_t)(part * 64);
+    ptx::mbar_wait(d_full, 0);
+    ptx::tc_fence_after();
+    if (FFN) {
+      const float* b1 = p.b1 + rank * 256 + part * 64;
+      uint8_t* row = sX + part * LN_X_CHUNK + m * 128;
+#pragma unroll
+      for (int j = 0; j < 4; ++j) {
+        float v[16];
+        ptx::tmem_ld16(taddr + (uint32_t)(j * 16), v);
+        uint32_t h[8];
+#pragma unroll
+        for (int i = 0; i < 8; ++i) {
+          const __half2 h2 = __floats2half2_rn(fmaxf(v[2 * i] + __ldg(b1 + j * 16 + 2 * i), 0.f),
+                                               fmaxf(v[2 * i + 1] + __ldg(b1 + j * 16 + 2 * i + 1), 0.f));
+          h[i] = *reinterpret_cast<const uint32_t*>(&h2);
+        }
+        *reinterpret_cast<uint4*>(row + (((2 * j) ^ (m & 7)) << 4)) = make_uint4(h[0], h[1], h[2], h[3]);
+        *reinterpret_cast<uint4*>(row + (((2 * j + 1) ^ (m & 7)) << 4)) = make_uint4(h[4], h[5], h[6], h[7]);
+      }
+      ptx::fence_proxy_async_smem();
+      ptx::tc_fence_before();
+      __syncwarp();
+      if (lane == 0) ptx::mbar_arrive(h_full);
+      ptx::mbar_wait(d_full, 1);
+      ptx::tc_fence_after();
+    }
+  }
+  const int n0 = lane * 8;
+  const long row0 = (long)tile * TC_BM + rank * rows_per + (warp - 2);
+  float4 res_a = make_float4(0.f, 0.f, 0.f, 0.f), res_c = res_a;
+  if (warp >= 2 && warp - 2 < rows_per && row0 < p.M) {
+    const float4* rp = reinterpret_cast<const float4*>(p.res + row0 * 256 + n0);
+    res_a = rp[0]; res_c = rp[1];
+  }
+  ptx::cluster_sync_all();
+  if (warp >= 2) {
+    const int quarter = warp & 3, part = (warp - 2) >> 2;
+    const int m = quarter * 32 + lane;
+    const int pcols = ncols / 4;
+    const uint32_t taddr = tmem_base + ((uint32_t)(quarter * 32) << 16) + (uint32_t)(part * pcols);
+    const int owner = m / rows_per;
+    const int drow = (FFN ? rank * rows_per : 0) + m - owner * rows_per, dcol = (FFN ? 0 : rank * ncols) + part * pcols;
+    const uint32_t dst = ptx::dsmem_map(ptx::smem_u32(recv + ((long)drow * LN_RECV_LD + dcol)), (uint32_t)owner);
+    for (int j = 0; j < pcols / 16; ++j) {
+      float v[16];
+      ptx::tmem_ld16(taddr + (uint32_t)(j * 16), v);
+#pragma unroll
+      for (int i = 0; i < 4; ++i)
+        ptx::dsmem_st4(dst + (uint32_t)((j * 16 + i * 4) * 4), v[4 * i], v[4 * i + 1], v[4 * i + 2], v[4 * i + 3]);
+    }
+  }
+  ptx::cluster_sync_all();
+  if (warp >= 2) {
+    const int slots = FFN ? G : 1;
+    for (int r = warp - 2; r < rows_per; r += EPI_WARPS) {
+      const long row = (long)tile * TC_BM + rank * rows_per + r;
+      if (row >= p.M) break;
+      float v[8];
+      const float4* s0 = reinterpret_cast<const float4*>(recv + (long)r * LN_RECV_LD + n0);
+      float4 a = s0[0], c = s0[1];
+      v[0] = a.x; v[1] = a.y; v[2] = a.z; v[3] = a.w; v[4] = c.x; v[5] = c.y; v[6] = c.z; v[7] = c.w;
+      for (int g = 1; g < slots; ++g) {
+        const float4* sg = reinterpret_cast<const float4*>(recv + ((long)g * rows_per + r) * LN_RECV_LD + n0);
+        a = sg[0]; c = sg[1];
+        v[0] += a.x; v[1] += a.y; v[2] += a.z; v[3] += a.w; v[4] += c.x; v[5] += c.y; v[6] += c.z; v[7] += c.w;
+      }
+      if (r == warp - 2) {
+        a = res_a; c = res_c;
+      } else {
+        const float4* rp = reinterpret_cast<const float4*>(p.res + row * 256 + n0);
+        a = rp[0]; c = rp[1];
+      }
+      const float rs[8] = {a.x, a.y, a.z, a.w, c.x, c.y, c.z, c.w};
+#pragma unroll
+      for (int i = 0; i < 8; ++i) v[i] = (v[i] + __ldg(p.bias + n0 + i)) + rs[i];
+      ln_row_store(v, row, lane, p.o);
+    }
+  }
+  ptx::tc_fence_before();
+  __syncthreads();
+  if (warp == 1) {
+    __syncwarp();
+    ptx::tmem_dealloc(tmem_base, 256);
+  }
+}
+}
+
+int tc_linear_ln(TcState* t, const __nv_bfloat16* X, int M, const __nv_bfloat16* W, const float* bias,
+                 const __nv_bfloat16* W1, const float* b1, int F, const float* res, const LnRowOut& out, cudaStream_t s) {
+  if (t->cfg.embed_dim != 256) return tc_fail(t, CGG_ERR_UNSUPPORTED, "tc_linear_ln needs embed_dim 256");
+  const bool ffn = W1 != nullptr;
+  const int G = ffn ? F / 256 : LN_OUT_G;
+  if (ffn && (F % 256 != 0 || (G != 1 && G != 2 && G != 4 && G != 8)))
+    return tc_fail(t, CGG_ERR_UNSUPPORTED, "the bf16 FFN needs ffn_dim in {256, 512, 1024, 2048}");
+  if (M < 1) return CGG_OK;
+  CUtensorMap mX, mW1, mW;
+  int st = make_map_B(t, &mX, X, M, 256, TC_BM);
+  if (st != CGG_OK) return st;
+  st = make_map_B(t, &mW, W, 256, ffn ? F : 256, ffn ? 256 : 256 / G);
+  if (st != CGG_OK) return st;
+  if (ffn) {
+    st = make_map_B(t, &mW1, W1, F, 256, 256);
+    if (st != CGG_OK) return st;
+  }
+  if (!t->attr_layer_ln) {
+    TCU(cudaFuncSetAttribute(layer_ln_kernel<false>, cudaFuncAttributeMaxDynamicSharedMemorySize, (int)LN_SMEM));
+    TCU(cudaFuncSetAttribute(layer_ln_kernel<true>, cudaFuncAttributeMaxDynamicSharedMemorySize, (int)LN_SMEM));
+    t->attr_layer_ln = true;
+  }
+  LayerLnP p;
+  p.M = M; p.bias = bias; p.b1 = b1; p.res = res; p.o = out;
+  const dim3 grid(G, (M + TC_BM - 1) / TC_BM), block(TC_THREADS);
+  if (ffn) TCU(launch_pdl_cluster(G, layer_ln_kernel<true>, grid, block, LN_SMEM, s, mX, mW1, mW, p));
+  else TCU(launch_pdl_cluster(G, layer_ln_kernel<false>, grid, block, LN_SMEM, s, mX, mX, mW, p));
+  count_launch();
+  TCU(cudaGetLastError());
+  return CGG_OK;
+}
+
+}
diff --git a/betrayed-by-captions_b200/csrc/gemm_tc.h b/betrayed-by-captions_b200/csrc/gemm_tc.h
--- a/betrayed-by-captions_b200/csrc/gemm_tc.h
+++ b/betrayed-by-captions_b200/csrc/gemm_tc.h
@@ -43,8 +43,11 @@
                    void* mask_bf16, long call_stride, void* ws, cudaStream_t s);
 
 int tc_linear(TcState* t, const __nv_bfloat16* A, int M, int K, const __nv_bfloat16* W, int n_padded, const float* bias,
-              const TcSeg* segs, int nsegs, cudaStream_t s, bool split_k = false, int kparts = 1, long kpart_stride = 0,
+              const TcSeg* segs, int nsegs, cudaStream_t s, bool split_k = false,
               bool f16 = false);
+struct LnRowOut;
+int tc_linear_ln(TcState* t, const __nv_bfloat16* X, int M, const __nv_bfloat16* W, const float* bias,
+                 const __nv_bfloat16* W1, const float* b1, int F, const float* res, const LnRowOut& out, cudaStream_t s);
 int tc_decoder_layer(TcState* t, const cgg_weights* w, int batch, int layer, const float* x_in, const void* k,
                      const void* v, long kv_stride, long kv_bstride, int num_keys, const uint32_t* bitmap,
                      const uint8_t* all_masked, float* x_out, void* ws, cudaStream_t s, bool chained_in = false,
diff --git a/betrayed-by-captions_b200/csrc/ln_row.cuh b/betrayed-by-captions_b200/csrc/ln_row.cuh
--- /dev/null
+++ b/betrayed-by-captions_b200/csrc/ln_row.cuh
@@ -0,0 +1,80 @@
+#pragma once
+#include <cuda_bf16.h>
+#include <cuda_fp16.h>
+#include <stdint.h>
+
+namespace cgg {
+
+struct LnRowOut {
+  const float *w, *b;
+  float* f32;
+  __nv_bfloat16 *h, *hq;
+  const float* qe; int Q;
+  __nv_bfloat16* hl;
+  const float *w2, *b2;
+};
+
+__device__ __forceinline__ void split_pack(float a, float b, uint32_t& hi, uint32_t& lo) {
+  const __nv_bfloat162 h = __floats2bfloat162_rn(a, b);
+  const float2 back = __bfloat1622float2(h);
+  const __nv_bfloat162 l = __floats2bfloat162_rn(a - back.x, b - back.y);
+  hi = *reinterpret_cast<const uint32_t*>(&h);
+  lo = *reinterpret_cast<const uint32_t*>(&l);
+}
+
+__device__ __forceinline__ void ln_warp_row(float (&v)[8], int n0, const float* __restrict__ w, const float* __restrict__ b) {
+  float s = 0.f;
+#pragma unroll
+  for (int i = 0; i < 8; ++i) s += v[i];
+#pragma unroll
+  for (int o = 16; o > 0; o >>= 1) s += __shfl_xor_sync(0xffffffffu, s, o);
+  const float mu = s * (1.0f / 256.0f);
+  float q = 0.f;
+#pragma unroll
+  for (int i = 0; i < 8; ++i) { const float d = v[i] - mu; q = fmaf(d, d, q); }
+#pragma unroll
+  for (int o = 16; o > 0; o >>= 1) q += __shfl_xor_sync(0xffffffffu, q, o);
+  const float rstd = 1.0f / sqrtf(q * (1.0f / 256.0f) + 1e-5f);
+#pragma unroll
+  for (int i = 0; i < 8; ++i) v[i] = (v[i] - mu) * rstd * __ldg(w + n0 + i) + __ldg(b + n0 + i);
+}
+
+__device__ __forceinline__ void ln_row_store(float (&v)[8], long row, int lane, const LnRowOut& o) {
+  const int n0 = lane * 8;
+  ln_warp_row(v, n0, o.w, o.b);
+  if (o.f32) {
+    float4* d = reinterpret_cast<float4*>(o.f32 + row * 256 + n0);
+    d[0] = make_float4(v[0], v[1], v[2], v[3]);
+    d[1] = make_float4(v[4], v[5], v[6], v[7]);
+  }
+  auto store_h = [&](__nv_bfloat16* dst, const float* v8) {
+    uint4 pk;
+    uint32_t* w = reinterpret_cast<uint32_t*>(&pk);
+#pragma unroll
+    for (int i = 0; i < 4; ++i) {
+      const __half2 h2 = __floats2half2_rn(v8[2 * i], v8[2 * i + 1]);
+      w[i] = *reinterpret_cast<const uint32_t*>(&h2);
+    }
+    *reinterpret_cast<uint4*>(dst + row * 256 + n0) = pk;
+  };
+  if (o.h) store_h(o.h, v);
+  if (o.hq) {
+    const float* e = o.qe + (long)(row % o.Q) * 256 + n0;
+    float yq[8];
+#pragma unroll
+    for (int i = 0; i < 8; ++i) yq[i] = v[i] + e[i];
+    store_h(o.hq, yq);
+  }
+  if (o.hl) {
+    if (o.w2) ln_warp_row(v, n0, o.w2, o.b2);
+    uint4 ph, pl;
+    split_pack(v[0], v[1], ph.x, pl.x);
+    split_pack(v[2], v[3], ph.y, pl.y);
+    split_pack(v[4], v[5], ph.z, pl.z);
+    split_pack(v[6], v[7], ph.w, pl.w);
+    *reinterpret_cast<uint4*>(o.hl + row * 512 + n0) = ph;
+    *reinterpret_cast<uint4*>(o.hl + row * 512 + 256 + n0) = pl;
+  }
+}
+
+}
diff --git a/betrayed-by-captions_b200/csrc/path_bf16.cu b/betrayed-by-captions_b200/csrc/path_bf16.cu
--- a/betrayed-by-captions_b200/csrc/path_bf16.cu
+++ b/betrayed-by-captions_b200/csrc/path_bf16.cu
@@ -1,5 +1,6 @@
 #include "gemm_tc.h"
 #include "kernels.h"
+#include "ln_row.cuh"
 #include "tc_ptx.cuh"
 #include "tc_state.h"
 #include <cuda_fp16.h>
@@ -12,14 +13,6 @@
 namespace {
 
 inline int round_up(int x, int m) { return (x + m - 1) / m * m; }
-
-__device__ __forceinline__ void split_pack(float a, float b, uint32_t& hi, uint32_t& lo) {
-  const __nv_bfloat162 h = __floats2bfloat162_rn(a, b);
-  const float2 back = __bfloat1622float2(h);
-  const __nv_bfloat162 l = __floats2bfloat162_rn(a - back.x, b - back.y);
-  hi = *reinterpret_cast<const uint32_t*>(&h);
-  lo = *reinterpret_cast<const uint32_t*>(&l);
-}
 
 __global__ void add_qe_cast_kernel(const float* __restrict__ x, const float* __restrict__ qe,
                                    __nv_bfloat16* __restrict__ dst, long total, int per ) {
@@ -36,101 +29,15 @@
   *reinterpret_cast<uint2*>(dst + i) = pk;
 }
 
-__global__ void __launch_bounds__(256) ln_rows_kernel(const float* __restrict__ x, int nparts, long part_stride,
-                                                      const float* __restrict__ w,
-                                                      const float* __restrict__ b, int rows, float* __restrict__ out_f32,
-                                                      __nv_bfloat16* __restrict__ out_bf16,
-                                                      __nv_bfloat16* __restrict__ out_bf16_q,
-                                                      const float* __restrict__ qe, int Q,
-                                                      __nv_bfloat16* __restrict__ out_hl,
-                                                      const float* __restrict__ w2, const float* __restrict__ b2) {
+__global__ void __launch_bounds__(256) ln_rows_kernel(const float* __restrict__ x, int rows, const LnRowOut o) {
   ptx::grid_dep_launch();
   ptx::grid_dep_wait();
   const int row = blockIdx.x * 8 + (threadIdx.x >> 5), lane = threadIdx.x & 31;
   if (row >= rows) return;
-  const int n0 = lane * 8;
-  const float4* xr = reinterpret_cast<const float4*>(x + (long)row * 256 + n0);
+  const float4* xr = reinterpret_cast<const float4*>(x + (long)row * 256 + lane * 8);
   const float4 a = xr[0], c = xr[1];
   float v[8] = {a.x, a.y, a.z, a.w, c.x, c.y, c.z, c.w};
-  for (int pt = 1; pt < nparts; ++pt) {
-    const float4* xp = reinterpret_cast<const float4*>(x + pt * part_stride + (long)row * 256 + n0);
-    const float4 e = xp[0], f = xp[1];
-    v[0] += e.x; v[1] += e.y; v[2] += e.z; v[3] += e.w; v[4] += f.x; v[5] += f.y; v[6] += f.z; v[7] += f.w;
-  }
-  float s = 0.f;
-#pragma unroll
-  for (int i = 0; i < 8; ++i) s += v[i];
-#pragma unroll
-  for (int o = 16; o > 0; o >>= 1) s += __shfl_xor_sync(0xffffffffu, s, o);
-  const float mu = s * (1.0f / 256.0f);
-  float q = 0.f;
-#pragma unroll
-  for (int i = 0; i < 8; ++i) { const float d = v[i] - mu; q = fmaf(d, d, q); }
-#pragma unroll
-  for (int o = 16; o > 0; o >>= 1) q += __shfl_xor_sync(0xffffffffu, q, o);
-  const float rstd = 1.0f / sqrtf(q * (1.0f / 256.0f) + 1e-5f);
-  float y[8];
-#pragma unroll
-  for (int i = 0; i < 8; ++i) y[i] = (v[i] - mu) * rstd * __ldg(w + n0 + i) + __ldg(b + n0 + i);
-  if (out_f32) {
-    float4* d = reinterpret_cast<float4*>(out_f32 + (long)row * 256 + n0);
-    d[0] = make_float4(y[0], y[1], y[2], y[3]);
-    d[1] = make_float4(y[4], y[5], y[6], y[7]);
-  }
-  auto store_hl = [&](__nv_bfloat16* dst, const float* v8) {
-    uint4 ph, pl;
-    split_pack(v8[0], v8[1], ph.x, pl.x);
-    split_pack(v8[2], v8[3], ph.y, pl.y);
-    split_pack(v8[4], v8[5], ph.z, pl.z);
-    split_pack(v8[6], v8[7], ph.w, pl.w);
-    *reinterpret_cast<uint4*>(dst + (long)row * 512 + n0) = ph;
-    *reinterpret_cast<uint4*>(dst + (long)row * 512 + 256 + n0) = pl;
-  };
-  auto store_h = [&](__nv_bfloat16* dst, const float* v8) {
-    uint4 pk;
-    uint32_t* w = reinterpret_cast<uint32_t*>(&pk);
-#pragma unroll
-    for (int i = 0; i < 4; ++i) {
-      const __half2 h2 = __floats2half2_rn(v8[2 * i], v8[2 * i + 1]);
-      w[i] = *reinterpret_cast<const uint32_t*>(&h2);
-    }
-    *reinterpret_cast<uint4*>(dst + (long)row * 256 + n0) = pk;
-  };
-  if (out_bf16) store_h(out_bf16, y);
-  if (out_bf16_q) {
-    const float* e = qe + (long)(row % Q) * 256 + n0;
-    float yq[8];
-#pragma unroll
-    for (int i = 0; i < 8; ++i) yq[i] = y[i] + e[i];
-    store_h(out_bf16_q, yq);
-  }
-  if (out_hl && w2) {
-    float s2 = 0.f;
-#pragma unroll
-    for (int i = 0; i < 8; ++i) s2 += y[i];
-#pragma unroll
-    for (int o = 16; o > 0; o >>= 1) s2 += __shfl_xor_sync(0xffffffffu, s2, o);
-    const float mu2 = s2 * (1.0f / 256.0f);
-    float q2 = 0.f;
-#pragma unroll
-    for (int i = 0; i < 8; ++i) { const float d = y[i] - mu2; q2 = fmaf(d, d, q2); }
-#pragma unroll
-    for (int o = 16; o > 0; o >>= 1) q2 += __shfl_xor_sync(0xffffffffu, q2, o);
-    const float rstd2 = 1.0f / sqrtf(q2 * (1.0f / 256.0f) + 1e-5f);
-#pragma unroll
-    for (int i = 0; i < 8; ++i) y[i] = (y[i] - mu2) * rstd2 * __ldg(w2 + n0 + i) + __ldg(b2 + n0 + i);
-  }
-  if (out_hl) store_hl(out_hl, y);
-}
-
-cudaError_t launch_ln_rows(const float* x, const float* w, const float* b, int rows, float* out_f32,
-                           __nv_bfloat16* out_bf16, __nv_bfloat16* out_bf16_q, const float* qe, int Q,
-                           __nv_bfloat16* out_hl, cudaStream_t s, const float* w2 = nullptr, const float* b2 = nullptr,
-                           int nparts = 1, long part_stride = 0) {
-  cudaError_t e = launch_pdl(ln_rows_kernel, dim3((rows + 7) / 8), dim3(256), 0, s, x, nparts, part_stride, w, b, rows, out_f32, out_bf16, out_bf16_q,
-                             qe, Q > 0 ? Q : 1, out_hl, w2, b2);
-  count_launch();
-  return e != cudaSuccess ? e : cudaGetLastError();
+  ln_row_store(v, row, lane, o);
 }
 
 template <typename T>
@@ -225,7 +132,12 @@
   __nv_bfloat16* zb = at<__nv_bfloat16>(ws, o.zb);
   __nv_bfloat16* h1b = at<__nv_bfloat16>(ws, o.h1b);
   __nv_bfloat16* h2b = at<__nv_bfloat16>(ws, o.h2b);
-  if (!z_ready) TCU(launch_ln_rows(x, w->post_norm_w, w->post_norm_b, M, nullptr, nullptr, nullptr, nullptr, 0, zb, s));
+  if (!z_ready) {
+    const LnRowOut lo = {w->post_norm_w, w->post_norm_b, nullptr, nullptr, nullptr, nullptr, 1, zb, nullptr, nullptr};
+    TCU(launch_pdl(ln_rows_kernel, dim3((M + 7) / 8), dim3(256), 0, s, x, M, lo));
+    count_launch();
+    TCU(cudaGetLastError());
+  }
   TcSeg sh[3] = {seg(0, c.d_lang, emb, c.d_lang, false, false),
                  seg(c.d_lang, C, h1b, 2 * C, true, true, 1.f, nullptr, 1, 0, true),
                  seg(c.d_lang + C, c.num_classes_p1, cls, c.num_classes_p1, false, false)};
@@ -255,13 +167,11 @@
   __nv_bfloat16* xqb = at<__nv_bfloat16>(ws, o.xqb);
   __nv_bfloat16* xb = at<__nv_bfloat16>(ws, o.xb);
   __nv_bfloat16* ob = at<__nv_bfloat16>(ws, o.ob);
-  __nv_bfloat16* fb = at<__nv_bfloat16>(ws, o.fb);
   float* qf = at<float>(ws, o.qf);
   float* qs = at<float>(ws, o.qs);
   float* kvs = at<float>(ws, o.kvs);
   float* x1 = at<float>(ws, o.x1);
   float* x2 = at<float>(ws, o.x2);
-  float* t1 = at<float>(ws, o.t1);
   const long total = (long)M * C;
   if (!chained_in) {
     TCU(launch_pdl(add_qe_cast_kernel, dim3((unsigned)((total / 4 + 255) / 256)), dim3(256), 0, s, x_in, w->query_embed, xqb,
@@ -271,7 +181,7 @@
   }
   if (!q_ready) {
     TcSeg sq[1] = {seg(0, C, qf, C, false, false, qscale)};
-    TST(tc_linear(t, xqb, M, C, pw.wq_c, C, lw.cross_in_b, sq, 1, s, false, 1, 0, true));
+    TST(tc_linear(t, xqb, M, C, pw.wq_c, C, lw.cross_in_b, sq, 1, s, false, true));
   }
   {
     const int level = layer % CGG_NUM_LEVELS, slot = layer / CGG_NUM_LEVELS;
@@ -280,31 +190,22 @@
     TST(tc_attention(t, batch, num_keys, qf, k, v, kv_stride, kv_bstride, bitmap, all_masked, nullptr, ob, s, rtab, rcols,
                      slot * C,  2));
   }
-  TcSeg so[1] = {seg(0, C, t1, C, false, false, 1.f, nullptr, 1, 0, false, x_in, C)};
-  TST(tc_linear(t, ob, M, C, pw.wo_c, C, lw.cross_out_b, so, 1, s, false, 1, 0, true));
-  TCU(launch_ln_rows(t1, lw.norm_w[0], lw.norm_b[0], M, x1, nullptr, xqb, w->query_embed, Q, nullptr, s));
+  const LnRowOut o1 = {lw.norm_w[0], lw.norm_b[0], x1, nullptr, xqb, w->query_embed, Q, nullptr, nullptr, nullptr};
+  TST(tc_linear_ln(t, ob, M, pw.wo_c, lw.cross_out_b, nullptr, nullptr, 0, x_in, o1, s));
   __nv_bfloat16* kvb = reinterpret_cast<__nv_bfloat16*>(kvs);
   TcSeg sk[3] = {seg(0, C, qs, C, false, false, qscale), seg(C, C, kvb, 2 * C, true, false),
                  seg(2 * C, C, kvb + C, 2 * C, true, false, 1.f, pw.rowbias_v, Q, C)};
-  TST(tc_linear(t, xqb, M, C, pw.wqkv_s, 3 * C, lw.self_in_b, sk, 3, s, false, 1, 0, true));
+  TST(tc_linear(t, xqb, M, C, pw.wqkv_s, 3 * C, lw.self_in_b, sk, 3, s, false, true));
   TST(tc_attention(t, batch, Q, qs, kvb, kvb + C, 2 * C, (long)Q * 2 * C, nullptr, nullptr, nullptr, ob, s, nullptr, 0, 0,
                     2));
-  TcSeg so2[1] = {seg(0, C, t1, C, false, false, 1.f, nullptr, 1, 0, false, x1, C)};
-  TST(tc_linear(t, ob, M, C, pw.wo_s, C, lw.self_out_b, so2, 1, s, false, 1, 0, true));
-  TCU(launch_ln_rows(t1, lw.norm_w[1], lw.norm_b[1], M, x2, xb, nullptr, nullptr, 0, nullptr, s));
-  TcSeg sf[1] = {seg(0, F, fb, F, true, true)};
-  sf[0].is_bf16 = 3;
-  TST(tc_linear(t, xb, M, C, pw.w1, F, lw.ffn_b1, sf, 1, s, false, 1, 0, true));
-  TcSeg sf2[1] = {seg(0, C, t1, C, false, false, 1.f, nullptr, 1, 0, false, x2, C)};
-  const int kparts = (F / 64) % 4 == 0 ? 4 : 1;
-  const long pstride = (long)M * C;
-  TST(tc_linear(t, fb, M, F, pw.w2, C, lw.ffn_b2, sf2, 1, s, false, kparts, pstride, true));
-  if (chained_out)
-    TCU(launch_ln_rows(t1, lw.norm_w[2], lw.norm_b[2], M, x_out, nullptr, xqb, w->query_embed, Q, at<__nv_bfloat16>(ws, o.zb), s,
-                       w->post_norm_w, w->post_norm_b, kparts, pstride));
-  else
-    TCU(launch_ln_rows(t1, lw.norm_w[2], lw.norm_b[2], M, x_out, nullptr, nullptr, nullptr, 0, nullptr, s, nullptr, nullptr,
-                       kparts, pstride));
+  const LnRowOut o2 = {lw.norm_w[1], lw.norm_b[1], x2, xb, nullptr, nullptr, 1, nullptr, nullptr, nullptr};
+  TST(tc_linear_ln(t, ob, M, pw.wo_s, lw.self_out_b, nullptr, nullptr, 0, x1, o2, s));
+  LnRowOut o3 = {lw.norm_w[2], lw.norm_b[2], x_out, nullptr, nullptr, nullptr, 1, nullptr, nullptr, nullptr};
+  if (chained_out) {
+    o3.hq = xqb; o3.qe = w->query_embed; o3.Q = Q;
+    o3.hl = at<__nv_bfloat16>(ws, o.zb); o3.w2 = w->post_norm_w; o3.b2 = w->post_norm_b;
+  }
+  TST(tc_linear_ln(t, xb, M, pw.w2, lw.ffn_b2, pw.w1, lw.ffn_b1, F, x2, o3, s));
   return CGG_OK;
 }
 
@@ -315,7 +216,7 @@
   TcWs o;
   o.carve(t, batch);
   TcSeg sq[1] = {seg(0, C, at<float>(ws, o.qf), C, false, false, qscale)};
-  TST(tc_linear(t, at<__nv_bfloat16>(ws, o.xqb), M, C, t->pl[layer].wq_c, C, w->layers[layer].cross_in_b, sq, 1, s, false, 1, 0,
+  TST(tc_linear(t, at<__nv_bfloat16>(ws, o.xqb), M, C, t->pl[layer].wq_c, C, w->layers[layer].cross_in_b, sq, 1, s, false,
                 true));
   return CGG_OK;
 }
diff --git a/betrayed-by-captions_b200/csrc/tc_ptx.cuh b/betrayed-by-captions_b200/csrc/tc_ptx.cuh
--- a/betrayed-by-captions_b200/csrc/tc_ptx.cuh
+++ b/betrayed-by-captions_b200/csrc/tc_ptx.cuh
@@ -121,6 +121,15 @@
 __device__ __forceinline__ void cluster_sync_all() {
   asm volatile("barrier.cluster.arrive.release.aligned;\n\tbarrier.cluster.wait.acquire.aligned;" ::: "memory");
 }
+__device__ __forceinline__ uint32_t dsmem_map(uint32_t smem_addr, uint32_t rank) {
+  uint32_t r;
+  asm volatile("mapa.shared::cluster.u32 %0, %1, %2;" : "=r"(r) : "r"(smem_addr), "r"(rank));
+  return r;
+}
+__device__ __forceinline__ void dsmem_st4(uint32_t cluster_addr, float a, float b, float c, float d) {
+  asm volatile("st.shared::cluster.v4.f32 [%0], {%1, %2, %3, %4};" ::"r"(cluster_addr), "f"(a), "f"(b), "f"(c), "f"(d)
+               : "memory");
+}
 
 __device__ __forceinline__ void tma_store_3d(const CUtensorMap* m, const void* smem_src, int c0, int c1, int c2) {
   asm volatile("cp.async.bulk.tensor.3d.global.shared::cta.bulk_group [%0, {%2, %3, %4}], [%1];"
diff --git a/betrayed-by-captions_b200/csrc/tc_state.h b/betrayed-by-captions_b200/csrc/tc_state.h
--- a/betrayed-by-captions_b200/csrc/tc_state.h
+++ b/betrayed-by-captions_b200/csrc/tc_state.h
@@ -31,7 +31,7 @@
   int nh_padded = 0;
   bool packed_alloc = false;
   bool smem_attr_set = false, attn_attr_set = false;
-  bool attr_kv_pair = false, attr_bits = false, attr_ein_t = false, attr_ein_pair = false;
+  bool attr_kv_pair = false, attr_bits = false, attr_layer_ln = false, attr_ein_t = false, attr_ein_pair = false;
   uint8_t* live_buf = nullptr;
   size_t live_bytes = 0;
   void free_all() {
@@ -52,7 +52,7 @@
 inline int pitch8(int k) { return (k + 7) & ~7; }
 
 struct TcWs {
-  size_t me_all, fds[3], memp[3], xqb, xb, ob, fb, zb, h1b, h2b, qf, qs, kvs, x1, x2, t1, total;
+  size_t me_all, fds[3], memp[3], xqb, xb, ob, zb, h1b, h2b, qf, qs, kvs, x1, x2, total;
   void carve(const TcState* t, int B) {
     size_t off = 0;
     auto take = [&](size_t b) { size_t o = off; off += (b + 255) & ~(size_t)255; return o; };
@@ -65,10 +65,9 @@
       memp[l] = take((K % 8) ? (size_t)B * C * pitch8(K) * 2 : 0);
     }
     xqb = take(M * C * 2); xb = take(M * C * 2); ob = take(M * C * 2);
-    fb = take(M * t->cfg.ffn_dim * 2);
     zb = take(M * 2 * C * 2); h1b = take(M * 2 * C * 2); h2b = take(M * 2 * C * 2);
     qf = take(M * C * 4); qs = take(M * C * 4); kvs = take(M * 2 * C * 4);
-    x1 = take(M * C * 4); x2 = take(M * C * 4); t1 = take(4 * M * C * 4);
+    x1 = take(M * C * 4); x2 = take(M * C * 4);
     total = off;
   }
 };
diff --git a/betrayed-by-captions_b200/lib.py b/betrayed-by-captions_b200/lib.py
--- a/betrayed-by-captions_b200/lib.py
+++ b/betrayed-by-captions_b200/lib.py
@@ -11,7 +11,7 @@
 
 EXPORTS = ['cgg_create', 'cgg_destroy', 'cgg_last_error', 'cgg_version', 'cgg_launch_count', 'cgg_prepare', 'cgg_workspace_bytes', 'cgg_workspace_offset',
            'cgg_decoder_forward', 'cgg_kv_project', 'cgg_head_call', 'cgg_attn_mask_from_logits',
-           'cgg_decoder_layer', 'cgg_mask_einsum', 'cgg_masked_attention', 'cgg_noun_embeddings', 'cgg_similarity',
+           'cgg_decoder_layer', 'cgg_linear_ln', 'cgg_mask_einsum', 'cgg_masked_attention', 'cgg_noun_embeddings', 'cgg_similarity',
            'cgg_grounding_scratch_bytes', 'cgg_grounding_loss', 'cgg_grounding_bwd_scratch_bytes',
            'cgg_grounding_loss_backward', 'cgg_set_final_mask_only',
            'cgg_gemm_f32', 'cgg_layernorm', 'cgg_layernorm_bwd_scratch_bytes', 'cgg_layernorm_backward', 'cgg_relu_backward',
@@ -92,6 +92,7 @@
     lib.cgg_attn_mask_from_logits.argtypes = [vp, i, vp, i, i, i, i, vp, vp, vp]
     lib.cgg_decoder_layer.argtypes = [vp, C.POINTER(Weights), i, i, vp, vp, vp, vp, vp, sz, vp]
     lib.cgg_masked_attention.argtypes = [vp, i, i, vp, vp, vp, C.c_long, C.c_long, vp, vp, vp, vp]
+    lib.cgg_linear_ln.argtypes = [vp, i] + [vp] * 16
     lib.cgg_noun_embeddings.argtypes = [vp, vp, vp, vp, vp, i, i, C.c_float, i, vp, vp]
     lib.cgg_similarity.argtypes = [vp, vp, vp, i, i, i, C.c_float, vp, vp]
     lib.cgg_grounding_scratch_bytes.argtypes = [i, i, i]
diff --git a/include/cgg_b200.h b/include/cgg_b200.h
--- a/include/cgg_b200.h
+++ b/include/cgg_b200.h
@@ -104,6 +104,11 @@
                          const void *v, long kv_stride, long kv_batch_stride,
                          const uint32_t *bitmap, const uint8_t *all_masked,
                          float *out, void *stream);
+
+int cgg_linear_ln(cgg_handle *h, int rows, const void *X, const void *W, const float *bias, const void *W1,
+                  const float *b1, const float *res, const float *ln_w, const float *ln_b, float *out_f32,
+                  void *out_h, void *out_hq, const float *qe, void *out_hl, const float *w2, const float *b2,
+                  void *stream);
 
 
 int cgg_noun_embeddings(cgg_handle *h, const float *table, const float *ln_w, const float *ln_b,
```
